# sloisel/MultiGridBarrierMPI.jl

Hardware: AMD Instinct MI355X
Metric: fem2d p-Laplace DoF/s per Newton step (higher is better)
Workload: dtype f64; 1 GPU; fem2d p-Laplace L=7 p=1 (n=57344 rows, N_L=49154 Newton unknowns), amgb main phase, tol=sqrt(eps); parallelism=single GPU

## Files before the change

### include/mgb_hip.h

```cpp
#ifndef MGB_HIP_H
#define MGB_HIP_H

#include <stdint.h>

#ifdef __cplusplus
extern "C" {
#endif

#define MGB_OK 0
#define MGB_E_ARG (-1)
#define MGB_E_HIP (-2)
#define MGB_E_NUMERIC (-3)
#define MGB_E_INTERNAL (-4)

typedef struct mgb_ctx_s* mgb_ctx;
typedef struct mgb_geo_s* mgb_geo;
typedef struct mgb_amg_s* mgb_amg;
typedef struct mgb_vec_s* mgb_vec;
typedef struct mgb_csr_s* mgb_csr;

const char* mgb_last_error(void);
int mgb_version(void);
int mgb_device_count(void);

// ... 43 lines not shown
int mgb_col_extract(mgb_vec M, int n, int K, int k, mgb_vec out);
int mgb_map_rows_barrier(int which, int K, int nterms, const int* kind, const int* nq, const int* idx_q, const int* idx_s,
                         const int* idx_s2, const double* p, const double* coef, const double* off, int n, mgb_vec Dz,
                         mgb_vec out);
int mgb_mul(mgb_vec x, mgb_vec y, mgb_vec out);
int mgb_axpy(mgb_vec x, double alpha, mgb_vec y, mgb_vec out);
int mgb_vec_allreduce_sum(mgb_vec x);
int mgb_all_isfinite(mgb_vec x, int* out);

int mgb_amg_create(mgb_ctx ctx, mgb_geo g, int S, const char* const* state_vars, int K, const char* const* D,
                   int nq, const int* idx_q, int idx_s, double p, mgb_amg* out);
int mgb_amg_create_cones(mgb_ctx ctx, mgb_geo g, int S, const char* const* state_vars, int K, const char* const* D,
                         int ncones, const int* nq, const int* idx_q, const int* idx_s, const int* idx_s2,
                         const double* p, mgb_amg* out);
int mgb_amg_create_terms(mgb_ctx ctx, mgb_geo g, int S, const char* const* state_vars, int K, const char* const* D,
                         int nterms, const int* kind, const int* nq, const int* idx_q, const int* idx_s, const int* idx_s2,
                         const double* p, const double* coef, const double* off, mgb_amg* out);
int mgb_amg_set_exponents(mgb_amg a, int term, const double* p_nodes);
int mgb_amg_set_term_mask(mgb_amg a, const unsigned char* mask);
int mgb_amg_destroy(mgb_amg a);
int mgb_amg_dims(mgb_amg a, int* n, int* S, int* K, int* L, int* nY);
int mgb_amg_local_rows(mgb_amg a, int* n_global, int* row0, int* n_local);
int mgb_amg_prepare(mgb_amg a, int level);
int mgb_amg_level_size(mgb_amg a, int level, int* N, int* nnz_lower);
int mgb_amg_f0_f32(mgb_amg a, int level, const float* s, float t, double* f0);
int mgb_amg_f1_f32(mgb_amg a, int level, const float* s, float t, float* g);
int mgb_amg_f2_f32(mgb_amg a, int level, const float* s, float t, float* lower_vals);
int mgb_amg_f1_template_f64(mgb_amg a, int level, const double* s, double t, double* g);
int mgb_amg_f2_template_f64(mgb_amg a, int level, const double* s, double t, double* lower_vals);
int mgb_amg_chol_info(mgb_amg a, int level, int* split_world, double* exchange_doubles, int* launches);
int mgb_amg_chol_schedule(mgb_amg a, int level, int cap, int* nlaunch, int* kind, int* workgroups, int* unknown_node,
                          int* unknown_col);
int mgb_amg_chol_tree(mgb_amg a, int level, int cap, int* nnodes, int* ns, int* nf, int* parent);
int mgb_amg_chol_values_local(mgb_amg a, int level, int* yes);
int mgb_amg_hessian_pattern(mgb_amg a, int level, int32_t* rowptr, int32_t* colidx);
int mgb_amg_set_c(mgb_amg a, const double* c);
int mgb_amg_set_z(mgb_amg a, const double* z);
int mgb_amg_get_z(mgb_amg a, double* z);
int mgb_amg_apply_D(mgb_amg a, int level, const double* s, double* Dz );
int mgb_amg_f0(mgb_amg a, int level, const double* s, double t, double* y, double* parts2);
int mgb_amg_f0_trial(mgb_amg a, int level, const double* s_ref, const double* s, double t, double* y);
int mgb_amg_f1(mgb_amg a, int level, const double* s, double t, double* g);
int mgb_amg_f2(mgb_amg a, int level, const double* s, double t, double* lower_vals);
int mgb_amg_solve_linear(mgb_amg a, int level, const double* lower_vals, const double* g, double* x);
int mgb_amg_solve_linear_gpu(mgb_amg a, int level, const double* lower_vals, const double* g, double* x);
int mgb_amg_set_solver(mgb_amg a, int solver);
int mgb_amg_set_schedule(mgb_amg a, int all_levels);
int mgb_amg_set_stop_rule(mgb_amg a, int upstream);
int mgb_amg_set_centering(mgb_amg a, int exact);
int mgb_amg_solve(mgb_amg a, double tol, double t0, double kappa, int maxit, int max_newton, int verbose);
int mgb_amg_set_early_stop(mgb_amg a, int col);
int mgb_amg_sol_info(mgb_amg a, int* nt, double* t_elapsed, double* time_factor, long long* counts4);
int mgb_amg_sol_get(mgb_amg a, long long* its , double* ts, double* c_dot_Dz);
int mgb_amg_sol_kernels(mgb_amg a, double* ms11, double* bytes11, long long* launches11);
int mgb_amg_time_kernels(mgb_amg a, int level, int reps, int nrot, double* ms8, double* bytes8);

int mgb_hessian_apply(mgb_amg a, int level, const double* s, const double* v, double* Hv, int matrix_free);
int mgb_smooth(mgb_amg a, int level, const double* s, const double* b, double* x, int degree, int sweeps, double lmax,
               int matrix_free, double* lmax_used);
int mgb_prolong(mgb_amg a, int level, const double* xc, double* xf);
int mgb_restrict(mgb_amg a, int level, const double* rf, double* rc);
int mgb_amg_prolongation(mgb_amg a, int level, int* rows, int* cols, int* nnz, int32_t* rowptr, int32_t* colidx, double* vals);
int mgb_amg_pcg_solve_linear(mgb_amg a, int level, const double* s, const double* g, double* x, int* iters, double* relres,
                             int* converged);
int mgb_amg_set_pcg(mgb_amg a, double rtol, int maxit, int degree, int power_its, double lo_frac, double hi_frac, int chunk,
                    int fallback, int assembled_top, int giveup);
int mgb_amg_sol_pcg(mgb_amg a, long long* counts4, double* time_s);
int mgb_amg_time_mg_kernels(mgb_amg a, int level, int reps, int nrot, double* ms6, double* bytes6, double* alg6);
int mgb_amg_mg_info(mgb_amg a, int top, int* coarsest);


typedef struct mgb_plan_s* mgb_plan;
int mgb_plan_create(mgb_geo g, int S, const char* const* state_vars, int K, const char* const* D, int nq,
                    const int* idx_q, int idx_s, int level, mgb_plan* out);
int mgb_reduction_scratch_doubles(int n_local, int max_level_unknowns, long long* out);
int mgb_plan_destroy(mgb_plan p);
int mgb_plan_prolongation(mgb_plan fine, mgb_plan coarse, int* rows, int* cols, int* nnz, int32_t* rowptr, int32_t* colidx,
                          double* vals);
int mgb_plan_sizes(mgb_plan p, int* N, int* nnz_lower, int* nnz_T, int* nnz_B);
int mgb_plan_pattern(mgb_plan p, int32_t* rowptr, int32_t* colidx);
int mgb_plan_eval_host(mgb_plan p, const double* Y , double* lower_vals);
int mgb_plan_shard(mgb_plan p, int S, int K, int rank, int world, int block, mgb_plan* out, int* r0, int* r1);
int mgb_plan_apply_B_host(mgb_plan p, const double* s , double* Bs );
int mgb_plan_apply_BT_host(mgb_plan p, const double* v , double* g );
int mgb_plan_chol_bench(mgb_plan p, const double* Y, int dim, int reps, double* seconds_per_factor,
                        double* seconds_per_solve, double* flops, double* front_doubles, double* residual);
typedef struct mgb_hostchol_s* mgb_hostchol;
int mgb_plan_hostchol_create(mgb_plan p, int dim, mgb_hostchol* out);
int mgb_hostchol_destroy(mgb_hostchol c);
int mgb_hostchol_info(mgb_hostchol c, int* n, int* threads, double* flops);
int mgb_hostchol_factor_solve(mgb_hostchol c, const double* lower_vals, const double* g, double* x);
int mgb_hostchol_partition(mgb_hostchol c, int world, int* split_world, int cap, int* nnodes, int* owner);
int mgb_hostchol_factor_solve_dist(mgb_hostchol c, int rank, int world, mgb_allreduce_fn fn, void* user,
                                   const double* lower_vals, const double* g, double* x);
int mgb_plan_hostchol_create_ranked(mgb_plan p, int dim, int K, int world, int block, mgb_hostchol* out);
int mgb_hostchol_rank_aligned(mgb_hostchol c, int world, int* aligned, int* top_values);
int mgb_hostchol_factor_solve_dist_local(mgb_hostchol c, int rank, int world, mgb_allreduce_fn fn, void* user,
                                         const double* local_lower_vals, const double* g, double* x);
int mgb_plan_chol_tree(mgb_plan p, int dim, int cap, int* nnodes, int* ns, int* nf, int* parent);
int mgb_plan_chol_bwd_fused(mgb_plan p, int dim, int cut, int top_nf, int threads, int* info, int cap_wg, int* wg, int cap_bdry,
                            int* bdry, int* slots, int cap_nodes, int* bofs, int* first);
int mgb_chol_selftest(int nx, int ny, double* max_residual, double* flops, double* seconds);

#ifdef __cplusplus
}
#endif
// ... 2 lines not shown
```

### multigridbarriermpi.jl_amd/__init__.py

```python
from __future__ import annotations

import math
from dataclasses import dataclass, field
from typing import Callable, Dict, List, Optional, Sequence

import numpy as np
import scipy.sparse as sp

from . import _lib
from ._lib import MGBError, call, dptr, f64, i32, iptr

import ctypes as C

__all__ = [
    "fem1d", "fem2d", "fem3d", "fem1d_mpi", "fem2d_mpi", "fem3d_mpi", "fem1d_mpi_solve", "fem2d_mpi_solve",
    "fem3d_mpi_solve", "parabolic_solve", "ParabolicSOL", "native_to_mpi",
    "mpi_to_native", "amgb", "Geometry", "AMGBSOL", "HPCVector", "HPCMatrix", "HPCSparseMatrix",
    "backend_hip", "amgb_zeros", "amgb_all_isfinite", "amgb_diag", "amgb_blockdiag", "map_rows", "map_rows_gpu",
    "_raw_array", "_to_cpu_array", "MGBError", "device_count", "AMG", "amg", "hcat", "BarrierFn", "barrier_functions",
]


def device_count() -> int:
    return int(_lib.load().mgb_device_count())
# ... 918 lines not shown
        rp, ci, va = np.empty(r.value + 1, dtype=np.int32), np.empty(nz.value, dtype=np.int32), np.empty(nz.value)
        call("mgb_amg_prolongation", self.handle, l, None, None, None, iptr(rp), iptr(ci), dptr(va))
        return sp.csr_matrix((va, ci, rp), shape=(r.value, c.value))

    def pcg_solve_linear(self, l, s, g):
        s, g = f64(s), f64(g)
        x = np.empty_like(g)
        it, ok, rr = C.c_int(), C.c_int(), C.c_double()
        call("mgb_amg_pcg_solve_linear", self.handle, l, dptr(s), dptr(g), dptr(x), C.byref(it), C.byref(rr), C.byref(ok))
        return x, it.value, rr.value, bool(ok.value)

    MG_KERNEL_NAMES = ("hessian_apply", "chebyshev_step", "hessian_apply_csr", "prolong", "restrict", "hessian_apply_unfused_csr")

    def time_mg_kernels(self, l, reps=50, nrot=1):
        ms, by, alg = np.empty(6), np.empty(6), np.empty(6)
        call("mgb_amg_time_mg_kernels", self.handle, int(l), int(reps), int(nrot), dptr(ms), dptr(by), dptr(alg))
        return {k: dict(ms=float(a), bytes=float(b), algorithmic_bytes=float(c)) for k, a, b, c in zip(self.MG_KERNEL_NAMES, ms, by, alg)}

    def mg_coarsest(self, top=None):
        c0 = C.c_int()
        call("mgb_amg_mg_info", self.handle, self.L - 1 if top is None else int(top), C.byref(c0))
        return c0.value

    def solve(self, tol=None, t=0.1, kappa=10.0, maxit=10000, max_newton=0, verbose=0, schedule="fine",
              solver="gpu", stop_rule="fixed", centering="exact"):
        if schedule not in ("fine", "all"):
            raise ValueError("schedule must be 'fine' or 'all'")
        if stop_rule not in ("fixed", "upstream"):
            raise ValueError("stop_rule must be 'fixed' or 'upstream'")
        if centering not in ("decrement", "exact"):
            raise ValueError("centering must be 'decrement' or 'exact'")
        call("mgb_amg_set_stop_rule", self.handle, 1 if stop_rule == "upstream" else 0)
        call("mgb_amg_set_centering", self.handle, 1 if centering == "exact" else 0)
        call("mgb_amg_set_schedule", self.handle, 1 if schedule == "all" else 0)
        self.set_solver(solver)
        call("mgb_amg_solve", self.handle, float(tol or 0.0), float(t), float(kappa), int(maxit), int(max_newton),
             int(verbose))
        nt, te, tf = C.c_int(), C.c_double(), C.c_double()
        counts = (C.c_longlong * 4)()
        call("mgb_amg_sol_info", self.handle, C.byref(nt), C.byref(te), C.byref(tf), counts)
        its = np.empty(self.L * nt.value, dtype=np.int64)
        ts = np.empty(nt.value)
        cd = np.empty(nt.value)
        call("mgb_amg_sol_get", self.handle, its.ctypes.data_as(_lib.c_ll_p), dptr(ts), dptr(cd))
        nk = len(self.KERNEL_NAMES)
        kms, kby = np.empty(nk), np.empty(nk)
        kl = np.empty(nk, dtype=np.int64)
        call("mgb_amg_sol_kernels", self.handle, dptr(kms), dptr(kby), kl.ctypes.data_as(_lib.c_ll_p))
        kernels = {k: dict(ms=float(m), bytes=float(b), launches=int(c))
                   for k, m, b, c in zip(self.KERNEL_NAMES, kms, kby, kl)}
        pc = (C.c_longlong * 4)()
        tp = C.c_double()
        call("mgb_amg_sol_pcg", self.handle, pc, C.byref(tp))
        return dict(t_elapsed=te.value, ts=ts, its=its.reshape(nt.value, self.L).T.copy(), c_dot_Dz=cd,
                    time_factor=tf.value, n_f0=counts[0], n_f1=counts[1], n_f2=counts[2], n_factor=counts[3],
                    kernels=kernels, pcg=dict(solves=pc[0], iterations=pc[1], fallbacks=pc[2], gave_up_at=pc[3], seconds=tp.value))

    KERNEL_NAMES = ("apply_D", "barrier_f2", "hessian_assemble", "barrier_f1", "restrict", "barrier_f0",
                    "chol_front_start", "chol_front_step", "chol_backward_rect", "chol_backward", "chol_front_single")

    def time_kernels(self, l, reps=50, nrot=1):
        ms = np.empty(8)
        by = np.empty(8)
        call("mgb_amg_time_kernels", self.handle, l, reps, int(nrot), dptr(ms), dptr(by))
        names = ("apply_D", "barrier_f2", "hessian_assemble", "barrier_f1", "restrict", "barrier_f0", "trial_f0")
        out = {k: dict(ms=float(m), bytes=float(b)) for k, m, b in zip(names, ms, by)}
        out["apply_D"]["element_local"] = bool(by[7])
        out["apply_D_csr"] = dict(ms=float(ms[7]), bytes=float(by[0]))
        return out

    def __del__(self):
        try:
            if getattr(self, "handle", None):
                _lib.load().mgb_amg_destroy(self.handle)
        except Exception:
            pass


def amg(geometry: Geometry, state_variables=DEFAULT_STATE, D=None, p=1.0, cones=None) -> AMG:
    return AMG(geometry, state_variables, D, p, cones=cones)


@dataclass
class AMGBSOL:
    z: object
    SOL_feasibility: Optional[dict]
    SOL_main: dict
    log: list
    geometry: Geometry


PHASE1_SLACK_FLOOR = 1.0
PHASE1_PENALTY = 10.0


def _phase1_slack(geometry, M: "AMG", p, z0, c, tol, schedule, solver):
    n, S = z0.shape
    K = len(M.D)
    cone, extras = M.cones[0], list(M.cones[1:])
    if len(extras) > 1 or cone[0] == "linear":
        raise NotImplementedError("amgb: the feasibility phase covers the power cone intersected with one half space")
    state1 = tuple(M.state_variables) + (("sigma", "full"),)
    D1 = tuple(M.D) + (("sigma", "id"),)
    terms = [(list(cone[0]), cone[1], K)]
    terms += [("linear", list(e[1]) + [K], list(map(float, e[2])) + [1.0], float(e[3])) for e in extras]
    terms.append(("linear", [K], [1.0], PHASE1_SLACK_FLOOR))
    Dz = M.apply_D_global(M.L - 1, np.zeros(M.level_size(M.L - 1)[0]))
    idx = list(cone[0])
# ... 250 lines not shown
```

### multigridbarriermpi.jl_amd/_lib.py

```python
from __future__ import annotations

import ctypes as C
import os

import numpy as np

_HERE = os.path.dirname(os.path.abspath(__file__))
LIB_PATH = os.path.join(_HERE, "lib", "libmgb_hip.so")

c_int_p = C.POINTER(C.c_int)
c_i32_p = C.POINTER(C.c_int32)
c_dbl_p = C.POINTER(C.c_double)
c_flt_p = C.POINTER(C.c_float)
c_ll_p = C.POINTER(C.c_longlong)
c_str_arr = C.POINTER(C.c_char_p)
H = C.c_void_p
ALLREDUCE_FN = C.CFUNCTYPE(C.c_int, C.c_void_p, C.c_void_p, C.c_longlong)


class MGBError(RuntimeError):
    def __init__(self, code, msg):
        super().__init__("mgb error %d: %s" % (code, msg))
        self.code = code

# ... 46 lines not shown
    "mgb_all_isfinite": [H, c_int_p],
    "mgb_amg_create": [H, H, C.c_int, c_str_arr, C.c_int, c_str_arr, C.c_int, c_int_p, C.c_int, C.c_double,
                       C.POINTER(H)],
    "mgb_amg_create_cones": [H, H, C.c_int, c_str_arr, C.c_int, c_str_arr, C.c_int, c_int_p, c_int_p, c_int_p, c_int_p,
                             c_dbl_p, C.POINTER(H)],
    "mgb_amg_create_terms": [H, H, C.c_int, c_str_arr, C.c_int, c_str_arr, C.c_int, c_int_p, c_int_p, c_int_p, c_int_p, c_int_p,
                             c_dbl_p, c_dbl_p, c_dbl_p, C.POINTER(H)],
    "mgb_amg_set_exponents": [H, C.c_int, c_dbl_p],
    "mgb_amg_set_term_mask": [H, C.POINTER(C.c_ubyte)],
    "mgb_amg_destroy": [H],
    "mgb_amg_dims": [H, c_int_p, c_int_p, c_int_p, c_int_p, c_int_p],
    "mgb_amg_local_rows": [H, c_int_p, c_int_p, c_int_p],
    "mgb_amg_prepare": [H, C.c_int],
    "mgb_amg_chol_info": [H, C.c_int, c_int_p, c_dbl_p, c_int_p],
    "mgb_amg_chol_schedule": [H, C.c_int, C.c_int, c_int_p, c_int_p, c_int_p, c_int_p, c_int_p],
    "mgb_amg_chol_tree": [H, C.c_int, C.c_int, c_int_p, c_int_p, c_int_p, c_int_p],
    "mgb_amg_chol_values_local": [H, C.c_int, c_int_p],
    "mgb_amg_level_size": [H, C.c_int, c_int_p, c_int_p],
    "mgb_amg_hessian_pattern": [H, C.c_int, c_i32_p, c_i32_p],
    "mgb_amg_set_c": [H, c_dbl_p],
    "mgb_amg_set_z": [H, c_dbl_p],
    "mgb_amg_get_z": [H, c_dbl_p],
    "mgb_amg_apply_D": [H, C.c_int, c_dbl_p, c_dbl_p],
    "mgb_amg_f0": [H, C.c_int, c_dbl_p, C.c_double, c_dbl_p, c_dbl_p],
    "mgb_amg_f0_trial": [H, C.c_int, c_dbl_p, c_dbl_p, C.c_double, c_dbl_p],
    "mgb_amg_f1": [H, C.c_int, c_dbl_p, C.c_double, c_dbl_p],
    "mgb_amg_f2": [H, C.c_int, c_dbl_p, C.c_double, c_dbl_p],
    "mgb_amg_set_early_stop": [H, C.c_int],
    "mgb_amg_f0_f32": [H, C.c_int, c_flt_p, C.c_float, c_dbl_p],
    "mgb_amg_f1_f32": [H, C.c_int, c_flt_p, C.c_float, c_flt_p],
    "mgb_amg_f2_f32": [H, C.c_int, c_flt_p, C.c_float, c_flt_p],
    "mgb_amg_f1_template_f64": [H, C.c_int, c_dbl_p, C.c_double, c_dbl_p],
    "mgb_amg_f2_template_f64": [H, C.c_int, c_dbl_p, C.c_double, c_dbl_p],
    "mgb_amg_solve_linear": [H, C.c_int, c_dbl_p, c_dbl_p, c_dbl_p],
    "mgb_amg_solve_linear_gpu": [H, C.c_int, c_dbl_p, c_dbl_p, c_dbl_p],
    "mgb_amg_set_solver": [H, C.c_int],
    "mgb_amg_set_schedule": [H, C.c_int],
    "mgb_amg_set_stop_rule": [H, C.c_int],
    "mgb_amg_set_centering": [H, C.c_int],
    "mgb_amg_set_pcg": [H, C.c_double, C.c_int, C.c_int, C.c_int, C.c_double, C.c_double, C.c_int, C.c_int, C.c_int, C.c_int],
    "mgb_amg_sol_pcg": [H, c_ll_p, c_dbl_p],
    "mgb_hessian_apply": [H, C.c_int, c_dbl_p, c_dbl_p, c_dbl_p, C.c_int],
    "mgb_smooth": [H, C.c_int, c_dbl_p, c_dbl_p, c_dbl_p, C.c_int, C.c_int, C.c_double, C.c_int, c_dbl_p],
    "mgb_prolong": [H, C.c_int, c_dbl_p, c_dbl_p],
    "mgb_restrict": [H, C.c_int, c_dbl_p, c_dbl_p],
    "mgb_amg_prolongation": [H, C.c_int, c_int_p, c_int_p, c_int_p, c_i32_p, c_i32_p, c_dbl_p],
    "mgb_amg_pcg_solve_linear": [H, C.c_int, c_dbl_p, c_dbl_p, c_dbl_p, c_int_p, c_dbl_p, c_int_p],
    "mgb_amg_mg_info": [H, C.c_int, c_int_p],
    "mgb_amg_time_mg_kernels": [H, C.c_int, C.c_int, C.c_int, c_dbl_p, c_dbl_p, c_dbl_p],
    "mgb_plan_prolongation": [H, H, c_int_p, c_int_p, c_int_p, c_i32_p, c_i32_p, c_dbl_p],
    "mgb_amg_solve": [H, C.c_double, C.c_double, C.c_double, C.c_int, C.c_int, C.c_int],
    "mgb_amg_sol_info": [H, c_int_p, c_dbl_p, c_dbl_p, c_ll_p],
    "mgb_amg_sol_get": [H, c_ll_p, c_dbl_p, c_dbl_p],
    "mgb_amg_sol_kernels": [H, c_dbl_p, c_dbl_p, c_ll_p],
    "mgb_amg_time_kernels": [H, C.c_int, C.c_int, C.c_int, c_dbl_p, c_dbl_p],
    "mgb_plan_create": [H, C.c_int, c_str_arr, C.c_int, c_str_arr, C.c_int, c_int_p, C.c_int, C.c_int,
                        C.POINTER(H)],
    "mgb_reduction_scratch_doubles": [C.c_int, C.c_int, c_ll_p],
    "mgb_plan_destroy": [H],
    "mgb_plan_sizes": [H, c_int_p, c_int_p, c_int_p, c_int_p],
    "mgb_plan_pattern": [H, c_i32_p, c_i32_p],
    "mgb_plan_eval_host": [H, c_dbl_p, c_dbl_p],
    "mgb_plan_shard": [H, C.c_int, C.c_int, C.c_int, C.c_int, C.c_int, C.POINTER(C.c_void_p), c_int_p, c_int_p],
    "mgb_plan_apply_B_host": [H, c_dbl_p, c_dbl_p],
    "mgb_plan_apply_BT_host": [H, c_dbl_p, c_dbl_p],
    "mgb_plan_chol_bench": [H, c_dbl_p, C.c_int, C.c_int, c_dbl_p, c_dbl_p, c_dbl_p, c_dbl_p, c_dbl_p],
    "mgb_plan_hostchol_create": [H, C.c_int, C.POINTER(H)],
    "mgb_hostchol_destroy": [H],
    "mgb_hostchol_info": [H, c_int_p, c_int_p, c_dbl_p],
    "mgb_hostchol_factor_solve": [H, c_dbl_p, c_dbl_p, c_dbl_p],
    "mgb_hostchol_partition": [H, C.c_int, c_int_p, C.c_int, c_int_p, c_int_p],
    "mgb_hostchol_factor_solve_dist": [H, C.c_int, C.c_int, ALLREDUCE_FN, C.c_void_p, c_dbl_p, c_dbl_p, c_dbl_p],
    "mgb_plan_hostchol_create_ranked": [H, C.c_int, C.c_int, C.c_int, C.c_int, C.POINTER(H)],
    "mgb_hostchol_rank_aligned": [H, C.c_int, c_int_p, c_int_p],
    "mgb_hostchol_factor_solve_dist_local": [H, C.c_int, C.c_int, ALLREDUCE_FN, C.c_void_p, c_dbl_p, c_dbl_p, c_dbl_p],
    "mgb_plan_chol_tree": [H, C.c_int, C.c_int, c_int_p, c_int_p, c_int_p, c_int_p],
    "mgb_plan_chol_bwd_fused": [H, C.c_int, C.c_int, C.c_int, C.c_int, c_int_p, C.c_int, c_int_p, C.c_int, c_int_p, c_int_p, C.c_int,
                                c_int_p, c_int_p],
    "mgb_chol_selftest": [C.c_int, C.c_int, c_dbl_p, c_dbl_p, c_dbl_p],
}
_SPECIAL = {"mgb_last_error": ([], C.c_char_p), "mgb_version": ([], C.c_int), "mgb_device_count": ([], C.c_int)}

_lib = None


def load():
    global _lib
    if _lib is not None:
        return _lib
    if not os.path.exists(LIB_PATH):
        raise ImportError("libmgb_hip.so not built: run `python -c 'import __graft_entry__ as g; g.build()'` "
                          "or multigridbarriermpi.jl_amd/csrc/build.sh (expected at %s)" % LIB_PATH)
    lib = C.CDLL(LIB_PATH)
    for name, args in PROTOTYPES.items():
        fn = getattr(lib, name)
        fn.argtypes = args
        fn.restype = C.c_int
    for name, (args, res) in _SPECIAL.items():
        fn = getattr(lib, name)
        fn.argtypes = args
        fn.restype = res
    _lib = lib
    return lib


def call(name, *args):
# ... 29 lines not shown
```

### multigridbarriermpi.jl_amd/csrc/amg.cpp

```cpp
#include "amg.hpp"


#include <chrono>
#include <cmath>
#include <thread>
#include <string>
#include <cstdlib>
#include <cstdio>

namespace mgb {

void hip_check(hipError_t e, const char* what) {
  if (e != hipSuccess) throw HipError(std::string("HIP error in ") + what + ": " + hipGetErrorString(e));
}

static inline void cpu_relax() {
#if defined(__x86_64__) || defined(__i386__)
  __builtin_ia32_pause();
#elif defined(__aarch64__)
  asm volatile("yield" ::: "memory");
#else
  std::this_thread::yield();
#endif
}

static double now_s() {
  return std::chrono::duration<double>(std::chrono::steady_clock::now().time_since_epoch()).count();
}

Ctx::Ctx(int dev) : device(dev) {
  int count = 0;
  hip_check(hipGetDeviceCount(&count), "hipGetDeviceCount");
  if (count <= 0) throw HipError("mgb: no HIP device visible (the HIP path has no CPU fallback)");
  if (dev < 0 || dev >= count) throw ArgError("mgb: device id out of range");
  hip_check(hipSetDevice(dev), "hipSetDevice");
  hip_check(hipStreamCreateWithFlags(&stream, hipStreamNonBlocking), "hipStreamCreate");
}

Ctx::~Ctx() {
  drop_comm();
  if (stream) (void)hipStreamDestroy(stream);
}

void Ctx::allreduce_sum(double* dev_ptr, long long count, bool even_single) {
  if ((world <= 1 && !(even_single && rccl_comm)) || count <= 0) return;
  if (rccl_comm) {
    rccl_allreduce(dev_ptr, count);
  } else {
    if (!allreduce) throw ArgError("mgb: sharded context without a communicator (mgb_ctx_set_comm_rccl / mgb_ctx_set_comm)");
    hip_check(hipStreamSynchronize(stream), "sync before allreduce");
    const int rc = allreduce(allreduce_user, dev_ptr, count);
    if (rc != 0) throw InternalError("mgb: allreduce callback failed with code " + std::to_string(rc));
  }
  n_allreduce++;
  allreduce_bytes += 8.0 * count;
}
// ... 307 lines not shown
        gather(q, S, u);
        const int nc = (int)u.cols.size();
        for (int i = 0; i < nc; ++i)
          for (int j = 0; j <= i; ++j) {
            int e = -1;
            int slot = base;
            for (int a = 0; a < nact; ++a)
              for (int b = a; b < nact; ++b, ++slot) {
                if (!structural(u, nc, a, b, i, j)) continue;
                if (e < 0) e = entry(u.cols[i], u.cols[j]);
                double coef = u.val[(size_t)a * nc + i] * u.val[(size_t)b * nc + j];
                if (a != b) coef += u.val[(size_t)b * nc + i] * u.val[(size_t)a * nc + j];
                terms.push_back({e, q * nY + slot, coef});
                cnt[e]++;
              }
          }
        base += S.nY();
      }
    }
  });
  phase("list terms");
  {
    long long tot = 0;
    for (int e = 0; e < nnzA; ++e) {
      pl.T.rowptr[e] = (int)tot;
      for (int t = 0; t < nthr; ++t) {
        const int c0 = tcnt[t][e];
        tcnt[t][e] = (int)tot;
        tot += c0;
      }
      if (tot > 2000000000LL) throw ArgError("amg: Hessian plan exceeds Int32 indexing");
    }
    pl.T.rowptr[nnzA] = (int)tot;
    pl.T.colidx.resize((size_t)tot);
    pl.T.vals.resize((size_t)tot);
  }
  chunks([&](int, int, int tI) {
    std::vector<int>& pos = tcnt[tI];
    for (const Term& tm : tterms[tI]) {
      const int pp = pos[tm.e]++;
      pl.T.colidx[pp] = tm.col;
      pl.T.vals[pp] = tm.coef;
    }
    std::vector<Term>().swap(tterms[tI]);
  });
  phase("fill terms");
}


Amg::Amg(Ctx& ctx, const GeometryHost& g, const AmgSpec& spec, const BarrierParams& P)
    : ctx_(ctx), n_(g.n), S_((int)spec.state_variables.size()), P_(P), spec_(spec) {
  hip_check(hipSetDevice(ctx_.device), "hipSetDevice");
  if (const char* e = std::getenv("MGB_FUSED_TRIAL_ROWS")) fused_trial_rows_ = std::atoi(e);
  if (P.K != (int)spec.D.size()) throw ArgError("amg: barrier K != number of D rows");
  if (P.ncones < 1 || P.ncones > kMaxCones) throw ArgError("amg: barrier supports 1 to 3 terms");
  if (P.K > 8) throw ArgError("amg: the barrier kernels support at most 8 rows of D");
  for (int ci = 0; ci < P.ncones; ++ci) {
    const ConeSpec& S = P.cone[ci];
    if (S.kind != 0 && S.kind != 1) throw ArgError("amg: unknown barrier term kind");
    if (S.nq < 1 || S.nq > 3) throw ArgError("amg: barrier supports 1..3 gradient components");
    for (int a = 0; a < S.nact(); ++a)
      if (S.col(a) < 0 || S.col(a) >= P.K) throw ArgError("amg: barrier index out of range");
  }
  if ((int)g.w.size() != n_ || (int)g.x.size() != n_ * g.dim) throw ArgError("amg: geometry x/w size mismatch");
  ng_ = g.n;
  Csr Dstack = build_dstack(g, spec);
  w_min_ = *std::min_element(g.w.begin(), g.w.end());
  if (ctx_.world > 1) {
    int r1 = 0;
    shard_rows(ctx_.rank, ctx_.world, ng_, g.block, &r0_, &r1);
    n_ = r1 - r0_;
    Dstack_.upload(shard_dstack(Dstack, ng_, S_, P.K, r0_, r1));
  } else {
    Dstack_.upload(Dstack);
  }
  w_.upload(g.w.data() + r0_, n_);
  const int K = P.K, nY = P.nY();
  c_.alloc((size_t)n_ * K);
  z_.alloc((size_t)n_ * S_);
  z_save_.alloc((size_t)n_ * S_);
  Dz0_.alloc((size_t)n_ * K);
  Dz0_save_.alloc((size_t)n_ * K);
  Dz_.alloc((size_t)n_ * K);
  DzA_.alloc((size_t)n_ * K);
  DzB_.alloc((size_t)n_ * K);
  DzC_.alloc((size_t)n_ * K);
  v_.alloc((size_t)n_ * K);
  Y_.alloc((size_t)n_ * nY);
  phi_cur_.alloc((size_t)n_ * P.ncones);
  phi_trial_.alloc((size_t)n_ * P.ncones);
  phi_trial2_.alloc((size_t)n_ * P.ncones);
  phi_trial3_.alloc((size_t)n_ * P.ncones);
  h_flag_.alloc(4);
  scal_.alloc(12);
  h_scal_.alloc(12);
  seq_dev_.alloc(1);
  hip_check(hipMemset(seq_dev_.p, 0, sizeof(unsigned long long)), "memset seq");
  h_seq_.alloc(1);
  h_seq_.p[0] = 0;
  hip_check(hipMemsetAsync(c_.p, 0, c_.n * sizeof(double), ctx_.stream), "memset");
  hip_check(hipMemsetAsync(z_.p, 0, z_.n * sizeof(double), ctx_.stream), "memset");
  hip_check(hipStreamSynchronize(ctx_.stream), "sync");
  geo_ = g;
  dstack_host_ = std::move(Dstack);
  for (int l = 0; l < g.L; ++l) {
    levels_.emplace_back(new Level);
    int N = 0;
    for (auto& sv : spec.state_variables) {
      if (sv.second == "fixed") continue;
      auto it = g.subspaces.find(sv.second);
      if (it == g.subspaces.end() || l >= (int)it->second.size())
        throw ArgError("amg: unknown subspace '" + sv.second + "'");
      N += it->second[l].cols;
    }
    levels_[l]->plan.N = N;
  }
  int maxN = 0;
  for (auto& lv : levels_) maxN = std::max(maxN, lv->plan.N);
  partials_.alloc(reduction_scratch_doubles(n_, maxN));
  hip_check(hipMemset(partials_.p, 0, partials_.n * sizeof(double)), "memset scratch");
}

size_t reduction_scratch_doubles(int n_local, int max_level_unknowns) {
  return (size_t)6 * std::max(f0_blocks(n_local), f0_blocks(max_level_unknowns)) + 8 + kReductionHeader;
}

int Amg::level_index(const Level& lv) const {
  for (size_t l = 0; l < levels_.size(); ++l)
    if (levels_[l].get() == &lv) return (int)l;
  throw InternalError("amg: level not found");
}

Amg::Level& Amg::level(int l) {
  Level& lv = *levels_.at(l);
  if (lv.built) return lv;
  if (lv.chol_analysis.joinable()) lv.chol_analysis.join();
  lv.chol_analyzed = false;
  lv.chol_analysis_error = nullptr;
  hip_check(hipSetDevice(ctx_.device), "hipSetDevice");
  static const bool use_elasm = !(std::getenv("MGB_ASSEMBLE") && std::string(std::getenv("MGB_ASSEMBLE")) == "plan");
  const bool try_elasm = use_elasm && ctx_.world == 1 && geo_.block > 1 && n_ % geo_.block == 0;
  lv.plan = build_level_plan(geo_, spec_, dstack_host_, l, P_, !try_elasm);
  lv.T_built = !try_elasm;
  if (ctx_.world > 1) {
    std::vector<unsigned long long> mask = dof_rank_masks(lv.plan.B, ng_, P_.K, ctx_.world, geo_.block);
    lv.plan = shard_level_plan(lv.plan, ng_, S_, P_.K, P_.nY(), r0_, r0_ + n_);
    lv.plan.rank_mask = std::move(mask);
  }
  if (!pcg_ && lv.plan.N > 0) {
    lv.chol_analysis = std::thread([this, &lv] {
      try {
        analyze_chol(lv);
      } catch (...) {
        lv.chol_analysis_error = std::current_exception();
      }
    });
  }
  const double t_up = now_s();
  lv.R.upload(lv.plan.R);
  lv.B.upload(lv.plan.B);
  if (n_ > fused_trial_rows_ && geo_.block > 1 && n_ % geo_.block == 0) lv.Bel.build(lv.plan.B, geo_.block * P_.K);
  lv.BT.upload(lv.plan.BT);
  if (lv.T_built) lv.T.upload(lv.plan.T);
  if (try_elasm && lv.plan.N > 0) {
    mg_of(lv);
    if (mg_ensure_elop(lv)) lv.elasm.build(lv.mg->elop, lv.plan.Apat, P_);
    if (!lv.elasm.view.valid()) ensure_T(lv);
  }
  const int N = lv.plan.N, nnzA = lv.plan.Apat.nnz();
  lv.s.alloc(N);
  lv.s_trial.alloc(N);
  lv.s_trial2.alloc(N);
  lv.s_trial3.alloc(N);
  lv.g_trial.alloc(N);
  lv.g.alloc(N);
  lv.nstep.alloc(N);
  lv.avals.alloc(nnzA);
  lv.h_avals.alloc(nnzA);
  lv.h_g.alloc(N);
  lv.h_n.alloc(N);
  lv.h_s.alloc(N);
  if (std::getenv("MGB_VERBOSE_SETUP")) std::fprintf(stderr, "[mgb setup] level upload + buffers       %.3f s\n", now_s() - t_up);
  lv.built = true;
  return lv;
}

void Amg::analyze_chol(Level& lv) {
  static const bool aligned_on = !(std::getenv("MGB_RANK_ALIGNED") && std::atoi(std::getenv("MGB_RANK_ALIGNED")) == 0);
  const bool ranked = aligned_on && ctx_.world > 1 && (int)lv.plan.rank_mask.size() == lv.plan.N;
  lv.chol.analyze(lv.plan.Apat, lv.plan.coords.data(), geo_.dim, 64, ranked ? lv.plan.rank_mask.data() : nullptr, ctx_.world);
  lv.chol_analyzed = true;
}

void Amg::ensure_chol(Level& lv) {
  if (lv.chol_built) return;
  hip_check(hipSetDevice(ctx_.device), "hipSetDevice");
  static const bool vt = std::getenv("MGB_VERBOSE_SETUP") != nullptr;
  double t0 = now_s();
  if (lv.chol_analysis.joinable()) lv.chol_analysis.join();
  if (lv.chol_analysis_error) {
    std::exception_ptr e = lv.chol_analysis_error;
    lv.chol_analysis_error = nullptr;
    std::rethrow_exception(e);
  }
  if (!lv.chol_analyzed) analyze_chol(lv);
  if (vt) std::fprintf(stderr, "[mgb setup] chol analyze (rest)         %.3f s\n", now_s() - t0);
  t0 = now_s();
  lv.gchol.build(lv.chol, &ctx_);
  if (vt) std::fprintf(stderr, "[mgb setup] gpuchol build + upload      %.3f s\n", now_s() - t0);
  lv.chol_built = true;
}

static double csr_bytes(const DevCsr& A, bool y0);

void Amg::ensure_T(Level& lv) {
  if (!lv.T_built) {
    build_plan_terms(lv.plan, ng_, P_);
    lv.T_built = true;
  }
  if (lv.T.view.rows == 0 && lv.plan.T.rows > 0) {
    hip_check(hipSetDevice(ctx_.device), "hipSetDevice");
    lv.T.upload(lv.plan.T);
  }
}

double Amg::assemble_bytes(Level& lv) {
// ... 206 lines not shown

void Amg::dev_apply(Level& lv, const double* s_dev, double* dz) {
  timer_.begin(ctx_.stream, KC_APPLY, csr_bytes(lv.B.view, true));
  if (lv.Bel.view.valid()) launch_spmv_el(ctx_.stream, lv.B.view, lv.Bel.view, s_dev, Dz0_.p, dz);
  else launch_spmv(ctx_.stream, lv.B.view, s_dev, Dz0_.p, dz);
  timer_.end(ctx_.stream);
}

double Amg::trial_bytes(const Level& lv, bool with_ref) const {
  return csr_bytes(lv.B.view, true) + (double)n_ * (P_.K + 1 + P_.ncones * (with_ref ? 2 : 1)) * 8;
}

void Amg::enqueue_f0(Level& lv, const double* s_dev, double alpha, const double* nstep, double* s_out, double* dz,
                     const double* phi_ref, double* phi_out, double* out2, HostSignal sig) {
  if (n_ <= fused_trial_rows_) {
    timer_.begin(ctx_.stream, KC_F0, trial_bytes(lv, phi_ref != nullptr));
    launch_trial_f0(ctx_.stream, lv.B.view, n_, P_, s_dev, alpha, nstep, s_out, Dz0_.p, dz, w_.p, c_.p, phi_ref,
                    kFracToBoundary, phi_out, partials_.p, out2, host_scal(out2), sig);
    timer_.end(ctx_.stream);
    return;
  }
  const double* x = s_dev;
  if (nstep) {
    launch_waxpby(ctx_.stream, lv.plan.N, s_dev, alpha, nstep, s_out);
    x = s_out;
  }
  dev_apply(lv, x, dz);
  timer_.begin(ctx_.stream, KC_F0, (double)n_ * (2 * P_.K + 2 + (phi_ref ? 1 : 0)) * 8);
  launch_barrier_f0(ctx_.stream, n_, P_, dz, w_.p, c_.p, phi_ref, kFracToBoundary, phi_out, partials_.p, out2, host_scal(out2), sig);
  timer_.end(ctx_.stream);
}

double Amg::dev_f0(Level& lv, const double* s_dev, double t, double* parts, const double* phi_ref, double* phi_out,
                   double* dz, double alpha, const double* nstep, double* s_out) {
  enqueue_f0(lv, s_dev, alpha, nstep, s_out, dz, phi_ref, phi_out, scal_.p, next_signal());
  if (ctx_.world > 1) {
    ctx_.allreduce_sum(scal_.p, 2);
    hip_check(hipMemcpyAsync(h_scal_.p, scal_.p, 2 * sizeof(double), hipMemcpyDeviceToHost, ctx_.stream), "D2H scal");
  }
  wait_signal("sync f0");
  if (parts) {
    parts[0] = h_scal_.p[0];
    parts[1] = h_scal_.p[1];
  }
  return h_scal_.p[0] + t * h_scal_.p[1];
}

bool Amg::values_stay_local(Level& lv) {
  if (ctx_.world <= 1 || host_solve_) return false;
  ensure_chol(lv);
  return lv.gchol.values_local();
}

void Amg::enqueue_f2_assemble(Level& lv, const double* dz, SolveStats& st) {
  timer_.begin(ctx_.stream, KC_F2, (double)n_ * (P_.K + 1 + P_.nY()) * 8);
  launch_barrier_f2(ctx_.stream, n_, P_, dz, w_.p, Y_.p);
  timer_.end(ctx_.stream);
  if (pcg_) {
    mg_values(level_index(lv));
    st.n_f2++;
    return;
  }
  timer_.begin(ctx_.stream, KC_ASSEMBLE, assemble_bytes(lv));
  assemble_values(lv);
  timer_.end(ctx_.stream);
  if (!values_stay_local(lv)) ctx_.allreduce_sum(lv.avals.p, lv.plan.Apat.nnz());
  st.n_f2++;
}

double Amg::dev_f1(Level& lv, const double* dz, double t, double* g_out, SolveStats* st, const double** pre) {
  timer_.begin(ctx_.stream, KC_F1, (double)n_ * (3 * P_.K + 1) * 8);
  launch_barrier_f1(ctx_.stream, n_, P_, dz, w_.p, c_.p, t, v_.p);
  timer_.end(ctx_.stream);
  timer_.begin(ctx_.stream, KC_RESTRICT, csr_bytes(lv.BT.view, false));
  launch_spmv(ctx_.stream, lv.BT.view, v_.p, nullptr, g_out);
  timer_.end(ctx_.stream);
  if (owner_local(lv)) {
    const int ntop = lv.gchol.ntop_unknowns();
    if (gtop_.n < (size_t)ntop + 1) gtop_.alloc((size_t)ntop + 1);
    launch_gather_top(ctx_.stream, ntop, lv.gchol.top_unknowns(), g_out, gtop_.p);
    launch_dot_owned(ctx_.stream, lv.plan.N, g_out, g_out, lv.gchol.unknown_kind(), 0, partials_.p, gtop_.p + ntop);
    ctx_.allreduce_sum(gtop_.p, ntop + 1);
    launch_scatter_top_norm(ctx_.stream, ntop, lv.gchol.top_unknowns(), gtop_.p, g_out, scal_.p + 2);
  } else {
    ctx_.allreduce_sum(g_out, lv.plan.N);
    launch_dot(ctx_.stream, lv.plan.N, g_out, g_out, partials_.p, scal_.p + 2, host_scal(scal_.p + 2), nullptr, nullptr, next_signal());
  }
  if (ctx_.world > 1)
    hip_check(hipMemcpyAsync(h_scal_.p + 2, scal_.p + 2, sizeof(double), hipMemcpyDeviceToHost, ctx_.stream), "D2H gg");
  if (host_solve_)
    hip_check(hipMemcpyAsync(lv.h_g.p, g_out, (size_t)lv.plan.N * sizeof(double), hipMemcpyDeviceToHost, ctx_.stream),
              "D2H g");
  if (pre && st && !host_solve_) {
    if (!pcg_) ensure_chol(lv);
    if (ctx_.world > 1) {
      if (!ev_f1_) hip_check(hipEventCreateWithFlags(&ev_f1_, hipEventDisableTiming), "event");
      hip_check(hipEventRecord(ev_f1_, ctx_.stream), "record f1");
    }
    enqueue_f2_assemble(lv, dz, *st);
    *pre = dz;
    if (ctx_.world == 1) wait_signal("sync f1");
    else hip_check(hipEventSynchronize(ev_f1_), "sync f1 event");
  } else {
    wait_signal("sync f1");
  }
  return std::sqrt(h_scal_.p[2]);
}

static const double kBeta = 0.5, kArmijo = 0.1, kMinStep = 1e-8;

void Amg::enqueue_trial(Level& lv, Trial& T, double step, int slot, HostSignal sig) {
  double* out = scal_.p + 4 + 2 * slot;
  enqueue_f0(lv, lv.s.p, -step, lv.nstep.p, T.s, T.dz, phi_cur_.p, T.phi, out, sig);
  T.step = step;
}

static const double kSpecSteps[3] = {1.0, kBeta, kBeta * kBeta};

void Amg::enqueue_spec_trials(Level& lv, Trial* spec, HostSignal sig) {
  const int ns = spec_count();
  if (ns == 3) {
    TrialSet T;
    T.na = 3;
    for (int q = 0; q < 3; ++q) {
      T.alpha[q] = -kSpecSteps[q];
      T.s_out[q] = spec[q].s;
      T.dz[q] = spec[q].dz;
      T.phi_out[q] = spec[q].phi;
      spec[q].step = kSpecSteps[q];
    }
    T.out_dev = scal_.p + 4;
    T.out_host = host_scal(scal_.p + 4);
    timer_.begin(ctx_.stream, KC_F0, trial_bytes(lv, true) + 2.0 * n_ * (P_.K + P_.ncones) * 8);
    launch_trial_set(ctx_.stream, lv.B.view, n_, P_, lv.s.p, lv.nstep.p, T, Dz0_.p, w_.p, c_.p, phi_cur_.p, kFracToBoundary,
                     partials_.p, sig);
    timer_.end(ctx_.stream);
  } else {
    enqueue_trial(lv, spec[0], kSpecSteps[0], 0);
    enqueue_trial(lv, spec[1], kSpecSteps[1], 1, sig);
  }
}

void Amg::launch_step_graph(Level& lv, Trial* spec) {
  const void* key[15] = {lv.avals.p, lv.g.p, lv.nstep.p, lv.s.p, spec[0].s, spec[0].phi, spec[0].dz, spec[1].s, spec[1].phi,
                         spec[1].dz, spec[2].s,  spec[2].phi, spec[2].dz, phi_cur_.p, Dz0_.p};
  for (const auto& g : lv.step_graphs)
    if (std::equal(key, key + 15, g.key)) {
      hip_check(hipGraphLaunch(g.exec, ctx_.stream), "hipGraphLaunch");
      ++seq_expected_;
      for (int q = 0; q < spec_count(); ++q) spec[q].step = kSpecSteps[q];
      return;
    }
  hipGraph_t graph = nullptr;
  hip_check(hipStreamBeginCapture(ctx_.stream, hipStreamCaptureModeThreadLocal), "hipStreamBeginCapture");
  try {
    lv.gchol.enqueue_chain(ctx_.stream, lv.avals.p, lv.g.p, lv.nstep.p);
    launch_dot(ctx_.stream, lv.plan.N, lv.g.p, lv.nstep.p, partials_.p, scal_.p + 3, host_scal(scal_.p + 3), lv.gchol.fail_flag(),
               h_flag_.p);
    HostSignal sig;
    sig.seq_dev = seq_dev_.p;
    sig.seq_host = h_seq_.p;
    enqueue_spec_trials(lv, spec, sig);
  } catch (...) {
    (void)hipStreamEndCapture(ctx_.stream, &graph);
    if (graph) (void)hipGraphDestroy(graph);
    throw;
  }
  hip_check(hipStreamEndCapture(ctx_.stream, &graph), "hipStreamEndCapture");
  Level::StepGraph sg{};
  std::copy(key, key + 15, sg.key);
  hipError_t e = hipGraphInstantiate(&sg.exec, graph, nullptr, nullptr, 0);
  (void)hipGraphDestroy(graph);
  hip_check(e, "hipGraphInstantiate");
  lv.step_graphs.push_back(sg);
  hip_check(hipGraphLaunch(sg.exec, ctx_.stream), "hipGraphLaunch");
  ++seq_expected_;
}

bool Amg::dev_f2_solve(Level& lv, const double* dz, double t, SolveStats& st, double* inc, Trial* spec,
                       const double* pre_assembled) {
  const int N = lv.plan.N, nnzA = lv.plan.Apat.nnz();
  if (!pcg_) ensure_chol(lv);
  if (pre_assembled != dz) enqueue_f2_assemble(lv, dz, st);
  st.n_factor++;
  timer_.sample((st.n_factor % 8) == 1);
  if (pcg_) {
    const int top = level_index(lv);
    bool ok = pcg_run(lv, top, lv.g.p, lv.nstep.p, &st, nullptr, nullptr);
    if (!ok && pcg_last_code_ == 2.0) {
      for (int l = mg_coarsest(top); l <= top; ++l)
        if (level(l).mg) level(l).mg->ev_warm = false;
      mg_values(top);
      ok = pcg_run(lv, top, lv.g.p, lv.nstep.p, &st, nullptr, nullptr);
    }
    h_flag_.p[0] = 0;
    if (ok) pcg_bad_streak_ = 0;
    if (!ok) {
      if (!pcg_opt.fallback) return false;
      st.pcg_fallbacks++;
      if (pcg_opt.giveup > 0 && ++pcg_bad_streak_ >= pcg_opt.giveup) {
        pcg_ = false;
        st.pcg_gaveup_at = st.n_factor;
      }
      ensure_chol(lv);
      assemble_values(lv);
      lv.gchol.factor_solve(ctx_.stream, lv.avals.p, lv.g.p, lv.nstep.p, nullptr, false);
      lv.flag_armed = false;
      hip_check(hipMemcpyAsync(h_flag_.p, lv.gchol.fail_flag(), sizeof(int), hipMemcpyDeviceToHost, ctx_.stream), "D2H flag");
    }
    launch_dot(ctx_.stream, N, lv.g.p, lv.nstep.p, partials_.p, scal_.p + 3, host_scal(scal_.p + 3), nullptr, nullptr,
               spec ? HostSignal() : next_signal());
    if (spec) {
      enqueue_spec_trials(lv, spec, next_signal());
      st.n_f0 += spec_count();
    }
    wait_signal("sync pcg solve");
    if (!ok) hip_check(hipStreamSynchronize(ctx_.stream), "sync fallback flag");
    if (spec)
      for (int q = 0; q < spec_count(); ++q) {
        spec[q].y = h_scal_.p[4 + 2 * q] + t * h_scal_.p[5 + 2 * q];
        spec[q].valid = true;
      }
    *inc = h_scal_.p[3];
    return h_flag_.p[0] == 0;
  }
  if (!host_solve_) {
    const bool use_graph = GpuChol::knobs().graph;
    KernelTimer* tm = (live_ && timer_.sampling()) ? &timer_ : nullptr;
    const bool flag_rides = ctx_.world == 1;
    hipEvent_t e0 = nullptr, e1 = nullptr;
    const bool time_chain = live_ && timer_.enabled() && (st.n_factor % 8) == 5;
    if (flag_rides && spec && !tm && !time_chain && use_graph && lv.flag_armed) {
      launch_step_graph(lv, spec);
      st.n_f0 += spec_count();
    } else {
      if (time_chain) {
        hip_check(hipEventCreate(&e0), "event");
        hip_check(hipEventCreate(&e1), "event");
        hip_check(hipEventRecord(e0, ctx_.stream), "record");
      }
      const bool olocal = owner_local(lv);
      lv.gchol.factor_solve(ctx_.stream, lv.avals.p, lv.g.p, lv.nstep.p, tm, flag_rides && lv.flag_armed, false, olocal);
      if (time_chain) hip_check(hipEventRecord(e1, ctx_.stream), "record");
      if (olocal) {
        launch_dot_owned(ctx_.stream, N, lv.g.p, lv.nstep.p, lv.gchol.unknown_kind(), ctx_.rank == 0, partials_.p, scal_.p + 3);
        launch_flag_to_double(ctx_.stream, lv.gchol.fail_flag(), scal_.p + 10);
      } else if (flag_rides) {
        launch_dot(ctx_.stream, N, lv.g.p, lv.nstep.p, partials_.p, scal_.p + 3, host_scal(scal_.p + 3), lv.gchol.fail_flag(),
                   h_flag_.p, spec ? HostSignal() : next_signal());
        lv.flag_armed = true;
      } else {
        launch_dot(ctx_.stream, N, lv.g.p, lv.nstep.p, partials_.p, scal_.p + 3);
        hip_check(hipMemcpyAsync(h_flag_.p, lv.gchol.fail_flag(), sizeof(int), hipMemcpyDeviceToHost, ctx_.stream), "D2H flag");
      }
      if (spec) {
        enqueue_spec_trials(lv, spec, next_signal());
        if (!olocal) ctx_.allreduce_sum(scal_.p + 4, 2 * spec_count());
        st.n_f0 += spec_count();
      }
      if (olocal) {
        if (!spec) hip_check(hipMemsetAsync(scal_.p + 4, 0, 6 * sizeof(double), ctx_.stream), "zero trial slots");
        ctx_.allreduce_sum(scal_.p + 3, 8);
        hip_check(hipMemcpyAsync(h_scal_.p + 3, scal_.p + 3, 8 * sizeof(double), hipMemcpyDeviceToHost, ctx_.stream), "D2H inc + trials + flag");
      } else if (ctx_.world > 1)
        hip_check(hipMemcpyAsync(h_scal_.p + 3, scal_.p + 3, (spec ? 1 + 2 * spec_count() : 1) * sizeof(double),
                                 hipMemcpyDeviceToHost, ctx_.stream), "D2H inc + trials");
    }
    wait_signal("sync solve");
    if (owner_local(lv)) h_flag_.p[0] = h_scal_.p[10] != 0.0 ? 1 : 0;
    if (spec)
      for (int q = 0; q < spec_count(); ++q) {
        spec[q].y = h_scal_.p[4 + 2 * q] + t * h_scal_.p[5 + 2 * q];
        spec[q].valid = true;
      }
    if (e0) {
      float ms = 0;
      hip_check(hipEventSynchronize(e1), "sync chain event");
      if (hipEventElapsedTime(&ms, e0, e1) == hipSuccess) st.time_factor += 8.0 * ms * 1e-3;
      (void)hipEventDestroy(e0);
      (void)hipEventDestroy(e1);
    }
    *inc = h_scal_.p[3];
    if (h_flag_.p[0] != 0 && h_flag_.p[0] != 1)
      throw InternalError("gpuchol: pivot flag holds " + std::to_string(h_flag_.p[0]) + " (only 0 / 1 are ever written)");
    return h_flag_.p[0] == 0;
  }
  hip_check(hipMemcpyAsync(lv.h_avals.p, lv.avals.p, (size_t)nnzA * sizeof(double), hipMemcpyDeviceToHost, ctx_.stream),
            "D2H avals");
  sync_collect("sync f2");
  const double t0 = now_s();
  bool ok = lv.chol.factor(lv.h_avals.p);
  double acc = 0;
  if (ok) {
    std::copy(lv.h_g.p, lv.h_g.p + N, lv.h_n.p);
    lv.chol.solve(lv.h_n.p);
    for (int i = 0; i < N; ++i) acc += lv.h_g.p[i] * lv.h_n.p[i];
    hip_check(hipMemcpyAsync(lv.nstep.p, lv.h_n.p, (size_t)N * sizeof(double), hipMemcpyHostToDevice, ctx_.stream),
              "H2D n");
  }
  st.time_factor += now_s() - t0;
  *inc = acc;
  return ok;
}


Amg::NewtonResult Amg::newton(int l, double t, bool finest, bool final, double lam_tol, int maxit, SolveStats& st, int verbose) {
  Level& lv = level(l);
  const int N = lv.plan.N;
  NewtonResult res;
  if (N == 0) {
    res.converged = true;
    return res;
  }
  hip_check(hipMemsetAsync(lv.s.p, 0, (size_t)N * sizeof(double), ctx_.stream), "memset s");
  double y = dev_f0(lv, lv.s.p, t, nullptr, nullptr, phi_cur_.p, Dz_.p);
  st.n_f0++;
  if (!std::isfinite(y)) {
    std::vector<double> hdz((size_t)n_ * P_.K);
    Dz_.download(hdz.data(), hdz.size());
    int bad = 0, worst = -1;
    double minphi = INFINITY;
    for (int q = 0; q < n_; ++q) {
      const double* d = hdz.data() + (size_t)q * P_.K;
      double phi = INFINITY, sv = INFINITY;
      for (int ci = 0; ci < P_.ncones; ++ci) {
        const ConeSpec& S = P_.cone[ci];
        if (S.kind == 1) {
          double ph = S.off;
          for (int i = 0; i < S.nq; ++i) ph += S.coef[i] * d[S.iq[i]];
          phi = std::min(phi, ph);
          continue;
        }
        double qq = 0;
        for (int i = 0; i < S.nq; ++i) qq += d[S.iq[i]] * d[S.iq[i]];
        const double sc = d[S.is] + (S.is2 >= 0 ? d[S.is2] : 0.0);
        phi = std::min(phi, (sc > 0 ? std::pow(sc, S.a) : -1.0) - qq);
        sv = std::min(sv, sc);
      }
      if (!(phi > 0) || !(sv > 0)) bad++;
      if (!(phi >= minphi)) {
        minphi = phi;
        worst = q;
      }
    }
    char buf[256];
    snprintf(buf, sizeof buf, "newton: infeasible start (level %d, t=%g, %d of %d rows outside the cone, min phi=%g at row %d, y=%g)",
             l, t, bad, n_, minphi, worst, y);
    throw NumericError(buf);
  }
  double gnorm = dev_f1(lv, Dz_.p, t, lv.g.p);
  st.n_f1++;
  double ymin = y, gmin = gnorm, incmin = INFINITY;
  const double theta = finest ? 0.1 : 0.5;
  Trial T[3];
  T[0].s = lv.s_trial.p;
  T[0].phi = phi_trial_.p;
  T[1].s = lv.s_trial2.p;
  T[1].phi = phi_trial2_.p;
  T[2].s = lv.s_trial3.p;
  T[2].phi = phi_trial3_.p;
  T[0].dz = DzA_.p;
  T[1].dz = DzB_.p;
  T[2].dz = DzC_.p;
  auto eval = [&](int pos, double step) {
    if (!(T[pos].valid && T[pos].step == step))
      for (int q = 0; q < 3; ++q)
        if (q != pos && T[q].valid && T[q].step == step) {
          std::swap(T[pos], T[q]);
          break;
        }
    Trial& X = T[pos];
    if (X.valid && X.step == step) return X.y;
    X.y = dev_f0(lv, lv.s.p, t, nullptr, phi_cur_.p, X.phi, X.dz, -step, lv.nstep.p, X.s);
    st.n_f0++;
    X.step = step;
    X.valid = true;
    return X.y;
  };
  const double* pre = nullptr;
  const bool speculate = !host_solve_;
  while (res.k < maxit && !res.converged) {
    res.k++;
    double inc = 0;
    T[0].valid = T[1].valid = T[2].valid = false;
    const double* have = pre;
    pre = nullptr;
    if (!dev_f2_solve(lv, Dz_.p, t, st, &inc, speculate ? T : nullptr, have)) {
      if (verbose > 1) fprintf(stderr, "    [mgb] level %d k=%d: Hessian not numerically SPD (pivot flag %d)\n", l, res.k, h_flag_.p[0]);
      break;
    }
    if (!std::isfinite(inc)) {
      if (verbose > 1) fprintf(stderr, "    [mgb] level %d k=%d: non-finite Newton decrement\n", l, res.k);
      break;
    }
    if (inc <= 0) {
      res.converged = true;
      break;
    }
    double step = 1.0, ynext = y, gnext = gnorm;
    bool accepted = false;
    while (step >= kMinStep) {
      double yA = eval(0, step);
      if (std::isfinite(yA) && yA <= y - kArmijo * step * inc) {
        while (step * kBeta >= kMinStep) {
          const double yB = eval(1, step * kBeta);
          if (!(std::isfinite(yB) && yB < yA)) break;
          std::swap(T[0], T[1]);
          yA = yB;
          step *= kBeta;
        }
        const double gn = dev_f1(lv, T[0].dz, t, lv.g_trial.p, &st, speculate ? &pre : nullptr);
        st.n_f1++;
        if (std::isfinite(gn)) {
          ynext = yA;
          gnext = gn;
          accepted = true;
          break;
        }
      }
      step *= kBeta;
    }
    if (accepted) {
      std::swap(lv.s.p, T[0].s);
      std::swap(phi_cur_.p, T[0].phi);
      std::swap(lv.g.p, lv.g_trial.p);
      std::swap(Dz_.p, T[0].dz);
    } else {
      step = 0.0;
      if (host_solve_)
        hip_check(hipMemcpy(lv.h_g.p, lv.g.p, (size_t)N * sizeof(double), hipMemcpyDeviceToHost), "D2H g");
    }
    const bool exact = ynext >= ymin && gnext >= theta * gmin;
    const double dec_tol = finest ? kDecrementFrac * w_min_ : lam_tol;
    if ((!(finest && final) && inc < dec_tol) || exact) res.converged = true;
    y = ynext;
    gnorm = gnext;
    ymin = std::min(ymin, y);
    gmin = std::min(gmin, gnorm);
    incmin = std::min(incmin, inc);
    if (verbose > 1)
      fprintf(stderr, "    [mgb] level %d k=%d y=%.12g |g|=%.3g inc=%.3g step=%.3g\n", l, res.k, y, gnorm, inc, step);
  }
  lv.s_trial.p = T[0].s;
  lv.s_trial2.p = T[1].s;
  lv.s_trial3.p = T[2].s;
  phi_trial_.p = T[0].phi;
  phi_trial2_.p = T[1].phi;
  phi_trial3_.p = T[2].phi;
  DzA_.p = T[0].dz;
  DzB_.p = T[1].dz;
  DzC_.p = T[2].dz;
  return res;
}

bool Amg::amgb_step(double t, bool final, double lam_tol, int max_newton, std::vector<long long>& its, SolveStats& st, int verbose) {
  const int L = (int)levels_.size();
  bool converged = true;
  for (int J = (schedule_all_ ? 0 : L - 1); J < L; ++J) {
    Level& lv = level(J);
    NewtonResult r = newton(J, t, J == L - 1, final, lam_tol, max_newton, st, verbose);
    its[J] += r.k;
    if (lv.plan.N > 0) {
      launch_spmv(ctx_.stream, lv.R.view, lv.s.p, z_.p, z_.p);
      hip_check(hipMemcpyAsync(Dz0_.p, Dz_.p, (size_t)n_ * P_.K * sizeof(double), hipMemcpyDeviceToDevice,
                               ctx_.stream), "Dz0 <- Dz");
    }
    if (J == L - 1) converged = r.converged;
  }
  return converged;
}

double Amg::c_dot_dz() {
  launch_barrier_f0(ctx_.stream, n_, P_, Dz0_.p, w_.p, c_.p, nullptr, 0.0, nullptr, partials_.p, scal_.p, host_scal(scal_.p));
  if (ctx_.world > 1) {
    ctx_.allreduce_sum(scal_.p, 2);
    hip_check(hipMemcpyAsync(h_scal_.p, scal_.p, 2 * sizeof(double), hipMemcpyDeviceToHost, ctx_.stream), "D2H scal");
  }
  hip_check(hipStreamSynchronize(ctx_.stream), "sync");
  return h_scal_.p[1];
}

bool Amg::slack_negative() {
  std::vector<double> h((size_t)n_ * P_.K);
  hip_check(hipStreamSynchronize(ctx_.stream), "sync early stop");
  Dz0_.download(h.data(), h.size());
  double bad = 0;
  for (int q = 0; q < n_; ++q) bad += (h[(size_t)q * P_.K + early_stop_col_] < 0.0) ? 0.0 : 1.0;
  if (ctx_.world > 1) {
    hip_check(hipMemcpy(scal_.p, &bad, sizeof(double), hipMemcpyHostToDevice), "H2D early stop");
    ctx_.allreduce_sum(scal_.p, 1);
    hip_check(hipMemcpy(&bad, scal_.p, sizeof(double), hipMemcpyDeviceToHost), "D2H early stop");
  }
  return bad == 0.0;
}

void Amg::solve(const SolveOptions& opt, SolveStats& st) {
  hip_check(hipSetDevice(ctx_.device), "hipSetDevice");
  const int L = (int)levels_.size();
  st = SolveStats();
  st.L = L;
  live_ = &st;
  timer_.enable(opt.time_kernels);
  struct LiveGuard {
    Amg* a;
// ... 28 lines not shown
  double t_stop = t;
  while (t_stop <= 1 / opt.tol) t_stop *= kappa0;
  if (early_stop_col_ >= P_.K) throw ArgError("amgb: early-stop column out of range");
  const bool fixed = !opt.upstream_stop;
  auto going = [&](double tt) { return fixed ? tt < t_stop : tt <= 1 / opt.tol; };
  auto final_at = [&](double tt) { return opt.exact_centering || early_stop_col_ >= 0 || !going(tt); };
  {
    bool ok0 = false;
    for (int attempt = 0; attempt < kInitialCenteringAttempts && !ok0; ++attempt)
      ok0 = amgb_step(t, final_at(t), lam_tol, opt.max_newton, its, st, opt.verbose);
    if (!ok0) throw NumericError("amgb: initial centering failed");
  }
  st.its.insert(st.its.end(), its.begin(), its.end());
  st.ts.push_back(t);
  st.c_dot_Dz.push_back(c_dot_dz());
  int k = 1;
  bool stopped = early_stop_col_ >= 0 && slack_negative();
  while (going(t) && kappa > 1 && k < opt.maxit && !stopped) {
    k++;
    std::fill(its.begin(), its.end(), 0);
    while (kappa > 1) {
      const double t1 = fixed ? std::min(kappa * t, t_stop) : kappa * t;
      hip_check(hipMemcpyAsync(z_save_.p, z_.p, zbytes, hipMemcpyDeviceToDevice, ctx_.stream), "save z");
      hip_check(hipMemcpyAsync(Dz0_save_.p, Dz0_.p, dzbytes, hipMemcpyDeviceToDevice, ctx_.stream), "save Dz0");
      std::vector<long long> it1(L, 0);
      bool ok = amgb_step(t1, final_at(t1), lam_tol, opt.max_newton, it1, st, opt.verbose);
      if (!going(t1) && !opt.exact_centering && early_stop_col_ < 0)
        for (int attempt = 0; attempt < kInitialCenteringAttempts - 1 && !ok; ++attempt)
          ok = amgb_step(t1, true, lam_tol, opt.max_newton, it1, st, opt.verbose);
      long long mx = 0;
      for (int l = 0; l < L; ++l) {
        its[l] += it1[l];
        mx = std::max(mx, it1[l]);
      }
      if (ok) {
        if (mx <= opt.max_newton * kKappaGrowFrac) kappa = std::min(kappa0, kappa * kappa);
        t = t1;
        break;
      }
      hip_check(hipMemcpyAsync(z_.p, z_save_.p, zbytes, hipMemcpyDeviceToDevice, ctx_.stream), "restore z");
      hip_check(hipMemcpyAsync(Dz0_.p, Dz0_save_.p, dzbytes, hipMemcpyDeviceToDevice, ctx_.stream), "restore Dz0");
      kappa = std::sqrt(kappa);
      if (kappa < 1 + 1e-3) kappa = 1.0;
    }
    st.its.insert(st.its.end(), its.begin(), its.end());
    st.ts.push_back(t);
    st.c_dot_Dz.push_back(c_dot_dz());
    if (opt.verbose)
      fprintf(stderr, "[mgb] t=%.4g kappa=%.3g its(finest)=%lld c.Dz=%.12g\n", t, kappa, its[L - 1], st.c_dot_Dz.back());
    stopped = early_stop_col_ >= 0 && slack_negative();
  }
  hip_check(hipStreamSynchronize(ctx_.stream), "sync");
  st.t_elapsed = now_s() - t_begin;
  if (going(t) && !stopped) throw NumericError("amgb: convergence failure (kappa collapsed)");
}


double Amg::f0(int l, const double* s_host, double t, double* parts) {
  Level& lv = level(l);
  resync_signals();
  lv.s_trial.upload(s_host, lv.plan.N);
  return dev_f0(lv, lv.s_trial.p, t, parts, nullptr, phi_cur_.p, Dz_.p);
}

double Amg::f0_trial(int l, const double* s_ref_host, const double* s_host, double t) {
  Level& lv = level(l);
  resync_signals();
  lv.s_trial.upload(s_ref_host, lv.plan.N);
  dev_f0(lv, lv.s_trial.p, t, nullptr, nullptr, phi_cur_.p, Dz_.p);
  lv.s_trial.upload(s_host, lv.plan.N);
  return dev_f0(lv, lv.s_trial.p, t, nullptr, phi_cur_.p, phi_trial_.p, Dz_.p);
}

void Amg::f1(int l, const double* s_host, double t, double* g_host) {
  Level& lv = level(l);
  resync_signals();
  lv.s_trial.upload(s_host, lv.plan.N);
  dev_apply(lv, lv.s_trial.p, Dz_.p);
  dev_f1(lv, Dz_.p, t, lv.g_trial.p);
  lv.g_trial.download(g_host, lv.plan.N);
}

void Amg::f2(int l, const double* s_host, double t, double* avals_host) {
  (void)t;
  Level& lv = level(l);
  resync_signals();
  lv.s_trial.upload(s_host, lv.plan.N);
  dev_apply(lv, lv.s_trial.p, Dz_.p);
  launch_barrier_f2(ctx_.stream, n_, P_, Dz_.p, w_.p, Y_.p);
  assemble_values(lv);
  ctx_.allreduce_sum(lv.avals.p, lv.plan.Apat.nnz());
  hip_check(hipStreamSynchronize(ctx_.stream), "sync f2");
  lv.avals.download(avals_host, lv.plan.Apat.nnz());
}

void Amg::ensure_f32(Level& lv) {
  const size_t nK = (size_t)n_ * P_.K;
  if (w32_.n != (size_t)n_) {
    w32_.alloc(n_);
    c32_.alloc(nK);
    Dz0_32_.alloc(nK);
    Dz32_.alloc(nK);
    v32_.alloc(nK);
    Y32_.alloc((size_t)n_ * P_.nY());
    rowF_.alloc(n_);
    rowC_.alloc(n_);
  }
  launch_to_f32(ctx_.stream, n_, w_.p, w32_.p);
  launch_to_f32(ctx_.stream, (long long)nK, c_.p, c32_.p);
// ... 213 lines not shown
```

### multigridbarriermpi.jl_amd/csrc/amg.hpp

```cpp
#pragma once
#include <memory>
#include <string>
#include <utility>
#include <thread>
#include <exception>
#include <vector>

#include "geometry.hpp"
#include "gpuchol.hpp"
#include "kernels.hpp"
#include "mfchol.hpp"
#include "mg.hpp"

namespace mgb {

void hip_check(hipError_t e, const char* what);

typedef int (*AllreduceFn)(void* user, double* dev_ptr, long long count);

struct Ctx {
  int device = 0;
  hipStream_t stream = nullptr;
  int rank = 0, world = 1;
  AllreduceFn allreduce = nullptr;
// ... 115 lines not shown
  Csr R;
  Csr B;
  Csr BT;
  Csr Apat;
  Csr T;
  std::vector<double> coords;
  std::vector<unsigned long long> rank_mask;
};

void shard_rows(int rank, int world, int n, int block, int* r0, int* r1);
std::vector<unsigned long long> dof_rank_masks(const Csr& B, int n, int K, int world, int block);
LevelPlan shard_level_plan(const LevelPlan& full, int n, int S, int K, int nY, int r0, int r1);
Csr shard_dstack(const Csr& Dstack, int n, int S, int K, int r0, int r1);

size_t reduction_scratch_doubles(int n_local, int max_level_unknowns);

Csr build_dstack(const GeometryHost& g, const AmgSpec& spec);
LevelPlan build_level_plan(const GeometryHost& g, const AmgSpec& spec, const Csr& Dstack, int level,
                           const BarrierParams& P, bool with_T = true);
void build_plan_terms(LevelPlan& pl, int n, const BarrierParams& P);

enum KernelClass {
  KC_APPLY = 0, KC_F2 = 1, KC_ASSEMBLE = 2, KC_F1 = 3, KC_RESTRICT = 4, KC_F0 = 5,
  KC_CHOL_START = 6, KC_CHOL_STEP = 7, KC_CHOL_BWD_RECT = 8, KC_CHOL_BWD = 9, KC_CHOL_SINGLE = 10, KC_COUNT = 11
};

constexpr double kFracToBoundary = 0.1;
constexpr double kKappaGrowFrac = 0.25;
constexpr int kInitialCenteringAttempts = 8;
constexpr double kDecrementFrac = 0.01;

struct SolveOptions {
  bool host_solve = false;
  bool pcg = false;
  bool schedule_all = false;
  bool time_kernels = true;
  bool upstream_stop = false;
  bool exact_centering = true;
  double tol = 1.4901161193847656e-08;
  double t0 = 0.1;
  double kappa = 10.0;
  int maxit = 10000;
  int max_newton = 48;
  int verbose = 0;
};

struct SolveStats {
  int L = 0;
  std::vector<long long> its;
  std::vector<double> ts, c_dot_Dz;
  double t_elapsed = 0, t_setup = 0;
  double time_factor = 0, time_device = 0;
  long long n_factor = 0, n_f0 = 0, n_f1 = 0, n_f2 = 0;
  long long pcg_solves = 0, pcg_iters = 0, pcg_fallbacks = 0;
  long long pcg_gaveup_at = -1;
  double time_pcg = 0;
  double kern_ms[KC_COUNT] = {};
  double kern_bytes[KC_COUNT] = {};
  long long kern_launches[KC_COUNT] = {};
};

class KernelTimer {
 public:
  ~KernelTimer();
  void enable(bool on) { on_ = on; sampling_ = true; }
  void sample(bool now) { sampling_ = now; }
  bool sampling() const { return on_ && sampling_; }
  bool enabled() const { return on_; }
  void begin(hipStream_t st, int cls, double bytes);
  void end(hipStream_t st);
  void collect(SolveStats& st);
 private:
  struct Pair {
    hipEvent_t a, b;
    int cls;
    double bytes;
  };
  std::vector<Pair> free_, pending_;
  Pair cur_{};
  bool on_ = false, open_ = false, sampling_ = true;
};

class Amg {
 public:
  Amg(Ctx& ctx, const GeometryHost& g, const AmgSpec& spec, const BarrierParams& P);
  int n() const { return n_; }
  int n_global() const { return ng_; }
  int row0() const { return r0_; }
  int S() const { return S_; }
  int K() const { return P_.K; }
  int L() const { return (int)levels_.size(); }
  int level_size(int l) const { return levels_[l]->plan.N; }
  const LevelPlan& plan(int l);
  void prepare(int l);
  const BarrierParams& params() const { return P_; }
  void chol_info(int l, int* split_world, double* exchange_doubles, int* launches);
  void chol_schedule(int l, int cap, int* nlaunch, int* kind, int* workgroups, int* unknown_node, int* unknown_col);
  void chol_tree(int l, int cap, int* nnodes, int* ns, int* nf, int* parent);
  bool chol_values_local(int l) { return values_stay_local(level(l)); }
  void set_early_stop(int col) { early_stop_col_ = col; }
  void set_exponents(int term, const double* p_nodes_global);
  void set_term_mask(const unsigned char* mask_global);
  void set_pcg(bool on) { pcg_ = on; }

  void set_c(const double* c_host);
  void set_z(const double* z_host);
  void get_z(double* z_host);

  double f0(int l, const double* s_host, double t, double* parts);
  double f0_trial(int l, const double* s_ref_host, const double* s_host, double t);
  void f1(int l, const double* s_host, double t, double* g_host);
  void f2(int l, const double* s_host, double t, double* avals_host);
  double f0_f32(int l, const float* s_host, float t);
  void f1_f32(int l, const float* s_host, float t, float* g_host);
  void f2_f32(int l, const float* s_host, float t, float* avals_host);
  void f1_tpl64(int l, const double* s_host, double t, double* g_host);
  void f2_tpl64(int l, const double* s_host, double t, double* avals_host);
  void apply_D(int l, const double* s_host, double* Dz_host);
  bool solve_host(int l, const double* avals, const double* g, double* nstep);
  bool solve_device(int l, const double* avals, const double* g, double* nstep);

  void solve(const SolveOptions& opt, SolveStats& st);

  struct KernelTimes {
    double apply_ms, f2_ms, assemble_ms, f1_ms, restrict_ms, f0_ms, trial_ms, apply_csr_ms, apply_el;
    double apply_bytes, f2_bytes, assemble_bytes, f1_bytes, restrict_bytes, f0_bytes, trial_bytes;
  };
  KernelTimes time_kernels(int l, int reps, int nrot = 1);

 private:
  struct Level {
    bool built = false, chol_built = false, T_built = false;
    DevElAsmOwned elasm;
    bool flag_armed = false;
    struct StepGraph {
      const void* key[15];
      hipGraphExec_t exec;
    };
    std::vector<StepGraph> step_graphs;
    std::thread chol_analysis;
    std::exception_ptr chol_analysis_error;
    bool chol_analyzed = false;
    ~Level() {
      if (chol_analysis.joinable()) chol_analysis.join();
      for (auto& g : step_graphs) (void)hipGraphExecDestroy(g.exec);
    }
    LevelPlan plan;
    DevCsrOwned R, B, BT, T;
    DevElCsrOwned Bel;
    DevBuf<float> B32, BT32, T32, s32, g32, avals32;
    bool f32_built = false;
    MfChol chol;
    GpuChol gchol;
    DevBuf<double> s, s_trial, s_trial2, s_trial3, g, g_trial, nstep, avals;
    PinnedBuf<double> h_avals, h_g, h_n, h_s;
    struct Mg {
      bool elop_tried = false, assembled = false, transfer = false, vectors = false;
      DevElOpOwned elop;
      DevBuf<double> elbuf;
      DevCsrOwned A;
      DevBuf<int> amap, diagpos, lo_rowptr, lo_colidx;
      DevCsrOwned P, PT;
      DevBuf<double> dinv, x, b, r, d0, d1, ev0, ev1, coef, Ainv;
      bool ev_warm = false;
    };
    std::unique_ptr<Mg> mg;
  };
  struct NewtonResult {
    int k = 0;
    bool converged = false;
  };
  Level& level(int l);
  int level_index(const Level& lv) const;
  void ensure_chol(Level& lv);
  void analyze_chol(Level& lv);
  void ensure_T(Level& lv);
  void assemble_values(Level& lv);
  double assemble_bytes(Level& lv);
  void refresh_dz0();
  void dev_apply(Level& lv, const double* s_dev, double* dz);
  double dev_f0(Level& lv, const double* s_dev, double t, double* parts, const double* phi_ref, double* phi_out,
                double* dz, double alpha = 0.0, const double* nstep = nullptr, double* s_out = nullptr);
  double trial_bytes(const Level& lv, bool with_ref) const;
  int fused_trial_rows_ = 64 * 2048;
  void enqueue_f0(Level& lv, const double* s_dev, double alpha, const double* nstep, double* s_out, double* dz,
                  const double* phi_ref, double* phi_out, double* out2, HostSignal sig = HostSignal());
  double dev_f1(Level& lv, const double* dz, double t, double* g_out, SolveStats* st = nullptr, const double** pre = nullptr);
  void enqueue_f2_assemble(Level& lv, const double* dz, SolveStats& st);
  bool values_stay_local(Level& lv);
  bool owner_local(Level& lv) { return in_solve_ && values_stay_local(lv); }
  bool in_solve_ = false;
  DevBuf<double> gtop_;
  struct EventHolder {
    hipEvent_t e = nullptr;
    ~EventHolder() {
      if (e) (void)hipEventDestroy(e);
    }
  } ev_f1_holder_;
  hipEvent_t& ev_f1_ = ev_f1_holder_.e;
  struct Trial {
    double* s = nullptr;
    double* phi = nullptr;
    double* dz = nullptr;
    double step = 0, y = 0;
    bool valid = false;
  };
  bool dev_f2_solve(Level& lv, const double* dz, double t, SolveStats& st, double* inc, Trial* spec = nullptr,
                    const double* pre_assembled = nullptr);
  void enqueue_trial(Level& lv, Trial& T, double step, int slot, HostSignal sig = HostSignal());
  int spec_count() const { return n_ <= fused_trial_rows_ ? 3 : 2; }
  void enqueue_spec_trials(Level& lv, Trial* spec, HostSignal sig);
  void launch_step_graph(Level& lv, Trial* spec);
  NewtonResult newton(int l, double t, bool finest, bool final, double lam_tol, int maxit, SolveStats& st, int verbose);
  bool amgb_step(double t, bool final, double lam_tol, int max_newton, std::vector<long long>& its, SolveStats& st, int verbose);
  double c_dot_dz();

 public:
  PcgOptions pcg_opt;
  void hessian_apply(int l, const double* s_host, const double* v_host, double* out_host, bool matrix_free);
  double mg_smooth(int l, const double* s_host, const double* b_host, double* x_host, int degree, int sweeps, double lmax,
                   bool matrix_free);
  void mg_prolong(int l, const double* xc_host, double* xf_host);
  void mg_restrict(int l, const double* rf_host, double* rc_host);
  int mg_coarsest(int top);
  bool pcg_solve_linear(int l, const double* s_host, const double* g_host, double* x_host, int* iters, double* relres);
  const Csr& prolongation_host(int l);
  struct MgKernelTimes {
    double ms[6], bytes[6], alg[6];
  };
  MgKernelTimes time_mg_kernels(int l, int reps, int nrot);

 private:
  Level::Mg& mg_of(Level& lv);
  void mg_ensure_vectors(Level& lv);
  bool mg_ensure_elop(Level& lv);
  void mg_ensure_assembled(Level& lv);
  void mg_ensure_transfer(int l);
  void mg_prepare(int top);
  bool mg_top_matrix_free(int top);
  void mg_values(int top);
  void mg_level_values(Level& lv, bool mf);
  void mg_estimate(Level& lv, bool mf, double lmax_given);
  void mg_apply(Level& lv, bool mf, const MgEpi& epi);
  void mg_smooth_pre(Level& lv, bool mf, const double* b, double* x, double* r, int degree, const double* done);
  void mg_smooth_post(Level& lv, bool mf, const double* b, double* x, double* r, int degree, const double* done);
  void mg_vcycle(int top, int l, const double* b, double* x, const double* done);
  bool pcg_run(Level& lv, int top, const double* g, double* x, SolveStats* st, int* iters, double* relres);
  void eval_Y_at(Level& lv, const double* s_host);
  std::vector<Csr> P_host_;
  DevBuf<double> mg_scal_, mg_scratch_, pcg_r_, pcg_z_, pcg_p_, pcg_Ap_;
  PinnedBuf<double> h_pcg_;
  DevBuf<int> mg_fail_;
  bool mg_inited_ = false;
  bool pcg_ = false;
  double pcg_last_code_ = 0;
  int pcg_bad_streak_ = 0;

  Ctx& ctx_;
  int n_ = 0, S_ = 0;
  int ng_ = 0, r0_ = 0;
  int early_stop_col_ = -1;
  bool slack_negative();
  DevBuf<float> w32_, c32_, Dz0_32_, Dz32_, v32_, Y32_;
  DevBuf<double> rowF_, rowC_, a_node_, mu_node_;
  DevBuf<unsigned char> term_mask_;
  void ensure_f32(Level& lv);
  BarrierParams P_;
  AmgSpec spec_;
  GeometryHost geo_;
  Csr dstack_host_;
  DevCsrOwned Dstack_;
  std::vector<std::unique_ptr<Level>> levels_;
  DevBuf<double> w_, c_, z_, z_save_, Dz0_, Dz0_save_, Dz_, DzA_, DzB_, DzC_, v_, Y_, partials_, scal_, phi_cur_, phi_trial_, phi_trial2_,
      phi_trial3_;
  PinnedBuf<int> h_flag_;
  bool host_solve_ = false;
  PinnedBuf<double> h_scal_;
  double w_min_ = 0;
  bool schedule_all_ = false;
  KernelTimer timer_;
  SolveStats* live_ = nullptr;
  void sync_collect(const char* what);
  DevBuf<unsigned long long> seq_dev_;
  PinnedBuf<unsigned long long> h_seq_;
  unsigned long long seq_expected_ = 0;
  void resync_signals();
  HostSignal next_signal();
  void wait_signal(const char* what);
  double* host_scal(double* dev_slot) const { return ctx_.world == 1 ? h_scal_.p + (dev_slot - scal_.p) : nullptr; }
};

}
```

### multigridbarriermpi.jl_amd/csrc/capi.cpp

```cpp
#include "../../include/mgb_hip.h"

#include <chrono>
#include <cmath>
#include <cstdlib>
#include <string>
#include <thread>

#include "amg.hpp"

using namespace mgb;

struct mgb_ctx_s {
  Ctx ctx;
  explicit mgb_ctx_s(int dev) : ctx(dev) {}
};
struct mgb_geo_s {
  GeometryHost g;
};
struct mgb_vec_s {
  mgb_ctx_s* ctx;
  DevBuf<double> buf;
  int n;
};
struct mgb_csr_s {
// ... 506 lines not shown
    std::vector<double> h(z->n);
    hip_check(hipStreamSynchronize(ctx->ctx.stream), "sync");
    z->buf.download(h.data(), z->n);
    Csr A(m, n);
    for (int i = 0; i < m; ++i) {
      if (i < d) {
        A.colidx.push_back(i);
        A.vals.push_back(h[i]);
      }
      A.rowptr[i + 1] = (int)A.colidx.size();
    }
    *out = new_csr(ctx, std::move(A));
  });
}
int mgb_spmv_add(mgb_csr A, mgb_vec x, mgb_vec y0, mgb_vec y) {
  return guard([&] {
    need(A && x && y, "null argument");
    need(A->A.view.cols == x->n && A->A.view.rows == y->n && (!y0 || y0->n == y->n), "spmv: shape mismatch");
    launch_spmv(A->ctx->ctx.stream, A->A.view, x->buf.p, y0 ? y0->buf.p : nullptr, y->buf.p);
    hip_check(hipGetLastError(), "spmv launch");
  });
}
int mgb_spmv(mgb_csr A, mgb_vec x, mgb_vec y) { return mgb_spmv_add(A, x, nullptr, y); }
int mgb_dot(mgb_vec x, mgb_vec y, double* out) {
  return guard([&] {
    need(x && y && out && x->n == y->n, "dot: shape mismatch");
    *out = reduce_scalar(x, [&](hipStream_t st, double* parts, double* res) { launch_dot(st, x->n, x->buf.p, y->buf.p, parts, res); });
  });
}
int mgb_norm(mgb_vec x, double* out) {
  return guard([&] {
    need(x && out, "null argument");
    *out = std::sqrt(reduce_scalar(x, [&](hipStream_t st, double* parts, double* res) { launch_dot(st, x->n, x->buf.p, x->buf.p, parts, res); }));
  });
}
int mgb_sum(mgb_vec x, double* out) {
  return guard([&] {
    need(x && out, "null argument");
    *out = reduce_scalar(x, [&](hipStream_t st, double* parts, double* res) { launch_sum(st, x->n, x->buf.p, parts, res); });
  });
}
int mgb_col_extract(mgb_vec M, int n, int K, int k, mgb_vec out) {
  return guard([&] {
    need(M && out && n >= 0 && K >= 1 && k >= 0 && k < K, "col_extract: bad arguments");
    need((long long)n * K == M->n && out->n == n, "col_extract: shape mismatch");
    launch_col_extract(M->ctx->ctx.stream, n, K, k, M->buf.p, out->buf.p);
    hip_check(hipGetLastError(), "col_extract launch");
  });
}
int mgb_map_rows_barrier(int which, int K, int nterms, const int* kind, const int* nq, const int* idx_q, const int* idx_s,
                         const int* idx_s2, const double* p, const double* coef, const double* off, int n, mgb_vec Dz,
                         mgb_vec out) {
  return guard([&] {
    need(Dz && out && n >= 0 && K >= 1 && K <= 8 && which >= 0 && which <= 2, "map_rows_barrier: bad arguments");
    BarrierParams P = make_params_terms(K, nterms, kind, nq, idx_q, idx_s, idx_s2, p, coef, off);
    const long long want = which == 0 ? n : (which == 1 ? (long long)n * K : (long long)n * K * K);
    need((long long)n * K == Dz->n && out->n == want, "map_rows_barrier: shape mismatch");
    hipStream_t st = Dz->ctx->ctx.stream;
    hip_check(hipSetDevice(Dz->ctx->ctx.device), "hipSetDevice");
    if (which == 0) {
      launch_barrier_rows_F(st, n, P, Dz->buf.p, out->buf.p);
    } else {
      std::vector<double> ones((size_t)std::max(n, 1), 1.0);
      DevBuf<double> w;
      w.upload(ones.data(), ones.size());
      if (which == 1) {
        DevBuf<double> c;
        c.alloc((size_t)std::max(n, 1) * K);
        hip_check(hipMemsetAsync(c.p, 0, c.n * sizeof(double), st), "memset");
        if (n) launch_barrier_f1(st, n, P, Dz->buf.p, w.p, c.p, 0.0, out->buf.p);
        hip_check(hipStreamSynchronize(st), "sync");
      } else {
        DevBuf<double> Y;
        Y.alloc((size_t)std::max(n, 1) * P.nY());
        if (n) launch_barrier_f2(st, n, P, Dz->buf.p, w.p, Y.p);
        launch_expand_hessian_rows(st, n, P, Y.p, out->buf.p);
        hip_check(hipStreamSynchronize(st), "sync");
      }
    }
    hip_check(hipGetLastError(), "map_rows_barrier launch");
  });
}
int mgb_mul(mgb_vec x, mgb_vec y, mgb_vec out) {
  return guard([&] {
    need(x && y && out && x->n == y->n && x->n == out->n, "mul: shape mismatch");
    launch_mul(x->ctx->ctx.stream, x->n, x->buf.p, y->buf.p, out->buf.p);
  });
}
int mgb_axpy(mgb_vec x, double alpha, mgb_vec y, mgb_vec out) {
  return guard([&] {
    need(x && y && out && x->n == y->n && x->n == out->n, "axpy: shape mismatch");
    launch_waxpby(x->ctx->ctx.stream, x->n, x->buf.p, alpha, y->buf.p, out->buf.p);
  });
}
int mgb_vec_allreduce_sum(mgb_vec x) {
  return guard([&] {
    need(x, "null argument");
    x->ctx->ctx.allreduce_sum(x->buf.p, x->n, true);
    hip_check(hipStreamSynchronize(x->ctx->ctx.stream), "sync allreduce");
  });
}
int mgb_all_isfinite(mgb_vec x, int* out) {
  return guard([&] {
    need(x && out, "null argument");
    hipStream_t st = x->ctx->ctx.stream;
    DevBuf<int> flag;
    flag.alloc(1);
    launch_all_isfinite(st, x->n, x->buf.p, flag.p);
    hip_check(hipStreamSynchronize(st), "sync");
    int h = 0;
    flag.download(&h, 1);
    *out = h != 0;
  });
}

int mgb_amg_create(mgb_ctx ctx, mgb_geo g, int S, const char* const* state_vars, int K, const char* const* D, int nq,
                   const int* idx_q, int idx_s, double p, mgb_amg* out) {
  return guard([&] {
    need(ctx && g && out, "null argument");
// ... 328 lines not shown
    if (coarsest) *coarsest = a->amg->mg_coarsest(top);
  });
}
int mgb_amg_set_stop_rule(mgb_amg a, int upstream) {
  return guard([&] {
    need(a, "null amg");
    a->upstream_stop = upstream != 0;
  });
}
int mgb_amg_set_centering(mgb_amg a, int exact) {
  return guard([&] {
    need(a, "null amg");
    a->exact_centering = exact != 0;
  });
}
int mgb_amg_set_schedule(mgb_amg a, int all_levels) {
  return guard([&] {
    need(a, "null amg");
    a->schedule_all = all_levels != 0;
  });
}
int mgb_amg_solve(mgb_amg a, double tol, double t0, double kappa, int maxit, int max_newton, int verbose) {
  return guard([&] {
    need(a, "null amg");
    SolveOptions o;
    o.schedule_all = a->schedule_all;
    o.host_solve = a->host_solve;
    o.pcg = a->pcg;
    o.upstream_stop = a->upstream_stop;
    o.exact_centering = a->exact_centering;
    if (tol > 0) o.tol = tol;
    if (t0 > 0) o.t0 = t0;
    if (kappa > 1) o.kappa = kappa;
    if (maxit > 0) o.maxit = maxit;
    if (max_newton > 0) o.max_newton = max_newton;
    o.verbose = verbose;
    const double ts = a->stats.t_setup;
    a->amg->solve(o, a->stats);
    a->stats.t_setup = ts;
  });
}
int mgb_amg_sol_info(mgb_amg a, int* nt, double* t_elapsed, double* time_factor, long long* counts4) {
  return guard([&] {
    need(a, "null amg");
    if (nt) *nt = (int)a->stats.ts.size();
    if (t_elapsed) *t_elapsed = a->stats.t_elapsed;
    if (time_factor) *time_factor = a->stats.time_factor;
    if (counts4) {
      counts4[0] = a->stats.n_f0;
      counts4[1] = a->stats.n_f1;
      counts4[2] = a->stats.n_f2;
      counts4[3] = a->stats.n_factor;
    }
  });
}
int mgb_amg_sol_get(mgb_amg a, long long* its, double* ts, double* c_dot_Dz) {
  return guard([&] {
    need(a, "null amg");
    if (its) std::copy(a->stats.its.begin(), a->stats.its.end(), its);
    if (ts) std::copy(a->stats.ts.begin(), a->stats.ts.end(), ts);
    if (c_dot_Dz) std::copy(a->stats.c_dot_Dz.begin(), a->stats.c_dot_Dz.end(), c_dot_Dz);
  });
}
int mgb_amg_sol_kernels(mgb_amg a, double* ms11, double* bytes11, long long* launches11) {
  return guard([&] {
    need(a, "null amg");
    for (int i = 0; i < KC_COUNT; ++i) {
      if (ms11) ms11[i] = a->stats.kern_ms[i];
      if (bytes11) bytes11[i] = a->stats.kern_bytes[i];
      if (launches11) launches11[i] = a->stats.kern_launches[i];
    }
  });
}
int mgb_amg_time_kernels(mgb_amg a, int level, int reps, int nrot, double* ms8, double* bytes8) {
  return guard([&] {
    need(a && ms8 && bytes8 && reps > 0 && nrot >= 1 && nrot <= 64 && level >= 0 && level < a->amg->L(), "time_kernels: bad arguments");
    Amg::KernelTimes k = a->amg->time_kernels(level, reps, nrot);
    const double ms[8] = {k.apply_ms, k.f2_ms, k.assemble_ms, k.f1_ms, k.restrict_ms, k.f0_ms, k.trial_ms, k.apply_csr_ms};
    const double by[8] = {k.apply_bytes, k.f2_bytes, k.assemble_bytes, k.f1_bytes, k.restrict_bytes, k.f0_bytes, k.trial_bytes,
                          k.apply_el};
    std::copy(ms, ms + 8, ms8);
    std::copy(by, by + 8, bytes8);
  });
}

int mgb_plan_prolongation(mgb_plan fine, mgb_plan coarse, int* rows, int* cols, int* nnz, int32_t* rowptr, int32_t* colidx,
                          double* vals) {
  return guard([&] {
    need(fine && coarse, "null plan");
    Csr P = build_prolongation(fine->plan.R, coarse->plan.R);
    if (rows) *rows = P.rows;
    if (cols) *cols = P.cols;
    if (nnz) *nnz = P.nnz();
    if (rowptr) std::copy(P.rowptr.begin(), P.rowptr.end(), rowptr);
    if (colidx) std::copy(P.colidx.begin(), P.colidx.end(), colidx);
    if (vals) std::copy(P.vals.begin(), P.vals.end(), vals);
  });
}
int mgb_plan_create(mgb_geo g, int S, const char* const* state_vars, int K, const char* const* D, int nq,
                    const int* idx_q, int idx_s, int level, mgb_plan* out) {
  return guard([&] {
    need(g && out, "null argument");
    AmgSpec spec = make_spec(S, state_vars, K, D);
    BarrierParams P = make_params(K, nq, idx_q, idx_s, 1.0);
    Csr Dstack = build_dstack(g->g, spec);
    auto* p = new mgb_plan_s;
// ... 302 lines not shown
```

### multigridbarriermpi.jl_amd/csrc/devutil.hpp

```cpp
#pragma once
#include <hip/hip_runtime.h>

#include "kernels.hpp"

namespace mgb {
namespace {

constexpr int kBlock = 256;
constexpr int kMaxBlocks = 2048;

inline int grid_for(long long work_items) {
  long long b = (work_items + kBlock - 1) / kBlock;
  if (b < 1) b = 1;
  if (b > kMaxBlocks) b = kMaxBlocks;
  return (int)b;
}

__device__ inline unsigned xcd_block(unsigned b, unsigned nb) {
  if (nb < 16u) return b;
  const unsigned per = nb >> 3, main = per << 3;
  return b < main ? (b & 7u) * per + (b >> 3) : b;
}

__device__ inline double wave_sum(double v) {
#pragma unroll
  for (int o = 32; o > 0; o >>= 1) v += __shfl_down(v, o, 64);
  return v;
}

__device__ inline double block_sum(double v, double* lds) {
  v = wave_sum(v);
  const int wave = threadIdx.x >> 6;
  if ((threadIdx.x & 63) == 0) lds[wave] = v;
  __syncthreads();
  double r = 0.0;
  if (threadIdx.x == 0)
    for (int i = 0; i < kBlock / 64; ++i) r += lds[i];
  __syncthreads();
  return r;
}

template <int N>
__device__ inline void block_sum_n(const double (&v)[N], double (&out)[N]) {
  __shared__ double red[N][kBlock / 64];
  const int wave = threadIdx.x >> 6;
#pragma unroll
  for (int o = 0; o < N; ++o) {
    const double w = wave_sum(v[o]);
    if ((threadIdx.x & 63) == 0) red[o][wave] = w;
  }
  __syncthreads();
#pragma unroll
  for (int o = 0; o < N; ++o) {
    double r = 0.0;
    if (threadIdx.x == 0)
      for (int i = 0; i < kBlock / 64; ++i) r += red[o][i];
    out[o] = r;
  }
  __syncthreads();
}

constexpr int kTicketDoubles = kReductionHeader;
constexpr int kTicketStride = 32;
static_assert(kReductionHeader * sizeof(double) >= 9 * kTicketStride * sizeof(unsigned), "ticket words");
template <int NOUT>
__device__ inline void grid_finish(const double (&r)[NOUT] , double* scratch, double* out_dev,
                                   double* out_host, double* lds, HostSignal sig = HostSignal(), unsigned slot = 0xffffffffu) {
  if (slot == 0xffffffffu) slot = blockIdx.x;
  __shared__ int is_last;
  unsigned* ticket = reinterpret_cast<unsigned*>(scratch);
  double* partials = scratch + kTicketDoubles;
  if (threadIdx.x == 0) {
#pragma unroll
    for (int o = 0; o < NOUT; ++o)
      __hip_atomic_store(&partials[(size_t)slot * NOUT + o], r[o], __ATOMIC_RELAXED, __HIP_MEMORY_SCOPE_AGENT);
    asm volatile("s_waitcnt vmcnt(0)" ::: "memory");
    const unsigned shard = blockIdx.x & 7u, nshards = gridDim.x < 8u ? gridDim.x : 8u;
    const unsigned in_shard = (gridDim.x - shard + 7u) / 8u;
    bool last = false;
    if (__hip_atomic_fetch_add(&ticket[kTicketStride * shard], 1u, __ATOMIC_RELAXED, __HIP_MEMORY_SCOPE_AGENT) == in_shard - 1) {
      __hip_atomic_store(&ticket[kTicketStride * shard], 0u, __ATOMIC_RELAXED, __HIP_MEMORY_SCOPE_AGENT);
      last = __hip_atomic_fetch_add(&ticket[kTicketStride * 8], 1u, __ATOMIC_RELAXED, __HIP_MEMORY_SCOPE_AGENT) == nshards - 1;
      if (last) __hip_atomic_store(&ticket[kTicketStride * 8], 0u, __ATOMIC_RELAXED, __HIP_MEMORY_SCOPE_AGENT);
    }
    is_last = last;
  }
  __syncthreads();
  if (!is_last) return;
  double acc[NOUT];
#pragma unroll
  for (int o = 0; o < NOUT; ++o) acc[o] = 0.0;
  for (int i0 = threadIdx.x; i0 < (int)gridDim.x; i0 += 4 * kBlock) {
    double v[4][NOUT];
#pragma unroll
    for (int u = 0; u < 4; ++u) {
      const int i = min(i0 + u * kBlock, (int)gridDim.x - 1);
#pragma unroll
      for (int o = 0; o < NOUT; ++o) v[u][o] = __hip_atomic_load(&partials[(size_t)i * NOUT + o], __ATOMIC_RELAXED, __HIP_MEMORY_SCOPE_AGENT);
    }
#pragma unroll
    for (int u = 0; u < 4; ++u)
#pragma unroll
      for (int o = 0; o < NOUT; ++o) acc[o] = (i0 + u * kBlock < (int)gridDim.x) ? acc[o] + v[u][o] : acc[o];
  }
  double tot[NOUT];
  block_sum_n<NOUT>(acc, tot);
  (void)lds;
  if (threadIdx.x == 0) {
#pragma unroll
    for (int o = 0; o < NOUT; ++o) {
      if (out_dev) out_dev[o] = tot[o];
      if (out_host) __hip_atomic_store(&out_host[o], tot[o], __ATOMIC_RELAXED, __HIP_MEMORY_SCOPE_SYSTEM);
    }
  }
  if (sig.seq_host && threadIdx.x == 0) {
    asm volatile("s_waitcnt vmcnt(0)" ::: "memory");
    const unsigned long long q = __hip_atomic_load(sig.seq_dev, __ATOMIC_RELAXED, __HIP_MEMORY_SCOPE_AGENT) + 1;
    __hip_atomic_store(sig.seq_dev, q, __ATOMIC_RELAXED, __HIP_MEMORY_SCOPE_AGENT);
    __hip_atomic_store(sig.seq_host, q, __ATOMIC_RELEASE, __HIP_MEMORY_SCOPE_SYSTEM);
  }
}
template <int NOUT, class Fn>
__device__ inline void grid_finish_fn(const double (&r)[NOUT] , double* scratch, double* lds, Fn&& fn) {
  __shared__ int is_last_fn;
  unsigned* ticket = reinterpret_cast<unsigned*>(scratch);
  double* partials = scratch + kTicketDoubles;
  if (threadIdx.x == 0) {
#pragma unroll
    for (int o = 0; o < NOUT; ++o)
      __hip_atomic_store(&partials[(size_t)blockIdx.x * NOUT + o], r[o], __ATOMIC_RELAXED, __HIP_MEMORY_SCOPE_AGENT);
    asm volatile("s_waitcnt vmcnt(0)" ::: "memory");
    const unsigned shard = blockIdx.x & 7u, nshards = gridDim.x < 8u ? gridDim.x : 8u;
    const unsigned in_shard = (gridDim.x - shard + 7u) / 8u;
    bool last = false;
    if (__hip_atomic_fetch_add(&ticket[kTicketStride * shard], 1u, __ATOMIC_RELAXED, __HIP_MEMORY_SCOPE_AGENT) == in_shard - 1) {
      __hip_atomic_store(&ticket[kTicketStride * shard], 0u, __ATOMIC_RELAXED, __HIP_MEMORY_SCOPE_AGENT);
      last = __hip_atomic_fetch_add(&ticket[kTicketStride * 8], 1u, __ATOMIC_RELAXED, __HIP_MEMORY_SCOPE_AGENT) == nshards - 1;
      if (last) __hip_atomic_store(&ticket[kTicketStride * 8], 0u, __ATOMIC_RELAXED, __HIP_MEMORY_SCOPE_AGENT);
    }
    is_last_fn = last;
  }
  __syncthreads();
  if (!is_last_fn) return;
  double tot[NOUT], acc[NOUT];
#pragma unroll
  for (int o = 0; o < NOUT; ++o) acc[o] = 0.0;
  for (int i0 = threadIdx.x; i0 < (int)gridDim.x; i0 += 4 * kBlock) {
    double v[4][NOUT];
#pragma unroll
    for (int u = 0; u < 4; ++u) {
      const int i = min(i0 + u * kBlock, (int)gridDim.x - 1);
#pragma unroll
      for (int o = 0; o < NOUT; ++o) v[u][o] = __hip_atomic_load(&partials[(size_t)i * NOUT + o], __ATOMIC_RELAXED, __HIP_MEMORY_SCOPE_AGENT);
    }
#pragma unroll
    for (int u = 0; u < 4; ++u)
#pragma unroll
      for (int o = 0; o < NOUT; ++o) acc[o] = (i0 + u * kBlock < (int)gridDim.x) ? acc[o] + v[u][o] : acc[o];
  }
// ... 8 lines not shown
```

### multigridbarriermpi.jl_amd/csrc/kernels.hip

```cpp
#include "kernels.hpp"
#include "kernels_tpl.hpp"

#include <algorithm>
#include <cmath>

namespace mgb {

namespace {


template <int G>
void spmv_launch(hipStream_t st, const DevCsr& A, const double* x, const double* y0, double* y) {
  const int grid = grid_for((long long)A.rows * G);
  hipLaunchKernelGGL((spmv_kernel_t<G, double>), dim3(grid), dim3(kBlock), 0, st, A.rows, A.rowptr, A.colidx, A.vals, x, y0, y);
}

template <int G>
__global__ __launch_bounds__(kBlock) void spmv_el_kernel(int rows, DevElCsr E, const int* __restrict__ rowptr,
                                                          const double* __restrict__ vals, const double* __restrict__ x,
                                                          const double* y0, double* y) {
  extern __shared__ double xs[];
  const int lane = threadIdx.x % G, grp = threadIdx.x / G;
  constexpr int GR = kBlock / G;
  const int rpe = E.rows_per_el;
  const int els = max(1, min(E.nel, (kBlock * 4) / rpe));
  const int npass = (E.nel + els - 1) / els;
  for (int ps = xcd_block(blockIdx.x, gridDim.x); ps < npass; ps += gridDim.x) {
    const int e0 = ps * els, ne = min(els, E.nel - e0);
    __syncthreads();
    for (int idx = threadIdx.x; idx < ne * E.cmax; idx += kBlock) xs[idx] = x[E.ecols[(long long)e0 * E.cmax + idx]];
    __syncthreads();
    const long long r0 = (long long)e0 * rpe;
    const int nrows = (int)min((long long)ne * rpe, (long long)rows - r0);
    for (int rr0 = grp; rr0 < nrows; rr0 += kSpmvU * GR) {
      int b[kSpmvU], e[kSpmvU];
      double acc[kSpmvU], base[kSpmvU];
#pragma unroll
      for (int u = 0; u < kSpmvU; ++u) {
        const int rr = rr0 + u * GR;
        const bool ok = rr < nrows;
        b[u] = ok ? rowptr[r0 + rr] : 0;
        e[u] = ok ? rowptr[r0 + rr + 1] : 0;
        base[u] = (ok && y0 && lane == 0) ? y0[r0 + rr] : 0.0;
      }
#pragma unroll
      for (int u = 0; u < kSpmvU; ++u) {
        const int rr = rr0 + u * GR;
        const double* xe = xs + (rr / rpe) * E.cmax;
        const int k = b[u] + lane;
        acc[u] = (k < e[u]) ? vals[k] * xe[E.lcol[k]] : 0.0;
        for (int kk = k + G; kk < e[u]; kk += G) acc[u] += vals[kk] * xe[E.lcol[kk]];
      }
#pragma unroll
      for (int u = 0; u < kSpmvU; ++u) {
        double a = acc[u];
#pragma unroll
        for (int o = G / 2; o > 0; o >>= 1) a += __shfl_down(a, o, G);
        const int rr = rr0 + u * GR;
        if (lane == 0 && rr < nrows) y[r0 + rr] = base[u] + a;
      }
    }
  }
}

template <int G>
void spmv_el_launch(hipStream_t st, const DevCsr& A, const DevElCsr& E, const double* x, const double* y0, double* y) {
  const int els = std::max(1, std::min(E.nel, (kBlock * 4) / E.rows_per_el));
  const int npass = (E.nel + els - 1) / els;
  const int grid = std::max(1, std::min(npass, kMaxBlocks * 4));
  hipLaunchKernelGGL(spmv_el_kernel<G>, dim3(grid), dim3(kBlock), (size_t)els * E.cmax * sizeof(double), st, A.rows, E, A.rowptr,
                     A.vals, x, y0, y);
}


using Cone = ConeT<double>;

__global__ __launch_bounds__(kBlock) void barrier_f0_kernel(int n, BarrierParams P, const double* __restrict__ Dz,
                                                             const double* __restrict__ w,
                                                             const double* __restrict__ c,
                                                             const double* __restrict__ phi_ref, double frac,
                                                             double* __restrict__ phi_out, double* scratch,
                                                             double* out_dev, double* out_host, HostSignal sig) {
  __shared__ double lds[kBlock / 64];
  double accF = 0.0, accL = 0.0;
  for (long long q = (long long)blockIdx.x * kBlock + threadIdx.x; q < n; q += (long long)gridDim.x * kBlock) {
    const double* dz = Dz + q * P.K;
    const double* cq = c + q * P.K;
    const double wq = w[q];
    double F = 0.0;
    for (int ci = 0; ci < P.ncones; ++ci) {
      if (!P.active(ci, q)) {
        if (phi_out) phi_out[q * P.ncones + ci] = INFINITY;
        continue;
      }
      const ConeAM<double> am = cone_am<double>(P, ci, q);
      Cone k = load_cone<double>(P.cone[ci], dz, am.a);
      if (phi_ref && !(k.phi >= frac * phi_ref[q * P.ncones + ci])) k.ok = false;
      if (phi_out) phi_out[q * P.ncones + ci] = k.phi;
      F += k.ok ? (-log(k.phi) - am.mu * log(k.s)) : INFINITY;
    }
    accF += wq * F;
    double lin = 0.0;
    for (int j = 0; j < P.K; ++j) lin += cq[j] * dz[j];
    accL += wq * lin;
  }
  const double r[2] = {block_sum(accF, lds), block_sum(accL, lds)};
  grid_finish<2>(r, scratch, out_dev, out_host, lds, sig);
}


constexpr int kTrialNodes = 64;
template <int G, int NA>
__global__ __launch_bounds__(kBlock) void trial_f0_kernel(int n, int N, BarrierParams P, const int* __restrict__ rowptr,
                                                           const int* __restrict__ colidx, const double* __restrict__ vals,
                                                           const double* __restrict__ s, const double* __restrict__ nstep,
                                                           TrialSet T, const double* __restrict__ Dz0,
                                                           const double* __restrict__ w, const double* __restrict__ c,
                                                           const double* __restrict__ phi_ref, double frac, double* scratch,
                                                           HostSignal sig) {
  __shared__ double lds[kBlock / 64];
  __shared__ double dzs[NA][kTrialNodes * kMaxK];
  constexpr int GR = kBlock / G;
  const int K = P.K, lane = threadIdx.x % G, grp = threadIdx.x / G;
#pragma unroll
  for (int a = 0; a < NA; ++a)
    if (T.s_out[a])
      for (long long i = (long long)blockIdx.x * kBlock + threadIdx.x; i < N; i += (long long)gridDim.x * kBlock)
        T.s_out[a][i] = s[i] + T.alpha[a] * nstep[i];
  auto xval = [&](int j, int a) { return nstep ? s[j] + T.alpha[a] * nstep[j] : s[j]; };
  double accF = 0.0, accL = 0.0;
  const int pa = threadIdx.x >> 6, pnode = threadIdx.x & 63;
  const int nchunks = (n + kTrialNodes - 1) / kTrialNodes;
  for (int ch = xcd_block(blockIdx.x, gridDim.x); ch < nchunks; ch += gridDim.x) {
    const int q0 = ch * kTrialNodes, nq = min(kTrialNodes, n - q0), nrows = nq * K;
    const long long r0 = (long long)q0 * K;
    for (int rr0 = grp; rr0 < nrows; rr0 += kSpmvU * GR) {
      int b[kSpmvU], e[kSpmvU], ci[kSpmvU];
      double acc[NA][kSpmvU], base[kSpmvU], va[kSpmvU];
#pragma unroll
      for (int u = 0; u < kSpmvU; ++u) {
        const int rr = rr0 + u * GR;
        const bool ok = rr < nrows;
        b[u] = ok ? rowptr[r0 + rr] : 0;
        e[u] = ok ? rowptr[r0 + rr + 1] : 0;
        base[u] = (ok && lane == 0) ? Dz0[r0 + rr] : 0.0;
      }
#pragma unroll
      for (int u = 0; u < kSpmvU; ++u) {
        const int k = b[u] + lane;
        const bool in = k < e[u];
        ci[u] = in ? colidx[k] : -1;
        va[u] = in ? vals[k] : 0.0;
      }
#pragma unroll
      for (int a = 0; a < NA; ++a)
#pragma unroll
        for (int u = 0; u < kSpmvU; ++u) acc[a][u] = (ci[u] >= 0) ? va[u] * xval(ci[u], a) : 0.0;
#pragma unroll
      for (int u = 0; u < kSpmvU; ++u)
        for (int k = b[u] + lane + G; k < e[u]; k += G) {
          const double vk = vals[k];
          const int ck = colidx[k];
#pragma unroll
          for (int a = 0; a < NA; ++a) acc[a][u] += vk * xval(ck, a);
        }
#pragma unroll
      for (int a = 0; a < NA; ++a)
#pragma unroll
        for (int u = 0; u < kSpmvU; ++u) {
          double t = acc[a][u];
#pragma unroll
          for (int o = G / 2; o > 0; o >>= 1) t += __shfl_down(t, o, G);
          const int rr = rr0 + u * GR;
          if (lane == 0 && rr < nrows) {
            const double v = base[u] + t;
            T.dz[a][r0 + rr] = v;
            dzs[a][rr] = v;
          }
        }
    }
    __syncthreads();
    if (pa < NA && pnode < nq) {
      const long long q = q0 + pnode;
      const double* dz = dzs[pa] + pnode * K;
      const double* cq = c + q * K;
      const double wq = w[q];
      double* phi_out = T.phi_out[pa];
      double F = 0.0;
      for (int ci2 = 0; ci2 < P.ncones; ++ci2) {
        if (!P.active(ci2, q)) {
          if (phi_out) phi_out[q * P.ncones + ci2] = INFINITY;
          continue;
        }
        const ConeAM<double> am = cone_am<double>(P, ci2, q);
        Cone k = load_cone<double>(P.cone[ci2], dz, am.a);
        if (phi_ref && !(k.phi >= frac * phi_ref[q * P.ncones + ci2])) k.ok = false;
        if (phi_out) phi_out[q * P.ncones + ci2] = k.phi;
        F += k.ok ? (-log(k.phi) - am.mu * log(k.s)) : INFINITY;
      }
      accF += wq * F;
      double lin = 0.0;
      for (int j = 0; j < K; ++j) lin += cq[j] * dz[j];
      accL += wq * lin;
    }
    __syncthreads();
  }
  double r[2 * NA], mine[2 * NA];
#pragma unroll
  for (int a = 0; a < NA; ++a) {
    mine[2 * a] = pa == a ? accF : 0.0;
    mine[2 * a + 1] = pa == a ? accL : 0.0;
  }
  block_sum_n<2 * NA>(mine, r);
  grid_finish<2 * NA>(r, scratch, T.out_dev, T.out_host, lds, sig, xcd_block(blockIdx.x, gridDim.x));
}

inline int trial_grid(int n) {
  const int b = (n + kTrialNodes - 1) / kTrialNodes;
  return b < 1 ? 1 : (b > kMaxBlocks ? kMaxBlocks : b);
}

template <int G>
void trial_launch(hipStream_t st, const DevCsr& B, int n, const BarrierParams& P, const double* s, const double* nstep,
                  const TrialSet& T, const double* Dz0, const double* w, const double* c, const double* phi_ref, double frac,
                  double* scratch, HostSignal sig) {
#define MGB_TRIAL_NA(NA)                                                                                                    \
  hipLaunchKernelGGL((trial_f0_kernel<G, NA>), dim3(trial_grid(n)), dim3(kBlock), 0, st, n, B.cols, P, B.rowptr, B.colidx,   \
                     B.vals, s, nstep, T, Dz0, w, c, phi_ref, frac, scratch, sig)
  switch (T.na) {
    case 1: MGB_TRIAL_NA(1); break;
    case 2: MGB_TRIAL_NA(2); break;
    default: MGB_TRIAL_NA(3); break;
  }
#undef MGB_TRIAL_NA
}

__global__ __launch_bounds__(kBlock) void barrier_rows_F_kernel(int n, BarrierParams P, const double* __restrict__ Dz,
                                                                 double* __restrict__ out) {
  for (long long q = (long long)blockIdx.x * kBlock + threadIdx.x; q < n; q += (long long)gridDim.x * kBlock) {
    const double* dz = Dz + q * P.K;
    double F = 0.0;
    for (int ci = 0; ci < P.ncones; ++ci) {
      if (!P.active(ci, q)) continue;
      const ConeAM<double> am = cone_am<double>(P, ci, q);
      Cone k = load_cone<double>(P.cone[ci], dz, am.a);
      F += k.ok ? (-log(k.phi) - am.mu * log(k.s)) : INFINITY;
    }
    out[q] = F;
  }
}

__global__ __launch_bounds__(kBlock) void expand_hessian_rows_kernel(int n, BarrierParams P, const double* __restrict__ Y,
                                                                      double* __restrict__ out) {
  const int K = P.K, nY = P.nY();
  for (long long q = (long long)blockIdx.x * kBlock + threadIdx.x; q < n; q += (long long)gridDim.x * kBlock) {
    double* o = out + q * K * K;
    for (int e = 0; e < K * K; ++e) o[e] = 0.0;
    const double* yq = Y + q * nY;
    int slot = 0;
    for (int ci = 0; ci < P.ncones; ++ci) {
      const ConeSpec& S = P.cone[ci];
      const int nact = S.nact();
      for (int a = 0; a < nact; ++a)
        for (int b = a; b < nact; ++b, ++slot) {
          const int ra = S.col(a), rb = S.col(b);
          o[ra * K + rb] += yq[slot];
          if (ra != rb) o[rb * K + ra] += yq[slot];
        }
    }
  }
}

__global__ __launch_bounds__(kBlock) void waxpby_kernel(int n, const double* __restrict__ x, double alpha,
                                                         const double* __restrict__ y, double* out) {
  for (long long i = (long long)blockIdx.x * kBlock + threadIdx.x; i < n; i += (long long)gridDim.x * kBlock)
    out[i] = x[i] + alpha * y[i];
}

__global__ __launch_bounds__(kBlock) void mul_kernel(int n, const double* __restrict__ x, const double* __restrict__ y,
                                                      double* out) {
  for (long long i = (long long)blockIdx.x * kBlock + threadIdx.x; i < n; i += (long long)gridDim.x * kBlock)
    out[i] = x[i] * y[i];
}

__global__ __launch_bounds__(kBlock) void col_extract_kernel(int n, int K, int k, const double* __restrict__ M,
// ... 34 lines not shown
__global__ __launch_bounds__(kBlock) void gather_top_kernel(int ntop, const int* __restrict__ top, const double* __restrict__ g,
                                                             double* __restrict__ buf) {
  for (long long i = (long long)blockIdx.x * kBlock + threadIdx.x; i < ntop; i += (long long)gridDim.x * kBlock) buf[i] = g[top[i]];
}

__global__ __launch_bounds__(kBlock) void scatter_top_norm_kernel(int ntop, const int* __restrict__ top, const double* __restrict__ buf,
                                                                   double* __restrict__ g, double* out) {
  __shared__ double lds[kBlock / 64];
  double acc = 0.0;
  for (int i = threadIdx.x; i < ntop; i += kBlock) {
    const double v = buf[i];
    g[top[i]] = v;
    acc += v * v;
  }
  const double tot = block_sum(acc, lds);
  if (threadIdx.x == 0) out[0] = buf[ntop] + tot;
}

__global__ void flag_to_double_kernel(const int* flag_dev, double* out) {
  if (threadIdx.x == 0 && blockIdx.x == 0) out[0] = *flag_dev != 0 ? 1.0 : 0.0;
}

__global__ __launch_bounds__(kBlock) void sum_kernel(int n, const double* __restrict__ x, double* scratch, double* out_dev,
                                                      double* out_host) {
  __shared__ double lds[kBlock / 64];
  double acc = 0.0;
  for (long long i = (long long)blockIdx.x * kBlock + threadIdx.x; i < n; i += (long long)gridDim.x * kBlock) acc += x[i];
  const double r[1] = {block_sum(acc, lds)};
  grid_finish<1>(r, scratch, out_dev, out_host, lds);
}

__global__ __launch_bounds__(kBlock) void isfinite_kernel(int n, const double* __restrict__ x, int* flag) {
  int bad = 0;
  for (long long i = (long long)blockIdx.x * kBlock + threadIdx.x; i < n; i += (long long)gridDim.x * kBlock)
    bad |= !isfinite(x[i]);
  if (__any(bad) && (threadIdx.x & 63) == 0) atomicAnd(flag, 0);
}

}

void launch_spmv(hipStream_t st, const DevCsr& A, const double* x, const double* y0, double* y) {
  if (A.rows == 0) return;
  switch (A.group) {
    case 1: spmv_launch<1>(st, A, x, y0, y); break;
    case 2: spmv_launch<2>(st, A, x, y0, y); break;
    case 4: spmv_launch<4>(st, A, x, y0, y); break;
    case 8: spmv_launch<8>(st, A, x, y0, y); break;
    case 16: spmv_launch<16>(st, A, x, y0, y); break;
    case 32: spmv_launch<32>(st, A, x, y0, y); break;
    default: spmv_launch<64>(st, A, x, y0, y); break;
  }
}

void launch_spmv_el(hipStream_t st, const DevCsr& A, const DevElCsr& E, const double* x, const double* y0, double* y) {
  if (A.rows == 0) return;
  switch (A.group) {
    case 1: spmv_el_launch<1>(st, A, E, x, y0, y); break;
    case 2: spmv_el_launch<2>(st, A, E, x, y0, y); break;
    case 4: spmv_el_launch<4>(st, A, E, x, y0, y); break;
    case 8: spmv_el_launch<8>(st, A, E, x, y0, y); break;
    case 16: spmv_el_launch<16>(st, A, E, x, y0, y); break;
    case 32: spmv_el_launch<32>(st, A, E, x, y0, y); break;
    default: spmv_el_launch<64>(st, A, E, x, y0, y); break;
  }
}

void launch_waxpby(hipStream_t st, int n, const double* x, double alpha, const double* y, double* out) {
  if (n == 0) return;
  hipLaunchKernelGGL(waxpby_kernel, dim3(grid_for(n)), dim3(kBlock), 0, st, n, x, alpha, y, out);
}

int f0_blocks(int n) { return std::max(grid_for(n), trial_grid(n)); }

void launch_trial_set(hipStream_t st, const DevCsr& B, int n, BarrierParams P, const double* s, const double* nstep,
                      const TrialSet& T, const double* Dz0, const double* w, const double* c, const double* phi_ref, double frac,
                      double* scratch, HostSignal sig) {
#define MGB_TRIAL(G) trial_launch<G>(st, B, n, P, s, nstep, T, Dz0, w, c, phi_ref, frac, scratch, sig)
  switch (B.group) {
    case 1: MGB_TRIAL(1); break;
    case 2: MGB_TRIAL(2); break;
    case 4: MGB_TRIAL(4); break;
    case 8: MGB_TRIAL(8); break;
    case 16: MGB_TRIAL(16); break;
    case 32: MGB_TRIAL(32); break;
    default: MGB_TRIAL(64); break;
  }
#undef MGB_TRIAL
}

void launch_trial_f0(hipStream_t st, const DevCsr& B, int n, BarrierParams P, const double* s, double alpha,
                     const double* nstep, double* s_out, const double* Dz0, double* Dz, const double* w, const double* c,
                     const double* phi_ref, double frac, double* phi_out, double* scratch, double* out2, double* out2_host,
                     HostSignal sig) {
  TrialSet T;
  T.na = 1;
  T.alpha[0] = alpha;
  T.s_out[0] = s_out;
  T.dz[0] = Dz;
  T.phi_out[0] = phi_out;
  T.out_dev = out2;
  T.out_host = out2_host;
  launch_trial_set(st, B, n, P, s, nstep, T, Dz0, w, c, phi_ref, frac, scratch, sig);
}

void launch_barrier_f0(hipStream_t st, int n, BarrierParams P, const double* Dz, const double* w, const double* c,
                       const double* phi_ref, double frac, double* phi_out, double* scratch, double* out2, double* out2_host,
                       HostSignal sig) {
  hipLaunchKernelGGL(barrier_f0_kernel, dim3(grid_for(n)), dim3(kBlock), 0, st, n, P, Dz, w, c, phi_ref, frac, phi_out, scratch,
                     out2, out2_host, sig);
}

void launch_barrier_f1(hipStream_t st, int n, BarrierParams P, const double* Dz, const double* w, const double* c,
                       double t, double* v) {
  hipLaunchKernelGGL(barrier_f1_kernel_t<double>, dim3(grid_for(n)), dim3(kBlock), 0, st, n, P, Dz, w, c, t, v);
}

void launch_barrier_f2(hipStream_t st, int n, BarrierParams P, const double* Dz, const double* w, double* Y) {
  hipLaunchKernelGGL(barrier_f2_kernel_t<double>, dim3(grid_for(n)), dim3(kBlock), 0, st, n, P, Dz, w, Y);
}

void launch_barrier_rows_F(hipStream_t st, int n, BarrierParams P, const double* Dz, double* out) {
  if (n == 0) return;
  hipLaunchKernelGGL(barrier_rows_F_kernel, dim3(grid_for(n)), dim3(kBlock), 0, st, n, P, Dz, out);
}

void launch_expand_hessian_rows(hipStream_t st, int n, BarrierParams P, const double* Y, double* out) {
  if (n == 0) return;
  hipLaunchKernelGGL(expand_hessian_rows_kernel, dim3(grid_for(n)), dim3(kBlock), 0, st, n, P, Y, out);
}

void launch_dot(hipStream_t st, int n, const double* x, const double* y, double* scratch, double* out, double* out_host,
                int* flag_dev, int* flag_host, HostSignal sig) {
  hipLaunchKernelGGL(dot_kernel, dim3(grid_for(n)), dim3(kBlock), 0, st, n, x, y, scratch, out, out_host, flag_dev, flag_host, sig);
}

void launch_dot_owned(hipStream_t st, int n, const double* x, const double* y, const int* kind, int count_top, double* scratch,
                      double* out) {
  hipLaunchKernelGGL(dot_owned_kernel, dim3(grid_for(n)), dim3(kBlock), 0, st, n, x, y, kind, count_top, scratch, out);
}

void launch_gather_top(hipStream_t st, int ntop, const int* top, const double* g, double* buf) {
  if (ntop > 0) hipLaunchKernelGGL(gather_top_kernel, dim3(grid_for(ntop)), dim3(kBlock), 0, st, ntop, top, g, buf);
}

void launch_scatter_top_norm(hipStream_t st, int ntop, const int* top, const double* buf, double* g, double* out) {
  hipLaunchKernelGGL(scatter_top_norm_kernel, dim3(1), dim3(kBlock), 0, st, ntop, top, buf, g, out);
}

void launch_flag_to_double(hipStream_t st, const int* flag_dev, double* out) {
  hipLaunchKernelGGL(flag_to_double_kernel, dim3(1), dim3(64), 0, st, flag_dev, out);
}

void launch_sum(hipStream_t st, int n, const double* x, double* scratch, double* out, double* out_host) {
  hipLaunchKernelGGL(sum_kernel, dim3(grid_for(n)), dim3(kBlock), 0, st, n, x, scratch, out, out_host);
}

void launch_all_isfinite(hipStream_t st, int n, const double* x, int* flag) {
  (void)hipMemsetAsync(flag, 0xFF, sizeof(int), st);
  if (n == 0) return;
  hipLaunchKernelGGL(isfinite_kernel, dim3(grid_for(n)), dim3(kBlock), 0, st, n, x, flag);
}

void launch_mul(hipStream_t st, int n, const double* x, const double* y, double* out) {
  if (n == 0) return;
  hipLaunchKernelGGL(mul_kernel, dim3(grid_for(n)), dim3(kBlock), 0, st, n, x, y, out);
}

void launch_col_extract(hipStream_t st, int n, int K, int k, const double* M, double* out) {
  if (n == 0) return;
  hipLaunchKernelGGL(col_extract_kernel, dim3(grid_for(n)), dim3(kBlock), 0, st, n, K, k, M, out);
}

}
// ... 1 lines not shown
```

### multigridbarriermpi.jl_amd/csrc/kernels.hpp

```cpp
#pragma once
#include <hip/hip_runtime.h>

namespace mgb {

struct DevCsr {
  int rows = 0, cols = 0, nnz = 0, group = 1;
  int* rowptr = nullptr;
  int* colidx = nullptr;
  double* vals = nullptr;
};

struct DevElCsr {
  int rows_per_el = 0, cmax = 0, nel = 0;
  const int* ecols = nullptr;
  const unsigned char* lcol = nullptr;
  bool valid() const { return nel > 0; }
};

struct ConeSpec {
  int kind = 0;
  int nq = 0;
  int iq[3] = {0, 0, 0};
  int is = 0;
  int is2 = -1;
  double a = 2.0;
  double mu = 1.0;
  double coef[3] = {0.0, 0.0, 0.0};
  double off = 0.0;
  __host__ __device__ int nact() const { return kind == 1 ? nq : nq + 1 + (is2 >= 0 ? 1 : 0); }
  __host__ __device__ int nY() const { return nact() * (nact() + 1) / 2; }
  __host__ __device__ int col(int a) const { return a < nq ? iq[a] : (a == nq ? is : is2); }
};

constexpr int kMaxCones = 3;
struct BarrierParams {
  int K = 0;
  int ncones = 1;
  ConeSpec cone[kMaxCones];
  const double* a_node = nullptr;
  const double* mu_node = nullptr;
  const unsigned char* term_mask = nullptr;
  __host__ __device__ bool active(int ci, long long q) const { return !term_mask || term_mask[q * ncones + ci]; }
  __host__ __device__ int nY() const {
    int s = 0;
    for (int c = 0; c < ncones; ++c) s += cone[c].nY();
    return s;
  }
};

void launch_spmv(hipStream_t st, const DevCsr& A, const double* x, const double* y0, double* y);
void launch_spmv_el(hipStream_t st, const DevCsr& A, const DevElCsr& E, const double* x, const double* y0, double* y);
void launch_spmv_f32(hipStream_t st, const DevCsr& A, const float* vals, const float* x, const float* y0, float* y);
void launch_barrier_f0_rows_f32(hipStream_t st, int n, BarrierParams P, const float* Dz, const float* w, const float* c,
                                double* outF, double* outC);
void launch_barrier_f1_f32(hipStream_t st, int n, BarrierParams P, const float* Dz, const float* w, const float* c, float t, float* v);
void launch_barrier_f2_f32(hipStream_t st, int n, BarrierParams P, const float* Dz, const float* w, float* Y);
void launch_to_f32(hipStream_t st, long long n, const double* in, float* out);
void launch_spmv_tpl_f64(hipStream_t st, const DevCsr& A, const double* x, const double* y0, double* y);
void launch_barrier_f1_tpl_f64(hipStream_t st, int n, BarrierParams P, const double* Dz, const double* w, const double* c, double t,
                               double* v);
void launch_barrier_f2_tpl_f64(hipStream_t st, int n, BarrierParams P, const double* Dz, const double* w, double* Y);
void launch_waxpby(hipStream_t st, int n, const double* x, double alpha, const double* y, double* out);
constexpr int kReductionHeader = 144;
struct HostSignal {
  unsigned long long* seq_dev = nullptr;
  unsigned long long* seq_host = nullptr;
};
int f0_blocks(int n);
void launch_barrier_f0(hipStream_t st, int n, BarrierParams P, const double* Dz, const double* w, const double* c,
                       const double* phi_ref, double frac, double* phi_out, double* scratch, double* out2,
                       double* out2_host = nullptr, HostSignal sig = HostSignal());
void launch_trial_f0(hipStream_t st, const DevCsr& B, int n, BarrierParams P, const double* s, double alpha,
                     const double* nstep, double* s_out, const double* Dz0, double* Dz, const double* w, const double* c,
                     const double* phi_ref, double frac, double* phi_out, double* scratch, double* out2,
                     double* out2_host = nullptr, HostSignal sig = HostSignal());
struct TrialSet {
  int na = 0;
  double alpha[3] = {0.0, 0.0, 0.0};
  double* s_out[3] = {nullptr, nullptr, nullptr};
  double* dz[3] = {nullptr, nullptr, nullptr};
  double* phi_out[3] = {nullptr, nullptr, nullptr};
  double* out_dev = nullptr;
  double* out_host = nullptr;
};
void launch_trial_set(hipStream_t st, const DevCsr& B, int n, BarrierParams P, const double* s, const double* nstep,
                      const TrialSet& T, const double* Dz0, const double* w, const double* c, const double* phi_ref, double frac,
                      double* scratch, HostSignal sig = HostSignal());
void launch_barrier_f1(hipStream_t st, int n, BarrierParams P, const double* Dz, const double* w, const double* c,
                       double t, double* v);
void launch_barrier_f2(hipStream_t st, int n, BarrierParams P, const double* Dz, const double* w, double* Y);
void launch_barrier_rows_F(hipStream_t st, int n, BarrierParams P, const double* Dz, double* out);
void launch_expand_hessian_rows(hipStream_t st, int n, BarrierParams P, const double* Y, double* out);
void launch_dot(hipStream_t st, int n, const double* x, const double* y, double* scratch, double* out, double* out_host = nullptr,
                int* flag_dev = nullptr, int* flag_host = nullptr, HostSignal sig = HostSignal());
void launch_dot_owned(hipStream_t st, int n, const double* x, const double* y, const int* kind, int count_top, double* scratch,
                      double* out);
void launch_gather_top(hipStream_t st, int ntop, const int* top, const double* g, double* buf);
void launch_scatter_top_norm(hipStream_t st, int ntop, const int* top, const double* buf, double* g, double* out);
void launch_flag_to_double(hipStream_t st, const int* flag_dev, double* out);
void launch_sum(hipStream_t st, int n, const double* x, double* scratch, double* out, double* out_host = nullptr);
void launch_all_isfinite(hipStream_t st, int n, const double* x, int* flag);
void launch_mul(hipStream_t st, int n, const double* x, const double* y, double* out);
void launch_col_extract(hipStream_t st, int n, int K, int k, const double* M, double* out);

}
```

### multigridbarriermpi.jl_amd/csrc/kernels_tpl.hpp

```cpp
#pragma once
#include "devutil.hpp"

namespace mgb {
namespace {

constexpr int kMaxK = 8;

constexpr int kSpmvU = 2;
template <int G, class T>
__global__ __launch_bounds__(kBlock) void spmv_kernel_t(int rows, const int* __restrict__ rowptr, const int* __restrict__ colidx,
                                                         const T* __restrict__ vals, const T* __restrict__ x, const T* y0, T* y) {
  const int lane = threadIdx.x % G;
  const long long stride = (long long)gridDim.x * (kBlock / G);
  for (long long row0 = (long long)xcd_block(blockIdx.x, gridDim.x) * (kBlock / G) + threadIdx.x / G; row0 < rows;
       row0 += kSpmvU * stride) {
    int b[kSpmvU], e[kSpmvU];
    T acc[kSpmvU], base[kSpmvU];
#pragma unroll
    for (int u = 0; u < kSpmvU; ++u) {
      const long long row = row0 + u * stride;
      const bool ok = row < rows;
      b[u] = ok ? rowptr[row] : 0;
      e[u] = ok ? rowptr[row + 1] : 0;
      base[u] = (ok && y0 && lane == 0) ? y0[row] : T(0);
// ... 57 lines not shown
    T phi = T(P.off);
#pragma unroll
    for (int i = 0; i < 3; ++i) {
      c.q[i] = (i < P.nq) ? dz[P.iq[i]] : T(0);
      phi += (i < P.nq) ? T(P.coef[i]) * c.q[i] : T(0);
    }
    c.s = T(1);
    c.sa = T(1);
    c.phi = phi;
    c.ok = phi > T(0);
    return c;
  }
  T qq = T(0);
#pragma unroll
  for (int i = 0; i < 3; ++i) {
    c.q[i] = (i < P.nq) ? dz[P.iq[i]] : T(0);
    qq += c.q[i] * c.q[i];
  }
  c.s = dz[P.is] + (P.is2 >= 0 ? dz[P.is2] : T(0));
  c.ok = c.s > T(0);
  c.sa = c.ok ? pow_a<T>(c.s, a) : T(-1);
  c.phi = c.sa - qq;
  c.ok = c.ok && (c.phi > T(0));
  return c;
}

template <class T>
__device__ inline T pick3(const T (&q)[3], int i) {
  return i == 0 ? q[0] : (i == 1 ? q[1] : q[2]);
}

template <class T>
__global__ __launch_bounds__(kBlock) void barrier_f0_rows_kernel_t(int n, BarrierParams P, const T* __restrict__ Dz,
                                                                    const T* __restrict__ w, const T* __restrict__ c,
                                                                    double* __restrict__ outF, double* __restrict__ outC) {
  for (long long q = (long long)blockIdx.x * kBlock + threadIdx.x; q < n; q += (long long)gridDim.x * kBlock) {
    const T* dz = Dz + q * P.K;
    T F = T(0);
    for (int ci = 0; ci < P.ncones; ++ci) {
      if (!P.active(ci, q)) continue;
      const ConeAM<T> am = cone_am<T>(P, ci, q);
      const ConeT<T> k = load_cone<T>(P.cone[ci], dz, am.a);
      F += k.ok ? (-log(k.phi) - am.mu * log(k.s)) : T(INFINITY);
    }
    T cd = T(0);
#pragma unroll
    for (int j = 0; j < kMaxK; ++j) cd += (j < P.K) ? c[q * P.K + j] * dz[j] : T(0);
    outF[q] = (double)(w[q] * F);
    outC[q] = (double)(w[q] * cd);
  }
}

template <class T>
__global__ __launch_bounds__(kBlock) void barrier_f1_kernel_t(int n, BarrierParams P, const T* __restrict__ Dz,
                                                               const T* __restrict__ w, const T* __restrict__ c, T t,
                                                               T* __restrict__ v) {
  for (long long q = (long long)blockIdx.x * kBlock + threadIdx.x; q < n; q += (long long)gridDim.x * kBlock) {
    const T* dz = Dz + q * P.K;
    const T* cq = c + q * P.K;
    const T wq = w[q];
    T vr[kMaxK];
#pragma unroll
    for (int j = 0; j < kMaxK; ++j) vr[j] = (j < P.K) ? wq * (t * cq[j]) : T(0);
    for (int ci = 0; ci < P.ncones; ++ci) {
      const ConeSpec& S = P.cone[ci];
      if (!P.active(ci, q)) continue;
      const ConeAM<T> am = cone_am<T>(P, ci, q);
      const ConeT<T> k = load_cone<T>(S, dz, am.a);
      if (S.kind == 1) {
#pragma unroll
        for (int j = 0; j < kMaxK; ++j) {
          T add = T(0);
#pragma unroll
          for (int i = 0; i < 3; ++i) add += (i < S.nq && S.iq[i] == j) ? -wq * (T(S.coef[i]) / k.phi) : T(0);
          vr[j] += add;
        }
        continue;
      }
      const T ds = am.a * pow_a<T>(k.s, am.a - T(1));
      const T gs = wq * (-ds / k.phi - am.mu / k.s);
#pragma unroll
      for (int j = 0; j < kMaxK; ++j) {
        T add = T(0);
#pragma unroll
        for (int i = 0; i < 3; ++i) add += (i < S.nq && S.iq[i] == j) ? wq * (T(2) * k.q[i] / k.phi) : T(0);
        add += (S.is == j) ? gs : T(0);
        add += (S.is2 == j) ? gs : T(0);
        vr[j] += add;
      }
    }
    T* vq = v + q * P.K;
#pragma unroll
    for (int j = 0; j < kMaxK; ++j)
      if (j < P.K) vq[j] = vr[j];
  }
}

template <class T>
__global__ __launch_bounds__(kBlock) void barrier_f2_kernel_t(int n, BarrierParams P, const T* __restrict__ Dz,
                                                               const T* __restrict__ w, T* __restrict__ Y) {
  const int nY = P.nY();
  for (long long q = (long long)blockIdx.x * kBlock + threadIdx.x; q < n; q += (long long)gridDim.x * kBlock) {
    const T* dz = Dz + q * P.K;
    T* yq = Y + q * nY;
    const T wq = w[q];
    int slot = 0;
    for (int ci = 0; ci < P.ncones; ++ci) {
      const ConeSpec& S = P.cone[ci];
      if (!P.active(ci, q)) {
        const int ns = S.nY();
        for (int i = 0; i < ns; ++i) yq[slot++] = T(0);
        continue;
      }
      const ConeAM<T> am = cone_am<T>(P, ci, q);
      const ConeT<T> k = load_cone<T>(S, dz, am.a);
      if (S.kind == 1) {
        const T ip2l = T(1) / (k.phi * k.phi);
#pragma unroll
        for (int i = 0; i < 3; ++i)
#pragma unroll
          for (int j = 0; j < 3; ++j)
            if (i < S.nq && j >= i && j < S.nq) yq[slot++] = wq * (T(S.coef[i]) * T(S.coef[j]) * ip2l);
        continue;
      }
      const T a = am.a;
      const T ds = a * pow_a<T>(k.s, a - T(1));
      const T dds = (a == T(1)) ? T(0) : a * (a - T(1)) * pow_a<T>(k.s, a - T(2));
      const T ip = T(1) / k.phi, ip2 = ip * ip;
      const T hss = -dds * ip + ds * ds * ip2 + am.mu / (k.s * k.s);
      const int nq = S.nq, nact = S.nact();
#pragma unroll
      for (int i = 0; i < 5; ++i)
#pragma unroll
        for (int j = 0; j < 5; ++j) {
          if (i < nact && j >= i && j < nact) {
            const int ai = min(i, nq), aj = min(j, nq);
            T h;
            if (aj < nq) h = T(4) * pick3<T>(k.q, ai) * pick3<T>(k.q, aj) * ip2 + (ai == aj ? T(2) * ip : T(0));
            else if (ai < nq) h = T(-2) * pick3<T>(k.q, ai) * ds * ip2;
            else h = hss;
            yq[slot++] = wq * h;
          }
        }
    }
  }
}


}
}
```

Before: 88.59 million DoF/s per Newton step.

## Fuse barrier f1/f2 kernels, ride dots on spmv/trials, batch line-search trials

Adds a fused barrier_f12 kernel that writes both the gradient contribution and the Hessian values in one pass over Dz. It folds the g·nstep dot into the restriction SpMV and into the speculative trial-set kernel, and adds a fourth speculative step point. Line-search follow-up evaluations are batched so several trial steps are computed in one launch. These paths sit behind environment flags and aim to cut kernel launches and host syncs per Newton step, at the cost of extra buffers, more complex graph keys and possibly wasted speculative work.

```diff
diff --git a/include/mgb_hip.h b/include/mgb_hip.h
--- a/include/mgb_hip.h
+++ b/include/mgb_hip.h
@@ -119,6 +119,8 @@
 int mgb_amg_set_early_stop(mgb_amg a, int col);
 int mgb_amg_sol_info(mgb_amg a, int* nt, double* t_elapsed, double* time_factor, long long* counts4);
 int mgb_amg_sol_get(mgb_amg a, long long* its , double* ts, double* c_dot_Dz);
+int mgb_amg_probe_step_dots(mgb_amg a, int level, const double* g, const double* nstep, const double* v, double* out4, double* g2);
+int mgb_amg_sol_linesearch(mgb_amg a, long long* followups, long long* step_graphs);
 int mgb_amg_sol_kernels(mgb_amg a, double* ms11, double* bytes11, long long* launches11);
 int mgb_amg_time_kernels(mgb_amg a, int level, int reps, int nrot, double* ms8, double* bytes8);
 
diff --git a/multigridbarriermpi.jl_amd/__init__.py b/multigridbarriermpi.jl_amd/__init__.py
--- a/multigridbarriermpi.jl_amd/__init__.py
+++ b/multigridbarriermpi.jl_amd/__init__.py
@@ -994,8 +994,11 @@
         pc = (C.c_longlong * 4)()
         tp = C.c_double()
         call("mgb_amg_sol_pcg", self.handle, pc, C.byref(tp))
+        nfu, nsg = C.c_longlong(), C.c_longlong()
+        call("mgb_amg_sol_linesearch", self.handle, C.byref(nfu), C.byref(nsg))
         return dict(t_elapsed=te.value, ts=ts, its=its.reshape(nt.value, self.L).T.copy(), c_dot_Dz=cd,
                     time_factor=tf.value, n_f0=counts[0], n_f1=counts[1], n_f2=counts[2], n_factor=counts[3],
+                    n_followup=nfu.value, n_step_graphs=nsg.value,
                     kernels=kernels, pcg=dict(solves=pc[0], iterations=pc[1], fallbacks=pc[2], gave_up_at=pc[3], seconds=tp.value))
 
     KERNEL_NAMES = ("apply_D", "barrier_f2", "hessian_assemble", "barrier_f1", "restrict", "barrier_f0",
diff --git a/multigridbarriermpi.jl_amd/_lib.py b/multigridbarriermpi.jl_amd/_lib.py
--- a/multigridbarriermpi.jl_amd/_lib.py
+++ b/multigridbarriermpi.jl_amd/_lib.py
@@ -122,6 +122,8 @@
     "mgb_amg_solve": [H, C.c_double, C.c_double, C.c_double, C.c_int, C.c_int, C.c_int],
     "mgb_amg_sol_info": [H, c_int_p, c_dbl_p, c_dbl_p, c_ll_p],
     "mgb_amg_sol_get": [H, c_ll_p, c_dbl_p, c_dbl_p],
+    "mgb_amg_sol_linesearch": [H, c_ll_p, c_ll_p],
+    "mgb_amg_probe_step_dots": [H, C.c_int, c_dbl_p, c_dbl_p, c_dbl_p, c_dbl_p, c_dbl_p],
     "mgb_amg_sol_kernels": [H, c_dbl_p, c_dbl_p, c_ll_p],
     "mgb_amg_time_kernels": [H, C.c_int, C.c_int, C.c_int, c_dbl_p, c_dbl_p],
     "mgb_plan_create": [H, C.c_int, c_str_arr, C.c_int, c_str_arr, C.c_int, c_int_p, C.c_int, C.c_int,
diff --git a/multigridbarriermpi.jl_amd/csrc/amg.cpp b/multigridbarriermpi.jl_amd/csrc/amg.cpp
--- a/multigridbarriermpi.jl_amd/csrc/amg.cpp
+++ b/multigridbarriermpi.jl_amd/csrc/amg.cpp
@@ -1,7 +1,9 @@
 #include "amg.hpp"
 
 
+#include <algorithm>
 #include <chrono>
+#include <functional>
 #include <cmath>
 #include <thread>
 #include <string>
@@ -415,6 +417,10 @@
     : ctx_(ctx), n_(g.n), S_((int)spec.state_variables.size()), P_(P), spec_(spec) {
   hip_check(hipSetDevice(ctx_.device), "hipSetDevice");
   if (const char* e = std::getenv("MGB_FUSED_TRIAL_ROWS")) fused_trial_rows_ = std::atoi(e);
+  if (const char* e = std::getenv("MGB_STEP_FUSE_DOTS")) fuse_dots_ = std::atoi(e) != 0;
+  if (const char* e = std::getenv("MGB_LS_BATCH")) ls_batch_ = std::atoi(e) != 0;
+  if (const char* e = std::getenv("MGB_STEP_FUSE_F12")) fuse_f12_ = std::atoi(e) != 0;
+  if (const char* e = std::getenv("MGB_SPEC_POINTS")) spec_points_ = std::atoi(e) == 3 ? 3 : 4;
   if (P.K != (int)spec.D.size()) throw ArgError("amg: barrier K != number of D rows");
   if (P.ncones < 1 || P.ncones > kMaxCones) throw ArgError("amg: barrier supports 1 to 3 terms");
   if (P.K > 8) throw ArgError("amg: the barrier kernels support at most 8 rows of D");
@@ -448,15 +454,17 @@
   DzA_.alloc((size_t)n_ * K);
   DzB_.alloc((size_t)n_ * K);
   DzC_.alloc((size_t)n_ * K);
+  DzD_.alloc((size_t)n_ * K);
   v_.alloc((size_t)n_ * K);
   Y_.alloc((size_t)n_ * nY);
   phi_cur_.alloc((size_t)n_ * P.ncones);
   phi_trial_.alloc((size_t)n_ * P.ncones);
   phi_trial2_.alloc((size_t)n_ * P.ncones);
   phi_trial3_.alloc((size_t)n_ * P.ncones);
+  phi_trial4_.alloc((size_t)n_ * P.ncones);
   h_flag_.alloc(4);
-  scal_.alloc(12);
-  h_scal_.alloc(12);
+  scal_.alloc(14);
+  h_scal_.alloc(14);
   seq_dev_.alloc(1);
   hip_check(hipMemset(seq_dev_.p, 0, sizeof(unsigned long long)), "memset seq");
   h_seq_.alloc(1);
@@ -485,7 +493,7 @@
 }
 
 size_t reduction_scratch_doubles(int n_local, int max_level_unknowns) {
-  return (size_t)6 * std::max(f0_blocks(n_local), f0_blocks(max_level_unknowns)) + 8 + kReductionHeader;
+  return (size_t)9 * std::max(f0_blocks(n_local), f0_blocks(max_level_unknowns)) + 8 + kReductionHeader;
 }
 
 int Amg::level_index(const Level& lv) const {
@@ -535,6 +543,7 @@
   lv.s_trial.alloc(N);
   lv.s_trial2.alloc(N);
   lv.s_trial3.alloc(N);
+  lv.s_trial4.alloc(N);
   lv.g_trial.alloc(N);
   lv.g.alloc(N);
   lv.nstep.alloc(N);
@@ -847,10 +856,12 @@
   return lv.gchol.values_local();
 }
 
-void Amg::enqueue_f2_assemble(Level& lv, const double* dz, SolveStats& st) {
-  timer_.begin(ctx_.stream, KC_F2, (double)n_ * (P_.K + 1 + P_.nY()) * 8);
-  launch_barrier_f2(ctx_.stream, n_, P_, dz, w_.p, Y_.p);
-  timer_.end(ctx_.stream);
+void Amg::enqueue_f2_assemble(Level& lv, const double* dz, SolveStats& st, bool have_Y) {
+  if (!have_Y) {
+    timer_.begin(ctx_.stream, KC_F2, (double)n_ * (P_.K + 1 + P_.nY()) * 8);
+    launch_barrier_f2(ctx_.stream, n_, P_, dz, w_.p, Y_.p);
+    timer_.end(ctx_.stream);
+  }
   if (pcg_) {
     mg_values(level_index(lv));
     st.n_f2++;
@@ -864,13 +875,19 @@
 }
 
 double Amg::dev_f1(Level& lv, const double* dz, double t, double* g_out, SolveStats* st, const double** pre) {
-  timer_.begin(ctx_.stream, KC_F1, (double)n_ * (3 * P_.K + 1) * 8);
-  launch_barrier_f1(ctx_.stream, n_, P_, dz, w_.p, c_.p, t, v_.p);
+  const bool with_f2 = fuse_f12_ && pre && st && !host_solve_ && !pcg_ && ctx_.world == 1;
+  const bool with_dot = fuse_dots_ && ctx_.world == 1 && spmv_dot_fits(lv.plan.N);
+  timer_.begin(ctx_.stream, KC_F1, (double)n_ * (3 * P_.K + 1 + (with_f2 ? P_.nY() : 0)) * 8);
+  if (with_f2) launch_barrier_f12(ctx_.stream, n_, P_, dz, w_.p, c_.p, t, v_.p, Y_.p);
+  else launch_barrier_f1(ctx_.stream, n_, P_, dz, w_.p, c_.p, t, v_.p);
   timer_.end(ctx_.stream);
   timer_.begin(ctx_.stream, KC_RESTRICT, csr_bytes(lv.BT.view, false));
-  launch_spmv(ctx_.stream, lv.BT.view, v_.p, nullptr, g_out);
+  if (with_dot)
+    launch_spmv_dot(ctx_.stream, lv.BT.view, v_.p, g_out, partials_.p, scal_.p + 2, host_scal(scal_.p + 2), next_signal());
+  else launch_spmv(ctx_.stream, lv.BT.view, v_.p, nullptr, g_out);
   timer_.end(ctx_.stream);
-  if (owner_local(lv)) {
+  if (with_dot) {
+  } else if (owner_local(lv)) {
     const int ntop = lv.gchol.ntop_unknowns();
     if (gtop_.n < (size_t)ntop + 1) gtop_.alloc((size_t)ntop + 1);
     launch_gather_top(ctx_.stream, ntop, lv.gchol.top_unknowns(), g_out, gtop_.p);
@@ -892,7 +909,7 @@
       if (!ev_f1_) hip_check(hipEventCreateWithFlags(&ev_f1_, hipEventDisableTiming), "event");
       hip_check(hipEventRecord(ev_f1_, ctx_.stream), "record f1");
     }
-    enqueue_f2_assemble(lv, dz, *st);
+    enqueue_f2_assemble(lv, dz, *st, with_f2);
     *pre = dz;
     if (ctx_.world == 1) wait_signal("sync f1");
     else hip_check(hipEventSynchronize(ev_f1_), "sync f1 event");
@@ -910,26 +927,41 @@
   T.step = step;
 }
 
-static const double kSpecSteps[3] = {1.0, kBeta, kBeta * kBeta};
-
-void Amg::enqueue_spec_trials(Level& lv, Trial* spec, HostSignal sig) {
+static const double kSpecSteps[4] = {1.0, kBeta, kBeta * kBeta, kBeta * kBeta * kBeta};
+
+void Amg::enqueue_trial_set(Level& lv, Trial* const* pts, int na, HostSignal sig, bool ride_dot) {
+  TrialSet T;
+  T.na = na;
+  for (int q = 0; q < na; ++q) {
+    T.alpha[q] = -pts[q]->step;
+    T.s_out[q] = pts[q]->s;
+    T.dz[q] = pts[q]->dz;
+    T.phi_out[q] = pts[q]->phi;
+  }
+  T.out_dev = scal_.p + 4;
+  T.out_host = host_scal(scal_.p + 4);
+  if (ride_dot) {
+    T.dot_x = lv.g.p;
+    T.dot_y = lv.nstep.p;
+    T.dot_n = lv.plan.N;
+    T.flag_dev = lv.gchol.fail_flag();
+    T.flag_host = h_flag_.p;
+  }
+  timer_.begin(ctx_.stream, KC_F0, trial_bytes(lv, true) + (na - 1.0) * n_ * (P_.K + P_.ncones) * 8 + (ride_dot ? 8.0 * lv.plan.N : 0.0));
+  launch_trial_set(ctx_.stream, lv.B.view, n_, P_, lv.s.p, lv.nstep.p, T, Dz0_.p, w_.p, c_.p, phi_cur_.p, kFracToBoundary,
+                   partials_.p, sig);
+  timer_.end(ctx_.stream);
+}
+
+void Amg::enqueue_spec_trials(Level& lv, Trial* spec, HostSignal sig, bool ride_dot) {
   const int ns = spec_count();
-  if (ns == 3) {
-    TrialSet T;
-    T.na = 3;
-    for (int q = 0; q < 3; ++q) {
-      T.alpha[q] = -kSpecSteps[q];
-      T.s_out[q] = spec[q].s;
-      T.dz[q] = spec[q].dz;
-      T.phi_out[q] = spec[q].phi;
+  if (ns >= 3) {
+    Trial* pts[kMaxTrialPoints];
+    for (int q = 0; q < ns; ++q) {
+      pts[q] = &spec[q];
       spec[q].step = kSpecSteps[q];
     }
-    T.out_dev = scal_.p + 4;
-    T.out_host = host_scal(scal_.p + 4);
-    timer_.begin(ctx_.stream, KC_F0, trial_bytes(lv, true) + 2.0 * n_ * (P_.K + P_.ncones) * 8);
-    launch_trial_set(ctx_.stream, lv.B.view, n_, P_, lv.s.p, lv.nstep.p, T, Dz0_.p, w_.p, c_.p, phi_cur_.p, kFracToBoundary,
-                     partials_.p, sig);
-    timer_.end(ctx_.stream);
+    enqueue_trial_set(lv, pts, ns, sig, ride_dot);
   } else {
     enqueue_trial(lv, spec[0], kSpecSteps[0], 0);
     enqueue_trial(lv, spec[1], kSpecSteps[1], 1, sig);
@@ -937,10 +969,12 @@
 }
 
 void Amg::launch_step_graph(Level& lv, Trial* spec) {
-  const void* key[15] = {lv.avals.p, lv.g.p, lv.nstep.p, lv.s.p, spec[0].s, spec[0].phi, spec[0].dz, spec[1].s, spec[1].phi,
-                         spec[1].dz, spec[2].s,  spec[2].phi, spec[2].dz, phi_cur_.p, Dz0_.p};
+  const bool four = spec_count() == 4;
+  const void* key[18] = {lv.avals.p, lv.g.p, lv.nstep.p, lv.s.p, spec[0].s, spec[0].phi, spec[0].dz, spec[1].s, spec[1].phi,
+                         spec[1].dz, spec[2].s,  spec[2].phi, spec[2].dz, four ? spec[3].s : nullptr, four ? spec[3].phi : nullptr,
+                         four ? spec[3].dz : nullptr, phi_cur_.p, Dz0_.p};
   for (const auto& g : lv.step_graphs)
-    if (std::equal(key, key + 15, g.key)) {
+    if (std::equal(key, key + 18, g.key)) {
       hip_check(hipGraphLaunch(g.exec, ctx_.stream), "hipGraphLaunch");
       ++seq_expected_;
       for (int q = 0; q < spec_count(); ++q) spec[q].step = kSpecSteps[q];
@@ -950,12 +984,14 @@
   hip_check(hipStreamBeginCapture(ctx_.stream, hipStreamCaptureModeThreadLocal), "hipStreamBeginCapture");
   try {
     lv.gchol.enqueue_chain(ctx_.stream, lv.avals.p, lv.g.p, lv.nstep.p);
-    launch_dot(ctx_.stream, lv.plan.N, lv.g.p, lv.nstep.p, partials_.p, scal_.p + 3, host_scal(scal_.p + 3), lv.gchol.fail_flag(),
-               h_flag_.p);
+    const bool ride_dot = fuse_dots_ && spec_count() >= 3 && trial_dot_fits(n_, lv.plan.N);
+    if (!ride_dot)
+      launch_dot(ctx_.stream, lv.plan.N, lv.g.p, lv.nstep.p, partials_.p, scal_.p + 3, host_scal(scal_.p + 3), lv.gchol.fail_flag(),
+                 h_flag_.p);
     HostSignal sig;
     sig.seq_dev = seq_dev_.p;
     sig.seq_host = h_seq_.p;
-    enqueue_spec_trials(lv, spec, sig);
+    enqueue_spec_trials(lv, spec, sig, ride_dot);
   } catch (...) {
     (void)hipStreamEndCapture(ctx_.stream, &graph);
     if (graph) (void)hipGraphDestroy(graph);
@@ -963,7 +999,7 @@
   }
   hip_check(hipStreamEndCapture(ctx_.stream, &graph), "hipStreamEndCapture");
   Level::StepGraph sg{};
-  std::copy(key, key + 15, sg.key);
+  std::copy(key, key + 18, sg.key);
   hipError_t e = hipGraphInstantiate(&sg.exec, graph, nullptr, nullptr, 0);
   (void)hipGraphDestroy(graph);
   hip_check(e, "hipGraphInstantiate");
@@ -1039,7 +1075,7 @@
       if (time_chain) hip_check(hipEventRecord(e1, ctx_.stream), "record");
       if (olocal) {
         launch_dot_owned(ctx_.stream, N, lv.g.p, lv.nstep.p, lv.gchol.unknown_kind(), ctx_.rank == 0, partials_.p, scal_.p + 3);
-        launch_flag_to_double(ctx_.stream, lv.gchol.fail_flag(), scal_.p + 10);
+        launch_flag_to_double(ctx_.stream, lv.gchol.fail_flag(), scal_.p + 12);
       } else if (flag_rides) {
         launch_dot(ctx_.stream, N, lv.g.p, lv.nstep.p, partials_.p, scal_.p + 3, host_scal(scal_.p + 3), lv.gchol.fail_flag(),
                    h_flag_.p, spec ? HostSignal() : next_signal());
@@ -1054,15 +1090,15 @@
         st.n_f0 += spec_count();
       }
       if (olocal) {
-        if (!spec) hip_check(hipMemsetAsync(scal_.p + 4, 0, 6 * sizeof(double), ctx_.stream), "zero trial slots");
-        ctx_.allreduce_sum(scal_.p + 3, 8);
-        hip_check(hipMemcpyAsync(h_scal_.p + 3, scal_.p + 3, 8 * sizeof(double), hipMemcpyDeviceToHost, ctx_.stream), "D2H inc + trials + flag");
+        if (!spec) hip_check(hipMemsetAsync(scal_.p + 4, 0, 8 * sizeof(double), ctx_.stream), "zero trial slots");
+        ctx_.allreduce_sum(scal_.p + 3, 10);
+        hip_check(hipMemcpyAsync(h_scal_.p + 3, scal_.p + 3, 10 * sizeof(double), hipMemcpyDeviceToHost, ctx_.stream), "D2H inc + trials + flag");
       } else if (ctx_.world > 1)
         hip_check(hipMemcpyAsync(h_scal_.p + 3, scal_.p + 3, (spec ? 1 + 2 * spec_count() : 1) * sizeof(double),
                                  hipMemcpyDeviceToHost, ctx_.stream), "D2H inc + trials");
     }
     wait_signal("sync solve");
-    if (owner_local(lv)) h_flag_.p[0] = h_scal_.p[10] != 0.0 ? 1 : 0;
+    if (owner_local(lv)) h_flag_.p[0] = h_scal_.p[12] != 0.0 ? 1 : 0;
     if (spec)
       for (int q = 0; q < spec_count(); ++q) {
         spec[q].y = h_scal_.p[4 + 2 * q] + t * h_scal_.p[5 + 2 * q];
@@ -1147,7 +1183,11 @@
   st.n_f1++;
   double ymin = y, gmin = gnorm, incmin = INFINITY;
   const double theta = finest ? 0.1 : 0.5;
-  Trial T[3];
+  const int nb = spec_points_;
+  Trial T[kMaxTrialPoints];
+  T[3].s = lv.s_trial4.p;
+  T[3].phi = phi_trial4_.p;
+  T[3].dz = DzD_.p;
   T[0].s = lv.s_trial.p;
   T[0].phi = phi_trial_.p;
   T[1].s = lv.s_trial2.p;
@@ -1159,13 +1199,35 @@
   T[2].dz = DzC_.p;
   auto eval = [&](int pos, double step) {
     if (!(T[pos].valid && T[pos].step == step))
-      for (int q = 0; q < 3; ++q)
+      for (int q = 0; q < nb; ++q)
         if (q != pos && T[q].valid && T[q].step == step) {
           std::swap(T[pos], T[q]);
           break;
         }
     Trial& X = T[pos];
     if (X.valid && X.step == step) return X.y;
+    st.n_followup++;
+    if (ls_batch_ && ctx_.world == 1 && n_ <= fused_trial_rows_) {
+      Trial* pts[kMaxTrialPoints] = {&X};
+      int na = 1;
+      X.step = step;
+      double next = step * kBeta;
+      for (int q = 0; q < nb && next >= kMinStep; ++q) {
+        if (q == pos || (pos == 1 && q == 0) || (T[q].valid && T[q].step < step)) continue;
+        T[q].step = next;
+        T[q].valid = false;
+        pts[na++] = &T[q];
+        next *= kBeta;
+      }
+      enqueue_trial_set(lv, pts, na, next_signal(), false);
+      st.n_f0 += na;
+      wait_signal("sync f0 batch");
+      for (int a = 0; a < na; ++a) {
+        pts[a]->y = h_scal_.p[4 + 2 * a] + t * h_scal_.p[5 + 2 * a];
+        pts[a]->valid = true;
+      }
+      return X.y;
+    }
     X.y = dev_f0(lv, lv.s.p, t, nullptr, phi_cur_.p, X.phi, X.dz, -step, lv.nstep.p, X.s);
     st.n_f0++;
     X.step = step;
@@ -1177,7 +1239,8 @@
   while (res.k < maxit && !res.converged) {
     res.k++;
     double inc = 0;
-    T[0].valid = T[1].valid = T[2].valid = false;
+    T[0].valid = T[1].valid = T[2].valid = T[3].valid = false;
+    std::sort(T, T + nb, [](const Trial& a, const Trial& b) { return std::less<const double*>()(a.s, b.s); });
     const double* have = pre;
     pre = nullptr;
     if (!dev_f2_solve(lv, Dz_.p, t, st, &inc, speculate ? T : nullptr, have)) {
@@ -1239,12 +1302,15 @@
   lv.s_trial.p = T[0].s;
   lv.s_trial2.p = T[1].s;
   lv.s_trial3.p = T[2].s;
+  lv.s_trial4.p = T[3].s;
   phi_trial_.p = T[0].phi;
   phi_trial2_.p = T[1].phi;
   phi_trial3_.p = T[2].phi;
+  phi_trial4_.p = T[3].phi;
   DzA_.p = T[0].dz;
   DzB_.p = T[1].dz;
   DzC_.p = T[2].dz;
+  DzD_.p = T[3].dz;
   return res;
 }
 
@@ -1379,9 +1445,54 @@
   }
   hip_check(hipStreamSynchronize(ctx_.stream), "sync");
   st.t_elapsed = now_s() - t_begin;
+  for (auto& lv : levels_) st.n_step_graphs += (long long)lv->step_graphs.size();
   if (going(t) && !stopped) throw NumericError("amgb: convergence failure (kappa collapsed)");
 }
 
+
+void Amg::probe_step_dots(int l, const double* g_host, const double* n_host, const double* v_host, double* out4, double* g2_host) {
+  if (ctx_.world != 1) throw ArgError("probe_step_dots: single-GPU contexts only");
+  Level& lv = level(l);
+  const int N = lv.plan.N;
+  resync_signals();
+  ensure_chol(lv);
+  lv.g.upload(g_host, N);
+  lv.nstep.upload(n_host, N);
+  v_.upload(v_host, (size_t)n_ * P_.K);
+  hip_check(hipMemsetAsync(lv.s.p, 0, (size_t)N * sizeof(double), ctx_.stream), "memset s");
+  const double nan = std::nan("");
+  out4[1] = out4[3] = nan;
+  launch_dot(ctx_.stream, N, lv.g.p, lv.nstep.p, partials_.p, scal_.p + 3, host_scal(scal_.p + 3), nullptr, nullptr, next_signal());
+  wait_signal("probe dot");
+  out4[0] = h_scal_.p[3];
+  if (spec_count() >= 3 && trial_dot_fits(n_, N)) {
+    h_scal_.p[3] = nan;
+    Trial T[kMaxTrialPoints];
+    double* sb[4] = {lv.s_trial.p, lv.s_trial2.p, lv.s_trial3.p, lv.s_trial4.p};
+    double* pb[4] = {phi_trial_.p, phi_trial2_.p, phi_trial3_.p, phi_trial4_.p};
+    double* db[4] = {DzA_.p, DzB_.p, DzC_.p, DzD_.p};
+    for (int q = 0; q < 4; ++q) {
+      T[q].s = sb[q];
+      T[q].phi = pb[q];
+      T[q].dz = db[q];
+    }
+    enqueue_spec_trials(lv, T, next_signal(), true);
+    wait_signal("probe trial dot");
+    out4[1] = h_scal_.p[3];
+  }
+  launch_spmv(ctx_.stream, lv.BT.view, v_.p, nullptr, lv.g_trial.p);
+  launch_dot(ctx_.stream, N, lv.g_trial.p, lv.g_trial.p, partials_.p, scal_.p + 2, host_scal(scal_.p + 2), nullptr, nullptr, next_signal());
+  wait_signal("probe gg");
+  out4[2] = h_scal_.p[2];
+  lv.g_trial.download(g2_host, N);
+  if (spmv_dot_fits(N)) {
+    h_scal_.p[2] = nan;
+    launch_spmv_dot(ctx_.stream, lv.BT.view, v_.p, lv.g.p, partials_.p, scal_.p + 2, host_scal(scal_.p + 2), next_signal());
+    wait_signal("probe spmv dot");
+    out4[3] = h_scal_.p[2];
+    lv.g.download(g2_host + N, N);
+  }
+}
 
 double Amg::f0(int l, const double* s_host, double t, double* parts) {
   Level& lv = level(l);
diff --git a/multigridbarriermpi.jl_amd/csrc/amg.hpp b/multigridbarriermpi.jl_amd/csrc/amg.hpp
--- a/multigridbarriermpi.jl_amd/csrc/amg.hpp
+++ b/multigridbarriermpi.jl_amd/csrc/amg.hpp
@@ -191,6 +191,8 @@
   double t_elapsed = 0, t_setup = 0;
   double time_factor = 0, time_device = 0;
   long long n_factor = 0, n_f0 = 0, n_f1 = 0, n_f2 = 0;
+  long long n_followup = 0;
+  long long n_step_graphs = 0;
   long long pcg_solves = 0, pcg_iters = 0, pcg_fallbacks = 0;
   long long pcg_gaveup_at = -1;
   double time_pcg = 0;
@@ -259,6 +261,7 @@
   bool solve_host(int l, const double* avals, const double* g, double* nstep);
   bool solve_device(int l, const double* avals, const double* g, double* nstep);
 
+  void probe_step_dots(int l, const double* g_host, const double* n_host, const double* v_host, double* out4, double* g2_host);
   void solve(const SolveOptions& opt, SolveStats& st);
 
   struct KernelTimes {
@@ -273,7 +276,7 @@
     DevElAsmOwned elasm;
     bool flag_armed = false;
     struct StepGraph {
-      const void* key[15];
+      const void* key[18];
       hipGraphExec_t exec;
     };
     std::vector<StepGraph> step_graphs;
@@ -291,7 +294,7 @@
     bool f32_built = false;
     MfChol chol;
     GpuChol gchol;
-    DevBuf<double> s, s_trial, s_trial2, s_trial3, g, g_trial, nstep, avals;
+    DevBuf<double> s, s_trial, s_trial2, s_trial3, s_trial4, g, g_trial, nstep, avals;
     PinnedBuf<double> h_avals, h_g, h_n, h_s;
     struct Mg {
       bool elop_tried = false, assembled = false, transfer = false, vectors = false;
@@ -322,10 +325,14 @@
                 double* dz, double alpha = 0.0, const double* nstep = nullptr, double* s_out = nullptr);
   double trial_bytes(const Level& lv, bool with_ref) const;
   int fused_trial_rows_ = 64 * 2048;
+  bool fuse_dots_ = true;
+  bool ls_batch_ = true;
+  bool fuse_f12_ = true;
+  int spec_points_ = 4;
   void enqueue_f0(Level& lv, const double* s_dev, double alpha, const double* nstep, double* s_out, double* dz,
                   const double* phi_ref, double* phi_out, double* out2, HostSignal sig = HostSignal());
   double dev_f1(Level& lv, const double* dz, double t, double* g_out, SolveStats* st = nullptr, const double** pre = nullptr);
-  void enqueue_f2_assemble(Level& lv, const double* dz, SolveStats& st);
+  void enqueue_f2_assemble(Level& lv, const double* dz, SolveStats& st, bool have_Y = false);
   bool values_stay_local(Level& lv);
   bool owner_local(Level& lv) { return in_solve_ && values_stay_local(lv); }
   bool in_solve_ = false;
@@ -347,8 +354,9 @@
   bool dev_f2_solve(Level& lv, const double* dz, double t, SolveStats& st, double* inc, Trial* spec = nullptr,
                     const double* pre_assembled = nullptr);
   void enqueue_trial(Level& lv, Trial& T, double step, int slot, HostSignal sig = HostSignal());
-  int spec_count() const { return n_ <= fused_trial_rows_ ? 3 : 2; }
-  void enqueue_spec_trials(Level& lv, Trial* spec, HostSignal sig);
+  int spec_count() const { return n_ <= fused_trial_rows_ ? spec_points_ : 2; }
+  void enqueue_spec_trials(Level& lv, Trial* spec, HostSignal sig, bool ride_dot = false);
+  void enqueue_trial_set(Level& lv, Trial* const* pts, int na, HostSignal sig, bool ride_dot);
   void launch_step_graph(Level& lv, Trial* spec);
   NewtonResult newton(int l, double t, bool finest, bool final, double lam_tol, int maxit, SolveStats& st, int verbose);
   bool amgb_step(double t, bool final, double lam_tol, int max_newton, std::vector<long long>& its, SolveStats& st, int verbose);
@@ -410,8 +418,8 @@
   Csr dstack_host_;
   DevCsrOwned Dstack_;
   std::vector<std::unique_ptr<Level>> levels_;
-  DevBuf<double> w_, c_, z_, z_save_, Dz0_, Dz0_save_, Dz_, DzA_, DzB_, DzC_, v_, Y_, partials_, scal_, phi_cur_, phi_trial_, phi_trial2_,
-      phi_trial3_;
+  DevBuf<double> w_, c_, z_, z_save_, Dz0_, Dz0_save_, Dz_, DzA_, DzB_, DzC_, DzD_, v_, Y_, partials_, scal_, phi_cur_, phi_trial_, phi_trial2_,
+      phi_trial3_, phi_trial4_;
   PinnedBuf<int> h_flag_;
   bool host_solve_ = false;
   PinnedBuf<double> h_scal_;
diff --git a/multigridbarriermpi.jl_amd/csrc/capi.cpp b/multigridbarriermpi.jl_amd/csrc/capi.cpp
--- a/multigridbarriermpi.jl_amd/csrc/capi.cpp
+++ b/multigridbarriermpi.jl_amd/csrc/capi.cpp
@@ -582,8 +582,10 @@
                          const int* idx_s2, const double* p, const double* coef, const double* off, int n, mgb_vec Dz,
                          mgb_vec out) {
   return guard([&] {
-    need(Dz && out && n >= 0 && K >= 1 && K <= 8 && which >= 0 && which <= 2, "map_rows_barrier: bad arguments");
+    need(Dz && out && n >= 0 && K >= 1 && K <= 8 && which >= 0 && which <= 4, "map_rows_barrier: bad arguments");
     BarrierParams P = make_params_terms(K, nterms, kind, nq, idx_q, idx_s, idx_s2, p, coef, off);
+    const bool both = which >= 3;
+    if (both) which -= 2;
     const long long want = which == 0 ? n : (which == 1 ? (long long)n * K : (long long)n * K * K);
     need((long long)n * K == Dz->n && out->n == want, "map_rows_barrier: shape mismatch");
     hipStream_t st = Dz->ctx->ctx.stream;
@@ -594,7 +596,16 @@
       std::vector<double> ones((size_t)std::max(n, 1), 1.0);
       DevBuf<double> w;
       w.upload(ones.data(), ones.size());
-      if (which == 1) {
+      if (both) {
+        DevBuf<double> c, Y, v;
+        c.alloc((size_t)std::max(n, 1) * K);
+        Y.alloc((size_t)std::max(n, 1) * P.nY());
+        if (which == 2) v.alloc((size_t)std::max(n, 1) * K);
+        hip_check(hipMemsetAsync(c.p, 0, c.n * sizeof(double), st), "memset");
+        if (n) launch_barrier_f12(st, n, P, Dz->buf.p, w.p, c.p, 0.0, which == 1 ? out->buf.p : v.p, Y.p);
+        if (which == 2) launch_expand_hessian_rows(st, n, P, Y.p, out->buf.p);
+        hip_check(hipStreamSynchronize(st), "sync");
+      } else if (which == 1) {
         DevBuf<double> c;
         c.alloc((size_t)std::max(n, 1) * K);
         hip_check(hipMemsetAsync(c.p, 0, c.n * sizeof(double), st), "memset");
@@ -1029,6 +1040,19 @@
       counts4[2] = a->stats.n_f2;
       counts4[3] = a->stats.n_factor;
     }
+  });
+}
+int mgb_amg_probe_step_dots(mgb_amg a, int level, const double* g, const double* nstep, const double* v, double* out4, double* g2) {
+  return guard([&] {
+    need(a && g && nstep && v && out4 && g2 && level >= 0 && level < a->amg->L(), "probe_step_dots: bad arguments");
+    a->amg->probe_step_dots(level, g, nstep, v, out4, g2);
+  });
+}
+int mgb_amg_sol_linesearch(mgb_amg a, long long* followups, long long* step_graphs) {
+  return guard([&] {
+    need(a, "null amg");
+    if (followups) *followups = a->stats.n_followup;
+    if (step_graphs) *step_graphs = a->stats.n_step_graphs;
   });
 }
 int mgb_amg_sol_get(mgb_amg a, long long* its, double* ts, double* c_dot_Dz) {
diff --git a/multigridbarriermpi.jl_amd/csrc/devutil.hpp b/multigridbarriermpi.jl_amd/csrc/devutil.hpp
--- a/multigridbarriermpi.jl_amd/csrc/devutil.hpp
+++ b/multigridbarriermpi.jl_amd/csrc/devutil.hpp
@@ -40,14 +40,14 @@
   return r;
 }
 
-template <int N>
+template <int N, int BLOCK = kBlock>
 __device__ inline void block_sum_n(const double (&v)[N], double (&out)[N]) {
   __shared__ double red[N][kBlock / 64];
   const int wave = threadIdx.x >> 6;
 #pragma unroll
   for (int o = 0; o < N; ++o) {
     const double w = wave_sum(v[o]);
-    if ((threadIdx.x & 63) == 0) red[o][wave] = w;
+    if ((threadIdx.x & 63) == 0 && (BLOCK == kBlock || wave < kBlock / 64)) red[o][wave] = w;
   }
   __syncthreads();
 #pragma unroll
@@ -63,7 +63,7 @@
 constexpr int kTicketDoubles = kReductionHeader;
 constexpr int kTicketStride = 32;
 static_assert(kReductionHeader * sizeof(double) >= 9 * kTicketStride * sizeof(unsigned), "ticket words");
-template <int NOUT>
+template <int NOUT, int BLOCK = kBlock>
 __device__ inline void grid_finish(const double (&r)[NOUT] , double* scratch, double* out_dev,
                                    double* out_host, double* lds, HostSignal sig = HostSignal(), unsigned slot = 0xffffffffu) {
   if (slot == 0xffffffffu) slot = blockIdx.x;
@@ -90,7 +90,8 @@
   double acc[NOUT];
 #pragma unroll
   for (int o = 0; o < NOUT; ++o) acc[o] = 0.0;
-  for (int i0 = threadIdx.x; i0 < (int)gridDim.x; i0 += 4 * kBlock) {
+  const int first = (BLOCK == kBlock || threadIdx.x < kBlock) ? (int)threadIdx.x : (int)gridDim.x;
+  for (int i0 = first; i0 < (int)gridDim.x; i0 += 4 * kBlock) {
     double v[4][NOUT];
 #pragma unroll
     for (int u = 0; u < 4; ++u) {
@@ -104,7 +105,7 @@
       for (int o = 0; o < NOUT; ++o) acc[o] = (i0 + u * kBlock < (int)gridDim.x) ? acc[o] + v[u][o] : acc[o];
   }
   double tot[NOUT];
-  block_sum_n<NOUT>(acc, tot);
+  block_sum_n<NOUT, BLOCK>(acc, tot);
   (void)lds;
   if (threadIdx.x == 0) {
 #pragma unroll
diff --git a/multigridbarriermpi.jl_amd/csrc/kernels.hip b/multigridbarriermpi.jl_amd/csrc/kernels.hip
--- a/multigridbarriermpi.jl_amd/csrc/kernels.hip
+++ b/multigridbarriermpi.jl_amd/csrc/kernels.hip
@@ -13,6 +13,75 @@
 void spmv_launch(hipStream_t st, const DevCsr& A, const double* x, const double* y0, double* y) {
   const int grid = grid_for((long long)A.rows * G);
   hipLaunchKernelGGL((spmv_kernel_t<G, double>), dim3(grid), dim3(kBlock), 0, st, A.rows, A.rowptr, A.colidx, A.vals, x, y0, y);
+}
+
+constexpr int kSpmvDotBlock = 1024;
+template <int G>
+__global__ __launch_bounds__(kSpmvDotBlock) void spmv_dot_kernel(int rows, const int* __restrict__ rowptr,
+                                                                  const int* __restrict__ colidx, const double* __restrict__ vals,
+                                                                  const double* __restrict__ x, double* __restrict__ y,
+                                                                  double* scratch, double* out_dev, double* out_host,
+                                                                  HostSignal sig) {
+  __shared__ double ys[kBlock];
+  __shared__ double lds[kBlock / 64];
+  constexpr int RP = (kSpmvDotBlock / G < kBlock) ? kSpmvDotBlock / G : kBlock;
+  constexpr int NP = kBlock / RP, U = NP < 4 ? NP : 4;
+  const unsigned blk = xcd_block(blockIdx.x, gridDim.x);
+  const long long r0 = (long long)blk * kBlock;
+  const int lane = threadIdx.x % G, grp = threadIdx.x / G;
+  for (int p0 = 0; p0 < NP; p0 += U) {
+    int b[U], e[U], ci[U];
+    double acc[U], va[U];
+#pragma unroll
+    for (int u = 0; u < U; ++u) {
+      const long long row = r0 + (p0 + u) * RP + grp;
+      const bool ok = grp < RP && row < rows;
+      b[u] = ok ? rowptr[row] : 0;
+      e[u] = ok ? rowptr[row + 1] : 0;
+    }
+#pragma unroll
+    for (int u = 0; u < U; ++u) {
+      const int k = b[u] + lane;
+      const bool in = k < e[u];
+      ci[u] = in ? colidx[k] : -1;
+      va[u] = in ? vals[k] : 0.0;
+    }
+#pragma unroll
+    for (int u = 0; u < U; ++u) acc[u] = (ci[u] >= 0) ? va[u] * x[ci[u]] : 0.0;
+#pragma unroll
+    for (int u = 0; u < U; ++u)
+      for (int k = b[u] + lane + G; k < e[u]; k += G) acc[u] += vals[k] * x[colidx[k]];
+#pragma unroll
+    for (int u = 0; u < U; ++u) {
+      double a = acc[u];
+#pragma unroll
+      for (int o = G / 2; o > 0; o >>= 1) a += __shfl_down(a, o, G);
+      const int lr = (p0 + u) * RP + grp;
+      if (lane == 0 && grp < RP && r0 + lr < rows) {
+        const double v = 0.0 + a;
+        y[r0 + lr] = v;
+        ys[lr] = v;
+      }
+    }
+  }
+  __syncthreads();
+  double sq = 0.0;
+  if (threadIdx.x < kBlock && r0 + threadIdx.x < rows) sq += ys[threadIdx.x] * ys[threadIdx.x];
+  sq = wave_sum(sq);
+  if ((threadIdx.x & 63) == 0 && threadIdx.x < kBlock) lds[threadIdx.x >> 6] = sq;
+  __syncthreads();
+  double r[1] = {0.0};
+  if (threadIdx.x == 0)
+    for (int i = 0; i < kBlock / 64; ++i) r[0] += lds[i];
+  __syncthreads();
+  grid_finish<1, kSpmvDotBlock>(r, scratch, out_dev, out_host, lds, sig, blk);
+}
+
+template <int G>
+void spmv_dot_launch(hipStream_t st, const DevCsr& A, const double* x, double* y, double* scratch, double* out, double* out_host,
+                     HostSignal sig) {
+  hipLaunchKernelGGL(spmv_dot_kernel<G>, dim3(grid_for(A.rows)), dim3(kSpmvDotBlock), 0, st, A.rows, A.rowptr, A.colidx, A.vals, x, y,
+                     scratch, out, out_host, sig);
 }
 
 template <int G>
@@ -110,7 +179,7 @@
 
 
 constexpr int kTrialNodes = 64;
-template <int G, int NA>
+template <int G, int NA, bool DOT>
 __global__ __launch_bounds__(kBlock) void trial_f0_kernel(int n, int N, BarrierParams P, const int* __restrict__ rowptr,
                                                            const int* __restrict__ colidx, const double* __restrict__ vals,
                                                            const double* __restrict__ s, const double* __restrict__ nstep,
@@ -128,6 +197,16 @@
       for (long long i = (long long)blockIdx.x * kBlock + threadIdx.x; i < N; i += (long long)gridDim.x * kBlock)
         T.s_out[a][i] = s[i] + T.alpha[a] * nstep[i];
   auto xval = [&](int j, int a) { return nstep ? s[j] + T.alpha[a] * nstep[j] : s[j]; };
+  double accD = 0.0;
+  if (DOT) {
+    if (T.flag_dev && blockIdx.x == 0 && threadIdx.x == 0) {
+      const int f = __hip_atomic_load(T.flag_dev, __ATOMIC_RELAXED, __HIP_MEMORY_SCOPE_AGENT);
+      __hip_atomic_store(T.flag_host, f, __ATOMIC_RELAXED, __HIP_MEMORY_SCOPE_SYSTEM);
+      __hip_atomic_store(T.flag_dev, 0, __ATOMIC_RELAXED, __HIP_MEMORY_SCOPE_AGENT);
+    }
+    const long long i = (long long)xcd_block(blockIdx.x, gridDim.x) * kBlock + threadIdx.x;
+    if (i < T.dot_n) accD += T.dot_x[i] * T.dot_y[i];
+  }
   double accF = 0.0, accL = 0.0;
   const int pa = threadIdx.x >> 6, pnode = threadIdx.x & 63;
   const int nchunks = (n + kTrialNodes - 1) / kTrialNodes;
@@ -205,14 +284,17 @@
     }
     __syncthreads();
   }
-  double r[2 * NA], mine[2 * NA];
+  constexpr int D = DOT ? 1 : 0, NOUT = 2 * NA + D;
+  double r[NOUT], mine[NOUT];
+  if (DOT) mine[0] = accD;
 #pragma unroll
   for (int a = 0; a < NA; ++a) {
-    mine[2 * a] = pa == a ? accF : 0.0;
-    mine[2 * a + 1] = pa == a ? accL : 0.0;
-  }
-  block_sum_n<2 * NA>(mine, r);
-  grid_finish<2 * NA>(r, scratch, T.out_dev, T.out_host, lds, sig, xcd_block(blockIdx.x, gridDim.x));
+    mine[D + 2 * a] = pa == a ? accF : 0.0;
+    mine[D + 2 * a + 1] = pa == a ? accL : 0.0;
+  }
+  block_sum_n<NOUT>(mine, r);
+  grid_finish<NOUT>(r, scratch, T.out_dev ? T.out_dev - D : nullptr, T.out_host ? T.out_host - D : nullptr, lds, sig,
+                    xcd_block(blockIdx.x, gridDim.x));
 }
 
 inline int trial_grid(int n) {
@@ -224,13 +306,19 @@
 void trial_launch(hipStream_t st, const DevCsr& B, int n, const BarrierParams& P, const double* s, const double* nstep,
                   const TrialSet& T, const double* Dz0, const double* w, const double* c, const double* phi_ref, double frac,
                   double* scratch, HostSignal sig) {
-#define MGB_TRIAL_NA(NA)                                                                                                    \
-  hipLaunchKernelGGL((trial_f0_kernel<G, NA>), dim3(trial_grid(n)), dim3(kBlock), 0, st, n, B.cols, P, B.rowptr, B.colidx,   \
+#define MGB_TRIAL_NA(NA, DOT)                                                                                                   \
+  hipLaunchKernelGGL((trial_f0_kernel<G, NA, DOT>), dim3(trial_grid(n)), dim3(kBlock), 0, st, n, B.cols, P, B.rowptr, B.colidx, \
                      B.vals, s, nstep, T, Dz0, w, c, phi_ref, frac, scratch, sig)
+  if (T.dot_x) {
+    if (T.na == 3) MGB_TRIAL_NA(3, true);
+    else MGB_TRIAL_NA(4, true);
+    return;
+  }
   switch (T.na) {
-    case 1: MGB_TRIAL_NA(1); break;
-    case 2: MGB_TRIAL_NA(2); break;
-    default: MGB_TRIAL_NA(3); break;
+    case 1: MGB_TRIAL_NA(1, false); break;
+    case 2: MGB_TRIAL_NA(2, false); break;
+    case 3: MGB_TRIAL_NA(3, false); break;
+    default: MGB_TRIAL_NA(4, false); break;
   }
 #undef MGB_TRIAL_NA
 }
@@ -371,6 +459,21 @@
   }
 }
 
+bool spmv_dot_fits(int rows) { return rows > 0 && rows <= kBlock * kMaxBlocks; }
+
+void launch_spmv_dot(hipStream_t st, const DevCsr& A, const double* x, double* y, double* scratch, double* out, double* out_host,
+                     HostSignal sig) {
+  switch (A.group) {
+    case 1: spmv_dot_launch<1>(st, A, x, y, scratch, out, out_host, sig); break;
+    case 2: spmv_dot_launch<2>(st, A, x, y, scratch, out, out_host, sig); break;
+    case 4: spmv_dot_launch<4>(st, A, x, y, scratch, out, out_host, sig); break;
+    case 8: spmv_dot_launch<8>(st, A, x, y, scratch, out, out_host, sig); break;
+    case 16: spmv_dot_launch<16>(st, A, x, y, scratch, out, out_host, sig); break;
+    case 32: spmv_dot_launch<32>(st, A, x, y, scratch, out, out_host, sig); break;
+    default: spmv_dot_launch<64>(st, A, x, y, scratch, out, out_host, sig); break;
+  }
+}
+
 void launch_spmv_el(hipStream_t st, const DevCsr& A, const DevElCsr& E, const double* x, const double* y0, double* y) {
   if (A.rows == 0) return;
   switch (A.group) {
@@ -390,6 +493,11 @@
 }
 
 int f0_blocks(int n) { return std::max(grid_for(n), trial_grid(n)); }
+
+bool trial_dot_fits(int n, int dot_n) {
+  const long long blocks = ((long long)dot_n + kBlock - 1) / kBlock;
+  return dot_n > 0 && blocks <= trial_grid(n) && blocks <= kMaxBlocks;
+}
 
 void launch_trial_set(hipStream_t st, const DevCsr& B, int n, BarrierParams P, const double* s, const double* nstep,
                       const TrialSet& T, const double* Dz0, const double* w, const double* c, const double* phi_ref, double frac,
@@ -438,6 +546,11 @@
   hipLaunchKernelGGL(barrier_f2_kernel_t<double>, dim3(grid_for(n)), dim3(kBlock), 0, st, n, P, Dz, w, Y);
 }
 
+void launch_barrier_f12(hipStream_t st, int n, BarrierParams P, const double* Dz, const double* w, const double* c, double t,
+                        double* v, double* Y) {
+  hipLaunchKernelGGL(barrier_f12_kernel_t<double>, dim3(grid_for(n)), dim3(kBlock), 0, st, n, P, Dz, w, c, t, v, Y);
+}
+
 void launch_barrier_rows_F(hipStream_t st, int n, BarrierParams P, const double* Dz, double* out) {
   if (n == 0) return;
   hipLaunchKernelGGL(barrier_rows_F_kernel, dim3(grid_for(n)), dim3(kBlock), 0, st, n, P, Dz, out);
diff --git a/multigridbarriermpi.jl_amd/csrc/kernels.hpp b/multigridbarriermpi.jl_amd/csrc/kernels.hpp
--- a/multigridbarriermpi.jl_amd/csrc/kernels.hpp
+++ b/multigridbarriermpi.jl_amd/csrc/kernels.hpp
@@ -74,25 +74,37 @@
                      const double* nstep, double* s_out, const double* Dz0, double* Dz, const double* w, const double* c,
                      const double* phi_ref, double frac, double* phi_out, double* scratch, double* out2,
                      double* out2_host = nullptr, HostSignal sig = HostSignal());
+constexpr int kMaxTrialPoints = 4;
 struct TrialSet {
   int na = 0;
-  double alpha[3] = {0.0, 0.0, 0.0};
-  double* s_out[3] = {nullptr, nullptr, nullptr};
-  double* dz[3] = {nullptr, nullptr, nullptr};
-  double* phi_out[3] = {nullptr, nullptr, nullptr};
+  double alpha[kMaxTrialPoints] = {0.0, 0.0, 0.0, 0.0};
+  double* s_out[kMaxTrialPoints] = {nullptr, nullptr, nullptr, nullptr};
+  double* dz[kMaxTrialPoints] = {nullptr, nullptr, nullptr, nullptr};
+  double* phi_out[kMaxTrialPoints] = {nullptr, nullptr, nullptr, nullptr};
   double* out_dev = nullptr;
   double* out_host = nullptr;
+  const double* dot_x = nullptr;
+  const double* dot_y = nullptr;
+  int dot_n = 0;
+  int* flag_dev = nullptr;
+  int* flag_host = nullptr;
 };
+bool trial_dot_fits(int n, int dot_n);
 void launch_trial_set(hipStream_t st, const DevCsr& B, int n, BarrierParams P, const double* s, const double* nstep,
                       const TrialSet& T, const double* Dz0, const double* w, const double* c, const double* phi_ref, double frac,
                       double* scratch, HostSignal sig = HostSignal());
 void launch_barrier_f1(hipStream_t st, int n, BarrierParams P, const double* Dz, const double* w, const double* c,
                        double t, double* v);
 void launch_barrier_f2(hipStream_t st, int n, BarrierParams P, const double* Dz, const double* w, double* Y);
+void launch_barrier_f12(hipStream_t st, int n, BarrierParams P, const double* Dz, const double* w, const double* c, double t,
+                        double* v, double* Y);
 void launch_barrier_rows_F(hipStream_t st, int n, BarrierParams P, const double* Dz, double* out);
 void launch_expand_hessian_rows(hipStream_t st, int n, BarrierParams P, const double* Y, double* out);
 void launch_dot(hipStream_t st, int n, const double* x, const double* y, double* scratch, double* out, double* out_host = nullptr,
                 int* flag_dev = nullptr, int* flag_host = nullptr, HostSignal sig = HostSignal());
+bool spmv_dot_fits(int rows);
+void launch_spmv_dot(hipStream_t st, const DevCsr& A, const double* x, double* y, double* scratch, double* out,
+                     double* out_host = nullptr, HostSignal sig = HostSignal());
 void launch_dot_owned(hipStream_t st, int n, const double* x, const double* y, const int* kind, int count_top, double* scratch,
                       double* out);
 void launch_gather_top(hipStream_t st, int ntop, const int* top, const double* g, double* buf);
diff --git a/multigridbarriermpi.jl_amd/csrc/kernels_tpl.hpp b/multigridbarriermpi.jl_amd/csrc/kernels_tpl.hpp
--- a/multigridbarriermpi.jl_amd/csrc/kernels_tpl.hpp
+++ b/multigridbarriermpi.jl_amd/csrc/kernels_tpl.hpp
@@ -133,47 +133,99 @@
 }
 
 template <class T>
+__device__ inline void barrier_f1_row(const BarrierParams& P, long long q, const T* __restrict__ Dz, const T* __restrict__ w,
+                                      const T* __restrict__ c, T t, T* __restrict__ v) {
+  const T* dz = Dz + q * P.K;
+  const T* cq = c + q * P.K;
+  const T wq = w[q];
+  T vr[kMaxK];
+#pragma unroll
+  for (int j = 0; j < kMaxK; ++j) vr[j] = (j < P.K) ? wq * (t * cq[j]) : T(0);
+  for (int ci = 0; ci < P.ncones; ++ci) {
+    const ConeSpec& S = P.cone[ci];
+    if (!P.active(ci, q)) continue;
+    const ConeAM<T> am = cone_am<T>(P, ci, q);
+    const ConeT<T> k = load_cone<T>(S, dz, am.a);
+    if (S.kind == 1) {
+#pragma unroll
+      for (int j = 0; j < kMaxK; ++j) {
+        T add = T(0);
+#pragma unroll
+        for (int i = 0; i < 3; ++i) add += (i < S.nq && S.iq[i] == j) ? -wq * (T(S.coef[i]) / k.phi) : T(0);
+        vr[j] += add;
+      }
+      continue;
+    }
+    const T ds = am.a * pow_a<T>(k.s, am.a - T(1));
+    const T gs = wq * (-ds / k.phi - am.mu / k.s);
+#pragma unroll
+    for (int j = 0; j < kMaxK; ++j) {
+      T add = T(0);
+#pragma unroll
+      for (int i = 0; i < 3; ++i) add += (i < S.nq && S.iq[i] == j) ? wq * (T(2) * k.q[i] / k.phi) : T(0);
+      add += (S.is == j) ? gs : T(0);
+      add += (S.is2 == j) ? gs : T(0);
+      vr[j] += add;
+    }
+  }
+  T* vq = v + q * P.K;
+#pragma unroll
+  for (int j = 0; j < kMaxK; ++j)
+    if (j < P.K) vq[j] = vr[j];
+}
+
+template <class T>
 __global__ __launch_bounds__(kBlock) void barrier_f1_kernel_t(int n, BarrierParams P, const T* __restrict__ Dz,
                                                                const T* __restrict__ w, const T* __restrict__ c, T t,
                                                                T* __restrict__ v) {
-  for (long long q = (long long)blockIdx.x * kBlock + threadIdx.x; q < n; q += (long long)gridDim.x * kBlock) {
-    const T* dz = Dz + q * P.K;
-    const T* cq = c + q * P.K;
-    const T wq = w[q];
-    T vr[kMaxK];
-#pragma unroll
-    for (int j = 0; j < kMaxK; ++j) vr[j] = (j < P.K) ? wq * (t * cq[j]) : T(0);
-    for (int ci = 0; ci < P.ncones; ++ci) {
-      const ConeSpec& S = P.cone[ci];
-      if (!P.active(ci, q)) continue;
-      const ConeAM<T> am = cone_am<T>(P, ci, q);
-      const ConeT<T> k = load_cone<T>(S, dz, am.a);
-      if (S.kind == 1) {
-#pragma unroll
-        for (int j = 0; j < kMaxK; ++j) {
-          T add = T(0);
-#pragma unroll
-          for (int i = 0; i < 3; ++i) add += (i < S.nq && S.iq[i] == j) ? -wq * (T(S.coef[i]) / k.phi) : T(0);
-          vr[j] += add;
+  for (long long q = (long long)blockIdx.x * kBlock + threadIdx.x; q < n; q += (long long)gridDim.x * kBlock)
+    barrier_f1_row<T>(P, q, Dz, w, c, t, v);
+}
+
+template <class T>
+__device__ inline void barrier_f2_row(const BarrierParams& P, int nY, long long q, const T* __restrict__ Dz,
+                                      const T* __restrict__ w, T* __restrict__ Y) {
+  const T* dz = Dz + q * P.K;
+  T* yq = Y + q * nY;
+  const T wq = w[q];
+  int slot = 0;
+  for (int ci = 0; ci < P.ncones; ++ci) {
+    const ConeSpec& S = P.cone[ci];
+    if (!P.active(ci, q)) {
+      const int ns = S.nY();
+      for (int i = 0; i < ns; ++i) yq[slot++] = T(0);
+      continue;
+    }
+    const ConeAM<T> am = cone_am<T>(P, ci, q);
+    const ConeT<T> k = load_cone<T>(S, dz, am.a);
+    if (S.kind == 1) {
+      const T ip2l = T(1) / (k.phi * k.phi);
+#pragma unroll
+      for (int i = 0; i < 3; ++i)
+#pragma unroll
+        for (int j = 0; j < 3; ++j)
+          if (i < S.nq && j >= i && j < S.nq) yq[slot++] = wq * (T(S.coef[i]) * T(S.coef[j]) * ip2l);
+      continue;
+    }
+    const T a = am.a;
+    const T ds = a * pow_a<T>(k.s, a - T(1));
+    const T dds = (a == T(1)) ? T(0) : a * (a - T(1)) * pow_a<T>(k.s, a - T(2));
+    const T ip = T(1) / k.phi, ip2 = ip * ip;
+    const T hss = -dds * ip + ds * ds * ip2 + am.mu / (k.s * k.s);
+    const int nq = S.nq, nact = S.nact();
+#pragma unroll
+    for (int i = 0; i < 5; ++i)
+#pragma unroll
+      for (int j = 0; j < 5; ++j) {
+        if (i < nact && j >= i && j < nact) {
+          const int ai = min(i, nq), aj = min(j, nq);
+          T h;
+          if (aj < nq) h = T(4) * pick3<T>(k.q, ai) * pick3<T>(k.q, aj) * ip2 + (ai == aj ? T(2) * ip : T(0));
+          else if (ai < nq) h = T(-2) * pick3<T>(k.q, ai) * ds * ip2;
+          else h = hss;
+          yq[slot++] = wq * h;
         }
-        continue;
       }
-      const T ds = am.a * pow_a<T>(k.s, am.a - T(1));
-      const T gs = wq * (-ds / k.phi - am.mu / k.s);
-#pragma unroll
-      for (int j = 0; j < kMaxK; ++j) {
-        T add = T(0);
-#pragma unroll
-        for (int i = 0; i < 3; ++i) add += (i < S.nq && S.iq[i] == j) ? wq * (T(2) * k.q[i] / k.phi) : T(0);
-        add += (S.is == j) ? gs : T(0);
-        add += (S.is2 == j) ? gs : T(0);
-        vr[j] += add;
-      }
-    }
-    T* vq = v + q * P.K;
-#pragma unroll
-    for (int j = 0; j < kMaxK; ++j)
-      if (j < P.K) vq[j] = vr[j];
   }
 }
 
@@ -181,52 +233,21 @@
 __global__ __launch_bounds__(kBlock) void barrier_f2_kernel_t(int n, BarrierParams P, const T* __restrict__ Dz,
                                                                const T* __restrict__ w, T* __restrict__ Y) {
   const int nY = P.nY();
+  for (long long q = (long long)blockIdx.x * kBlock + threadIdx.x; q < n; q += (long long)gridDim.x * kBlock)
+    barrier_f2_row<T>(P, nY, q, Dz, w, Y);
+}
+
+template <class T>
+__global__ __launch_bounds__(kBlock) void barrier_f12_kernel_t(int n, BarrierParams P, const T* __restrict__ Dz,
+                                                                const T* __restrict__ w, const T* __restrict__ c, T t,
+                                                                T* __restrict__ v, T* __restrict__ Y) {
+  const int nY = P.nY();
   for (long long q = (long long)blockIdx.x * kBlock + threadIdx.x; q < n; q += (long long)gridDim.x * kBlock) {
-    const T* dz = Dz + q * P.K;
-    T* yq = Y + q * nY;
-    const T wq = w[q];
-    int slot = 0;
-    for (int ci = 0; ci < P.ncones; ++ci) {
-      const ConeSpec& S = P.cone[ci];
-      if (!P.active(ci, q)) {
-        const int ns = S.nY();
-        for (int i = 0; i < ns; ++i) yq[slot++] = T(0);
-        continue;
-      }
-      const ConeAM<T> am = cone_am<T>(P, ci, q);
-      const ConeT<T> k = load_cone<T>(S, dz, am.a);
-      if (S.kind == 1) {
-        const T ip2l = T(1) / (k.phi * k.phi);
-#pragma unroll
-        for (int i = 0; i < 3; ++i)
-#pragma unroll
-          for (int j = 0; j < 3; ++j)
-            if (i < S.nq && j >= i && j < S.nq) yq[slot++] = wq * (T(S.coef[i]) * T(S.coef[j]) * ip2l);
-        continue;
-      }
-      const T a = am.a;
-      const T ds = a * pow_a<T>(k.s, a - T(1));
-      const T dds = (a == T(1)) ? T(0) : a * (a - T(1)) * pow_a<T>(k.s, a - T(2));
-      const T ip = T(1) / k.phi, ip2 = ip * ip;
-      const T hss = -dds * ip + ds * ds * ip2 + am.mu / (k.s * k.s);
-      const int nq = S.nq, nact = S.nact();
-#pragma unroll
-      for (int i = 0; i < 5; ++i)
-#pragma unroll
-        for (int j = 0; j < 5; ++j) {
-          if (i < nact && j >= i && j < nact) {
-            const int ai = min(i, nq), aj = min(j, nq);
-            T h;
-            if (aj < nq) h = T(4) * pick3<T>(k.q, ai) * pick3<T>(k.q, aj) * ip2 + (ai == aj ? T(2) * ip : T(0));
-            else if (ai < nq) h = T(-2) * pick3<T>(k.q, ai) * ds * ip2;
-            else h = hss;
-            yq[slot++] = wq * h;
-          }
-        }
-    }
-  }
-}
-
-
-}
-}
+    barrier_f1_row<T>(P, q, Dz, w, c, t, v);
+    barrier_f2_row<T>(P, nY, q, Dz, w, Y);
+  }
+}
+
+
+}
+}
```

Result: slower. 87.28 million DoF/s per Newton step (-1.5%).
